# enkeejunior1/Diffusion-Pullback

Measured on AMD Instinct MI355X. Metric: pullback top-k SVD iters/sec (SD-v1.5 mid-block, 4x64x64), higher is better.
Workload: dtype bf16; 1 GPU; BASELINE configs[2]: SD-v1.5 4x64x64 latent, no edit prompt (seeded null ctx[1,77,768]), mid-block h[1280,8,8], t=696.27; pca_rank=5, ctx=null, samples_total=5, samples_this_rank=5, samples_advanced_together=1, spectrum=shaped (configs.Spectrum()), parallelism=single process, no collective, rccl_world_size=0, repeats=7

## Files before the change

diffusion_pullback_amd/csrc/elementwise.hip:

```cpp
#include "kernels.h"

namespace dpb {

static inline unsigned grid_for(long n) {
  long b = (n + 255) / 256;
  return (unsigned)(b < 1 ? 1 : (b > 16384 ? 16384 : b));
}

template <typename T, int MODE>
__global__ __launch_bounds__(256) void geglu_kernel(GegluArgs a, long nrows) {
  constexpr int CH = TT<T>::CH;
  const int fch = a.F / CH;
  const long total = nrows * fch;
  for (long idx = (long)blockIdx.x * 256 + threadIdx.x; idx < total; idx += (long)gridDim.x * 256) {
    const long row = idx / fch;
    const int c = (int)(idx - row * fch) * CH;
    long prow = row;
    if (MODE != MODE_PRIMAL) {
      long j = row / a.rows_per_sample, l = row - j * a.rows_per_sample;
      prow = (j / a.kps) * a.rows_per_sample + l;
    }
    const int ca = a.il ? ((c >> 6) << 7) + (c & 63) : c, dg_ = a.il ? 64 : a.F;
    const T* hp = (const T*)a.h + prow * 2 * a.F;
    float av[CH], gv[CH], o[CH];
    Vec<T>::load(hp + ca, av);
    Vec<T>::load(hp + ca + dg_, gv);
    if (MODE == MODE_PRIMAL) {
      float g1[CH], g2[CH];
#pragma unroll
      for (int e = 0; e < CH; ++e) {
        const float er = erff(gv[e] * 0.70710678118654752f);
        g1[e] = 0.5f * gv[e] * (1.f + er);
        g2[e] = av[e] * (0.5f * (1.f + er) + gv[e] * 0.39894228040143268f * __expf(-0.5f * gv[e] * gv[e]));
        o[e] = av[e] * g1[e];
      }
      Vec<T>::store((T*)a.y + row * a.F + c, o);
      if (a.stash) {
        T* hw = (T*)a.h + prow * 2 * a.F;
        Vec<T>::store(hw + ca, g1);
        Vec<T>::store(hw + ca + dg_, g2);
      }
    } else if (MODE == MODE_TANGENT) {
      const T* dp = (const T*)a.d + row * 2 * a.F;
      float da[CH], dg[CH];
      Vec<T>::load(dp + ca, da);
      Vec<T>::load(dp + ca + dg_, dg);
#pragma unroll
      for (int e = 0; e < CH; ++e) o[e] = da[e] * av[e] + dg[e] * gv[e];
      Vec<T>::store((T*)a.y + row * a.F + c, o);
    } else {
      float gy[CH], o2[CH];
      Vec<T>::load((const T*)a.d + row * a.F + c, gy);
#pragma unroll
      for (int e = 0; e < CH; ++e) {
        o[e] = gy[e] * av[e];
        o2[e] = gy[e] * gv[e];
      }
      T* yp = (T*)a.y + row * 2 * a.F;
      if (a.accumulate) {
        float t1[CH], t2[CH];
        Vec<T>::load(yp + ca, t1);
        Vec<T>::load(yp + ca + dg_, t2);
#pragma unroll
        for (int e = 0; e < CH; ++e) { o[e] += t1[e]; o2[e] += t2[e]; }
      }
      Vec<T>::store(yp + ca, o);
      Vec<T>::store(yp + ca + dg_, o2);
    }
  }
}

template <typename T>
static int geglu_t(int mode, const GegluArgs& a, hipStream_t st) {
  if (a.F % TT<T>::CH) { set_error("geglu: F=%d not chunk aligned", a.F); return -1; }
  if (a.il && (a.il != 64 || a.F % 64)) { set_error("geglu: interleave %d with F=%d unsupported (blocks of 64)", a.il, a.F); return -1; }
  long nrows = (long)(mode == MODE_PRIMAL ? a.Bp : a.NT) * a.rows_per_sample;
  unsigned g = grid_for(nrows * (a.F / TT<T>::CH));
  if (mode == MODE_PRIMAL) DPB_LAUNCH((geglu_kernel<T, MODE_PRIMAL>), dim3(g), dim3(256), 0, st, a, nrows);
  else if (mode == MODE_TANGENT) DPB_LAUNCH((geglu_kernel<T, MODE_TANGENT>), dim3(g), dim3(256), 0, st, a, nrows);
  else DPB_LAUNCH((geglu_kernel<T, MODE_ADJOINT>), dim3(g), dim3(256), 0, st, a, nrows);
  DPB_CHECK(hipGetLastError());
  return 0;
}
int launch_geglu(int dtype, int mode, const GegluArgs& a, hipStream_t st) {
  return DPB_DISPATCH_T(dtype, T, geglu_t<T>(mode, a, st));
}

template <typename T, int OP>
__global__ __launch_bounds__(256) void unary_kernel(const T* x, T* y, long nchunks) {
  constexpr int CH = TT<T>::CH;
  for (long i = (long)blockIdx.x * 256 + threadIdx.x; i < nchunks; i += (long)gridDim.x * 256) {
    float v[CH];
    Vec<T>::load(x + i * CH, v);
    if (OP == 0) {
#pragma unroll
      for (int e = 0; e < CH; ++e) v[e] = silu_(v[e]);
    } else if (OP == 3) {
#pragma unroll
      for (int e = 0; e < CH; ++e) v[e] = v[e] / (1.f + __expf(-1.702f * v[e]));
    } else if (OP == 4) {
#pragma unroll
      for (int e = 0; e < CH; ++e) v[e] = gelu_(v[e]);
    } else if (OP == 2) {
      float o[CH];
      Vec<T>::load(y + i * CH, o);
#pragma unroll
      for (int e = 0; e < CH; ++e) v[e] += o[e];
    }
    Vec<T>::store(y + i * CH, v);
  }
}

template <typename T>
static int unary_t(int op, const void* x, void* y, long n, hipStream_t st) {
  if (n % TT<T>::CH) { set_error("elementwise: n=%ld not chunk aligned", n); return -1; }
  long nc = n / TT<T>::CH;
  unsigned g = grid_for(nc);
  if (op == 0) DPB_LAUNCH((unary_kernel<T, 0>), dim3(g), dim3(256), 0, st, (const T*)x, (T*)y, nc);
  else if (op == 1) DPB_LAUNCH((unary_kernel<T, 1>), dim3(g), dim3(256), 0, st, (const T*)x, (T*)y, nc);
  else if (op == 3) DPB_LAUNCH((unary_kernel<T, 3>), dim3(g), dim3(256), 0, st, (const T*)x, (T*)y, nc);
  else if (op == 4) DPB_LAUNCH((unary_kernel<T, 4>), dim3(g), dim3(256), 0, st, (const T*)x, (T*)y, nc);
  else DPB_LAUNCH((unary_kernel<T, 2>), dim3(g), dim3(256), 0, st, (const T*)x, (T*)y, nc);
  DPB_CHECK(hipGetLastError());
  return 0;
}
int launch_silu(int dtype, const void* x, void* y, long n, hipStream_t st) {
  return DPB_DISPATCH_T(dtype, T, unary_t<T>(0, x, y, n, st));
}
int launch_quick_gelu(int dtype, const void* x, void* y, long n, hipStream_t st) {
  return DPB_DISPATCH_T(dtype, T, unary_t<T>(3, x, y, n, st));
}
int launch_gelu(int dtype, const void* x, void* y, long n, hipStream_t st) {
  return DPB_DISPATCH_T(dtype, T, unary_t<T>(4, x, y, n, st));
}

template <typename T>
__global__ __launch_bounds__(256) void embed_tokens_kernel(const int* ids, const T* tok, const T* pos, float* out, int L, int C, int vocab) {
  const int b = blockIdx.y, t = blockIdx.x;
  int id = ids[b * L + t];
  id = id < 0 ? 0 : (id >= vocab ? vocab - 1 : id);
  for (int c = threadIdx.x; c < C; c += 256)
    out[((long)b * C + c) * L + t] = TT<T>::ld(tok + (long)id * C + c) + TT<T>::ld(pos + (long)t * C + c);
}
int launch_embed_tokens(int dtype, const int* ids, const void* tok, const void* pos, float* out, int batch, int L, int C, int vocab, hipStream_t st) {
  if (batch <= 0 || L <= 0 || C <= 0 || vocab <= 0) { set_error("embed_tokens: empty problem"); return -1; }
  DPB_DISPATCH_STMT(dtype, T, DPB_LAUNCH((embed_tokens_kernel<T>), dim3(L, batch), dim3(256), 0, st, ids, (const T*)tok, (const T*)pos, out, L, C, vocab));
  DPB_CHECK(hipGetLastError());
  return 0;
}

int launch_axpy(int dtype, const void* x, void* y, long n, int accumulate, hipStream_t st) {
  int op = accumulate ? 2 : 1;
  return DPB_DISPATCH_T(dtype, T, unary_t<T>(op, x, y, n, st));
}

template <typename T>
__global__ __launch_bounds__(256) void copy_cols_kernel(const T* src, int lds_, int cs0, T* dst, int ldd, int cd0, long rows,
                                                        int ncols, int accumulate) {
  constexpr int CH = TT<T>::CH;
  const int nch = ncols / CH;
  const long total = rows * nch;
  for (long idx = (long)blockIdx.x * 256 + threadIdx.x; idx < total; idx += (long)gridDim.x * 256) {
    const long r = idx / nch;
    const int c = (int)(idx - r * nch) * CH;
    float v[CH];
    Vec<T>::load(src + r * lds_ + cs0 + c, v);
    T* dp = dst + r * ldd + cd0 + c;
    if (accumulate) {
      float o[CH];
      Vec<T>::load(dp, o);
#pragma unroll
      for (int e = 0; e < CH; ++e) v[e] += o[e];
    }
    Vec<T>::store(dp, v);
  }
}
int launch_copy_cols(int dtype, const void* src, int lds_, int cs0, void* dst, int ldd, int cd0, long rows, int ncols, int accumulate,
                     hipStream_t st) {
  int CH = dt_chunk(dtype);
  if (ncols % CH || cs0 % CH || cd0 % CH || lds_ % CH || ldd % CH) { set_error("copy_cols: misaligned window"); return -1; }
  unsigned g = grid_for(rows * (ncols / CH));
  DPB_DISPATCH_STMT(dtype, T, DPB_LAUNCH((copy_cols_kernel<T>), dim3(g), dim3(256), 0, st, (const T*)src, lds_, cs0, (T*)dst, ldd, cd0, rows, ncols, accumulate));
  DPB_CHECK(hipGetLastError());
  return 0;
}

template <typename T>
__global__ __launch_bounds__(256) void zero_cols_kernel(T* dst, int ldd, int cd0, long rows, int ncols) {
  constexpr int CH = TT<T>::CH;
  const int nch = ncols / CH;
  const long total = rows * nch;
  float v[CH];
#pragma unroll
  for (int e = 0; e < CH; ++e) v[e] = 0.f;
  for (long idx = (long)blockIdx.x * 256 + threadIdx.x; idx < total; idx += (long)gridDim.x * 256) {
    const long r = idx / nch;
    const int c = (int)(idx - r * nch) * CH;
    Vec<T>::store(dst + r * ldd + cd0 + c, v);
  }
}
int launch_zero_cols(int dtype, void* dst, int ldd, int cd0, long rows, int ncols, hipStream_t st) {
  int CH = dt_chunk(dtype);
  if (ncols % CH || cd0 % CH || ldd % CH || cd0 + ncols > ldd) { set_error("zero_cols: misaligned window"); return -1; }
  unsigned g = grid_for(rows * (ncols / CH));
  DPB_DISPATCH_STMT(dtype, T, DPB_LAUNCH((zero_cols_kernel<T>), dim3(g), dim3(256), 0, st, (T*)dst, ldd, cd0, rows, ncols));
  DPB_CHECK(hipGetLastError());
  return 0;
}

template <typename T>
__global__ __launch_bounds__(256) void nchw_to_nhwc_kernel(const float* src, T* dst, int C, int HW, int Cpad) {
  __shared__ float tile[32][33];
  const int n = blockIdx.z;
  const int p0 = blockIdx.x * 32, c0 = blockIdx.y * 32;
  const int tx = threadIdx.x & 31, ty = threadIdx.x >> 5;
  for (int k = ty; k < 32; k += 8) {
    int c = c0 + k, p = p0 + tx;
    tile[k][tx] = (c < C && p < HW) ? src[((long)n * C + c) * HW + p] : 0.f;
  }
  __syncthreads();
  for (int k = ty; k < 32; k += 8) {
    int p = p0 + k, c = c0 + tx;
    if (p < HW && c < Cpad) TT<T>::st(dst + ((long)n * HW + p) * Cpad + c, tile[tx][k]);
  }
}
template <typename T>
__global__ __launch_bounds__(256) void nhwc_to_nchw_kernel(const T* src, float* dst, int C, int HW, int Cpad) {
  __shared__ float tile[32][33];
  const int n = blockIdx.z;
  const int p0 = blockIdx.x * 32, c0 = blockIdx.y * 32;
  const int tx = threadIdx.x & 31, ty = threadIdx.x >> 5;
  for (int k = ty; k < 32; k += 8) {
    int p = p0 + k, c = c0 + tx;
    tile[k][tx] = (p < HW && c < C) ? TT<T>::ld(src + ((long)n * HW + p) * Cpad + c) : 0.f;
  }
  __syncthreads();
  for (int k = ty; k < 32; k += 8) {
    int c = c0 + k, p = p0 + tx;
    if (c < C && p < HW) dst[((long)n * C + c) * HW + p] = tile[tx][k];
  }
}
int launch_nchw_to_nhwc(int dtype, const float* src, void* dst, int n, int C, int HW, int Cpad, hipStream_t st) {
  dim3 grid((HW + 31) / 32, (Cpad + 31) / 32, n);
  DPB_DISPATCH_STMT(dtype, T, DPB_LAUNCH((nchw_to_nhwc_kernel<T>), grid, dim3(256), 0, st, src, (T*)dst, C, HW, Cpad));
  DPB_CHECK(hipGetLastError());
  return 0;
}
int launch_nhwc_to_nchw(int dtype, const void* src, float* dst, int n, int C, int HW, int Cpad, hipStream_t st) {
  dim3 grid((HW + 31) / 32, (C + 31) / 32, n);
  DPB_DISPATCH_STMT(dtype, T, DPB_LAUNCH((nhwc_to_nchw_kernel<T>), grid, dim3(256), 0, st, (const T*)src, dst, C, HW, Cpad));
  DPB_CHECK(hipGetLastError());
  return 0;
}

constexpr int SHIFT_TP = 32, SHIFT_TC = 64;
template <typename T, int VEC>
__global__ __launch_bounds__(256) void shift_tap_kernel(T* h, const float* u, ShiftRows rows, int b0, int nb, int bcast, int C, int Cv, long HW) {
  constexpr int CPP = SHIFT_TC / VEC;
  constexpr int ITER = SHIFT_TP * CPP / 256;
  __shared__ float tile[SHIFT_TC][SHIFT_TP + 1];
  const long p0 = (long)blockIdx.x * SHIFT_TP;
  const int c0 = blockIdx.y * SHIFT_TC;
  const int tx = threadIdx.x & 31, ty = threadIdx.x >> 5;
  const long img = HW * (long)C;
  float src[ITER][VEC];
  auto ld = [&](const T* p, float* o) {
    if constexpr (VEC == 1) o[0] = TT<T>::ld(p); else Vec<T>::load(p, o);
  };
  auto st = [&](T* p, const float* o) {
    if constexpr (VEC == 1) TT<T>::st(p, o[0]); else Vec<T>::store(p, o);
  };
  if (bcast) {
#pragma unroll
    for (int it = 0; it < ITER; ++it) {
      const int q = it * 256 + threadIdx.x, pl = q / CPP, c = c0 + (q % CPP) * VEC;
      if (p0 + pl < HW && c < C) ld(h + (p0 + pl) * C + c, src[it]);
    }
  }
  for (int r = 0; r < nb; ++r) {
    const int b = b0 + r, dir = rows.dir[r];
    const float sc = rows.scale[r];
    if (dir < 0 && !(bcast && b > 0)) continue;
    if (dir >= 0) {
      __syncthreads();
      const float* ub = u + (long)dir * Cv * HW;
      for (int k = ty; k < SHIFT_TC; k += 8) {
        const int c = c0 + k;
        tile[k][tx] = (c < Cv && p0 + tx < HW) ? ub[(long)c * HW + p0 + tx] : 0.f;
      }
      __syncthreads();
    }
    T* hb = h + (long)b * img;
#pragma unroll
    for (int it = 0; it < ITER; ++it) {
      const int q = it * 256 + threadIdx.x, pl = q / CPP, cl = (q % CPP) * VEC, c = c0 + cl;
      if (p0 + pl >= HW || c >= C) continue;
      T* p = hb + (p0 + pl) * C + c;
      float v[VEC];
      if (bcast) {
#pragma unroll
        for (int e = 0; e < VEC; ++e) v[e] = src[it][e];
      } else {
        ld(p, v);
      }
      if (dir >= 0) {
#pragma unroll
        for (int e = 0; e < VEC; ++e) v[e] += sc * tile[cl + e][pl];
      }
      st(p, v);
    }
  }
}

template <typename T>
static int shift_tap_t(void* h, const float* u, const int* dir, const float* scale, int batch, int bcast, int C, int Cv, long HW, hipStream_t st) {
  const dim3 grid((unsigned)((HW + SHIFT_TP - 1) / SHIFT_TP), (unsigned)((C + SHIFT_TC - 1) / SHIFT_TC));
  for (int b0 = (batch - 1) / SHIFT_MAX_ROWS * SHIFT_MAX_ROWS; b0 >= 0; b0 -= SHIFT_MAX_ROWS) {
    ShiftRows rows;
    const int nb = std::min(SHIFT_MAX_ROWS, batch - b0);
    for (int r = 0; r < nb; ++r) { rows.dir[r] = dir[b0 + r]; rows.scale[r] = scale[b0 + r]; }
    if (C % TT<T>::CH == 0) DPB_LAUNCH((shift_tap_kernel<T, TT<T>::CH>), grid, dim3(256), 0, st, (T*)h, u, rows, b0, nb, bcast, C, Cv, HW);
    else DPB_LAUNCH((shift_tap_kernel<T, 1>), grid, dim3(256), 0, st, (T*)h, u, rows, b0, nb, bcast, C, Cv, HW);
    DPB_CHECK(hipGetLastError());
  }
  return 0;
}
int launch_shift_tap(int dtype, void* h, const float* u, const int* dir, const float* scale, int batch, int bcast, int C, int Cv, long HW,
                     hipStream_t st) {
  if (batch < 1 || C < 1 || Cv < 1 || Cv > C || HW < 1) { set_error("shift_tap: empty or inconsistent problem"); return -1; }
  return DPB_DISPATCH_T(dtype, T, shift_tap_t<T>(h, u, dir, scale, batch, bcast, C, Cv, HW, st));
}

__global__ __launch_bounds__(256) void replicate_rows_kernel(ReplTable t, int batch) {
  uint4* p = (uint4*)t.p[blockIdx.y];
  const long n = t.chunks[blockIdx.y];
  for (long i = (long)blockIdx.x * 256 + threadIdx.x; i < n; i += (long)gridDim.x * 256) {
    const uint4 v = p[i];
    for (int b = 1; b < batch; ++b) p[(long)b * n + i] = v;
  }
}
int launch_replicate_rows(void* const* bufs, const size_t* sample_bytes, int nbufs, int batch, hipStream_t st) {
  if (batch < 2) return 0;
  for (int i0 = 0; i0 < nbufs; i0 += REPL_MAX_BUFS) {
    ReplTable t;
    const int n = std::min(REPL_MAX_BUFS, nbufs - i0);
    long most = 1;
    for (int i = 0; i < n; ++i) {
      if (sample_bytes[i0 + i] % 16 || (uintptr_t)bufs[i0 + i] % 16) { set_error("replicate_rows: buffer %d is not a whole number of aligned 16-byte chunks per sample", i0 + i); return -1; }
      t.p[i] = bufs[i0 + i];
      t.chunks[i] = (long)(sample_bytes[i0 + i] / 16);
      most = std::max(most, t.chunks[i]);
    }
    DPB_LAUNCH(replicate_rows_kernel, dim3(std::min(grid_for(most), 2048u), n), dim3(256), 0, st, t, batch);
    DPB_CHECK(hipGetLastError());
  }
  return 0;
}

template <typename T>
__global__ __launch_bounds__(256) void pool2x2_kernel(const T* in, T* out, int n, int H, int W, int C, int accumulate, float scale) {
  constexpr int CH = TT<T>::CH;
  const int cch = C / CH;
  const long total = (long)n * H * W * cch;
  for (long idx = (long)blockIdx.x * 256 + threadIdx.x; idx < total; idx += (long)gridDim.x * 256) {
    const int c = (int)(idx % cch) * CH;
    long pix = idx / cch;
    const int x = (int)(pix % W);
    pix /= W;
    const int y = (int)(pix % H);
    const long s = pix / H;
    float acc[CH];
#pragma unroll
    for (int e = 0; e < CH; ++e) acc[e] = 0.f;
#pragma unroll
    for (int dy = 0; dy < 2; ++dy)
#pragma unroll
      for (int dx = 0; dx < 2; ++dx) {
        float v[CH];
        Vec<T>::load(in + ((s * 2 * H + 2 * y + dy) * 2 * W + 2 * x + dx) * C + c, v);
#pragma unroll
        for (int e = 0; e < CH; ++e) acc[e] += v[e];
      }
    T* op = out + ((s * H + y) * W + x) * C + c;
#pragma unroll
    for (int e = 0; e < CH; ++e) acc[e] *= scale;
    if (accumulate) {
      float o[CH];
      Vec<T>::load(op, o);
#pragma unroll
      for (int e = 0; e < CH; ++e) acc[e] += o[e];
    }
    Vec<T>::store(op, acc);
  }
}
template <typename T>
__global__ __launch_bounds__(256) void up2x2_kernel(const T* in, T* out, int n, int H, int W, int C, int accumulate, float scale) {
  constexpr int CH = TT<T>::CH;
// ... 83 lines not shown
```

diffusion_pullback_amd/csrc/engine.cpp:

```cpp
#include <math.h>
#include <stdarg.h>
#include <stdio.h>
#include <stdlib.h>
#include <string.h>

#include <string>
#include <vector>

#include "../../include/dpb.h"
#include "kernels.h"

namespace dpb {

static thread_local char g_err[1024] = "";
void set_error(const char* fmt, ...) {
  va_list ap;
  va_start(ap, fmt);
  vsnprintf(g_err, sizeof(g_err), fmt, ap);
  va_end(ap);
}
const char* last_error() { return g_err; }
thread_local long launch_count = 0;

static inline size_t align_up(size_t v, size_t a = 256) { return (v + a - 1) / a * a; }
static inline int round8(int v) { return (v + 7) / 8 * 8; }

struct Buf {
  int rows = 0, C = 0, kind = 0, Cv = 0;
  bool is_const = true;
  size_t p_off = 0, t_off = 0, g_off = 0, g_off0 = 0;
};

struct AttnPlan {
  int heads = 0, d = 0, Lq = 0, Lk = 0, Lqp = 0, Lkp = 0;
  bool causal = false;
  bool kv_const = false, fused = false, cross = false;
  int oq = 0, ok = 0, ov = 0;
  size_t P = 0, PT = 0, KT = 0, VT = 0, QT = 0, stats = 0;
  bool fold_ok = false;
  bool fold_live = false;
  int q_op = -1, o_op = -1;
  size_t Gt = 0, Gk = 0, F = 0, Fk = 0, Pf = 0;
  const char* gA = nullptr;
};

struct Op {
  dpb_op_desc d;
  bool is_const = true;
  int attn = -1;
  size_t pstats = 0, tstats = 0;
  size_t aff = 0;
  int geglu_next = -1;
  int geglu_prev = -1;
  int ln_next = -1;
  int ln_prev = -1;
  int fold_plan = -1, fold_role = 0;
};

}

using namespace dpb;

struct dpb_engine {
  int dtype = DT_F32, es = 4;
  int maxB = 1, maxT = 1;
  std::vector<Buf> bufs;
  std::vector<Op> ops;
  std::vector<AttnPlan> plans;
  std::vector<int> producer;
  std::vector<std::vector<int>> mod_users;
  int x_buf = -1, x_channels = 0, temb_buf = -1, temb_dim = 0, temb_flip = 0, temb_hm1 = 0, ctx_buf = -1;
  std::string per_sample_t_why;
  bool temb_read = false;
  hipStream_t stream = 0;
  char* ws = nullptr;
  size_t ws_bytes = 0;
  size_t pstats_off = 0, pstats_bytes = 0, tstats_off = 0, tstats_bytes = 0, gnpart = 0, gnpart_bytes = 0, gnticket = 0;
  size_t S1 = 0, S2 = 0, T1 = 0, Dv = 0, convtmp = 0, io_in = 0, io_out = 0, orth = 0, slab = 0, slab_bytes = 64u << 20, zeros = 0;
  size_t orth_stride = 0;
  size_t pbW = 0;
  size_t temb_host_stage = 0;
  int cur_batch = 0;
  std::vector<int> uses;
  std::vector<std::vector<char>> act_cache;
  int primal_last = -1;
  struct { bool on = false; GemmArgs a; } pend;
  std::vector<char> ginit;
  std::vector<char> skip;
  long n_launch = 0;
  double flops = 0, gbytes = 0;
  struct GraphKey {
    int tap, k, B; const void *V, *U, *s, *conv;
    bool operator==(const GraphKey& o) const { return tap == o.tap && k == o.k && B == o.B && V == o.V && U == o.U && s == o.s && conv == o.conv; }
  };
  hipGraphExec_t gexec = nullptr;
  GraphKey gkey{};
  long g_launches = 0; double g_flops = 0, g_bytes = 0;
  bool profiling = false;
  struct Prof { hipEvent_t a, b; double flops; int big; int M, N, K, Z, gather; };
  std::vector<Prof> prof;
  float prof_overhead_ms = 0.f;

  char* P(int b) const { return ws + bufs[b].p_off; }
  char* T(int b) const { return ws + bufs[b].t_off; }
  char* G(int b) const { return ws + bufs[b].g_off; }
};

namespace {

int fail(const char* fmt, ...) {
  va_list ap;
  va_start(ap, fmt);
  vsnprintf(g_err, sizeof(g_err), fmt, ap);
  va_end(ap);
  return -1;
}

struct Forward {
  bool stash = true;
  bool temb_resident = false;
  int seed = -1;
  const float* h = nullptr;
  const float* u = nullptr; const int32_t* dir = nullptr; const float* scale = nullptr;
  int xbatch = 0;
};

struct Pass {
  int mode, tap;
  int src;
  const char *bact, *oact;
  Forward fwd;
  bool per_sample_t = false;
  int srow = 0;
  Pass(const dpb_engine* e, int mode_, int tap_, int src_, const char* flags)
      : mode(mode_), tap(tap_), src(src_), bact(flags), oact(flags + e->bufs.size()) {}
};

struct OpInputs {
  int id[4], n;
  const int* begin() const { return id; }
  const int* end() const { return id + n; }
};
OpInputs op_inputs(const dpb_op_desc& d) {
  OpInputs r{{d.in0}, 1};
  if (d.kind == DPB_OP_ATTENTION || d.kind == DPB_OP_CONCAT) r.id[r.n++] = d.in1;
  if (d.kind == DPB_OP_ATTENTION) r.id[r.n++] = d.in2;
  if (d.kind == DPB_OP_CONV && d.res >= 0) r.id[r.n++] = d.res;
  if (d.kind == DPB_OP_GROUPNORM && d.ip[2]) r.id[r.n++] = d.in1;
  return r;
}
bool gn_modulated(const dpb_op_desc& d) { return d.kind == DPB_OP_GROUPNORM && d.ip[2] != 0; }

struct LaunchSpan {
  dpb_engine* e; long at;
  explicit LaunchSpan(dpb_engine* e_) : e(e_), at(launch_count) {}
  ~LaunchSpan() { e->n_launch = launch_count - at; }
};

char* primal_ptr(const dpb_engine* e, const Pass& ps, int b) {
  const Buf& bf = e->bufs[b];
  return e->P(b) + (bf.kind == DPB_BUF_SHARED ? (size_t)ps.srow * bf.rows * bf.C * e->es : 0);
}

void gemm_prep(dpb_engine* e, GemmArgs& a) {
  a.slab = (float*)(e->ws + e->slab);
  a.zeros = e->ws + e->zeros;
  a.slab_bytes = e->slab_bytes;
}

int g_lazy_reduce = getenv("DPB_LAZY_REDUCE") ? atoi(getenv("DPB_LAZY_REDUCE")) : 1;
int g_ln_fuse = getenv("DPB_LN_FUSE") ? atoi(getenv("DPB_LN_FUSE")) : 0;
int g_ln_kmax = getenv("DPB_LN_FUSE_KMAX") ? atoi(getenv("DPB_LN_FUSE_KMAX")) : 1024;

int flush_pending(dpb_engine* e) {
  if (!e->pend.on) return 0;
  e->pend.on = false;
  return launch_gemm_reduce(e->dtype, e->pend.a, e->stream);
}

int prof_open(dpb_engine* e, double flops, int kind, int M, int N, int K, int Z, int gather) {
  if (!e->profiling) return -1;
  dpb_engine::Prof p;
  p.flops = flops; p.big = kind; p.M = M; p.N = N; p.K = K; p.Z = Z; p.gather = gather;
  if (hipEventCreate(&p.a) != hipSuccess) return -1;
  if (hipEventCreate(&p.b) != hipSuccess) { (void)hipEventDestroy(p.a); return -1; }
  (void)hipEventRecord(p.a, e->stream);
  e->prof.push_back(p);
  return (int)e->prof.size() - 1;
}
void prof_close(dpb_engine* e, int idx) {
  if (idx >= 0) (void)hipEventRecord(e->prof[idx].b, e->stream);
}

int g_geglu_fwd = getenv("DPB_GEGLU_FWD") ? atoi(getenv("DPB_GEGLU_FWD")) : 1;
int g_cross_primal = getenv("DPB_CROSS_PRIMAL") ? atoi(getenv("DPB_CROSS_PRIMAL")) : 1;
int g_cross_fold = getenv("DPB_CROSS_FOLD") ? atoi(getenv("DPB_CROSS_FOLD")) : 1;
bool fold_route(const dpb_engine* e, const AttnPlan& p) {
  if (!g_cross_fold || !p.fold_ok || e->cur_batch != 1 || !g_cross_primal) return false;
  if (g_cross_fold == 2) return true;
  const long H = p.heads, C = H * p.d;
  return 208 * H * C <= 2 * C * C + 384 * C && (g_cross_fold == 1 || C >= g_cross_fold);
}
bool fold_on(const dpb_engine* e, const Pass& ps, const AttnPlan& p) {
  return p.fold_live && fold_route(e, p) && e->producer[ps.src] < p.q_op && e->producer[ps.tap] >= p.o_op;
}
int gemm(dpb_engine* e, GemmArgs a, bool can_defer = false) {
  if (e->pend.on)
    if (int r = flush_pending(e)) return r;
  gemm_prep(e, a);
  GemmArgs* pend = (can_defer && g_lazy_reduce) ? &e->pend.a : nullptr;
  const double fl = 2.0 * a.M * (double)a.N * ((double)a.K + (a.A2 ? a.K2 : 0)) * a.Z1 * a.Z2;
  e->flops += fl;
  e->gbytes += ((double)a.M * a.K + (double)a.N * a.K + (double)a.M * a.N) * a.Z1 * a.Z2 * e->es;
  const GemmPlan pl = gemm_plan(e->dtype, a);
  const int pi = prof_open(e, fl, pl.row ? pl.row->kind : 0, a.M, a.N, a.K, a.Z1 * a.Z2, a.gather);
  const int r = launch_gemm(e->dtype, a, e->stream, pend, &pl);
  e->pend.on = pend && pend->splitk > 1;
  prof_close(e, pi);
  return r;
}

int conv_fwd(dpb_engine* e, const Op& op, const Pass& ps, int n) {
  const dpb_op_desc& d = op.d;
  const int mode = ps.mode;
  const int H = d.ip[0], W = d.ip[1], Cin = d.ip[2], Ho = d.ip[3], Wo = d.ip[4], Cout = d.ip[5], KS = d.ip[6];
  const Buf& bi = e->bufs[d.in0];
  const Buf& bo = e->bufs[d.out];
  if (mode == 1 && !ps.bact[d.in0]) {
    return launch_axpy(e->dtype, e->T(d.res), e->T(d.out), (long)n * bo.rows * bo.C, 0, e->stream);
  }
  GemmArgs g;
  const bool shared_out = bo.kind == DPB_BUF_SHARED;
  const int ns = shared_out ? 1 : n;
  g.A = mode == 0 ? primal_ptr(e, ps, d.in0) : e->T(d.in0);
  g.B = d.w[0];
  g.C = mode == 0 ? primal_ptr(e, ps, d.out) : e->T(d.out);
  g.N = Cout;
  g.K = KS * KS * Cin;
  g.ldb = g.K;
  g.ldc = bo.C;
  g.lda = bi.C;
  g.gather = d.ip[9];
  if (g.gather == GATHER_NONE) {
    g.M = ns * bi.rows;
  } else {
    g.M = ns * Ho * Wo;
    g.H = H; g.W = W; g.Cin = Cin; g.Ho = Ho; g.Wo = Wo; g.KS = KS; g.stride = d.ip[7]; g.pad = d.ip[8];
  }
  if (mode == 0) {
    g.bias = (const float*)d.w[2];
    if (d.rowbias >= 0) {
      g.rowbias = e->P(d.rowbias) + (size_t)d.ip[10] * e->es;
      g.rows_per_sample = bo.rows;
      g.ldrb = e->bufs[d.rowbias].rows * e->bufs[d.rowbias].C;
      g.rowbias_div = ps.per_sample_t ? 1 : 1 << 30;
    }
  }
  if (d.res >= 0 && (mode == 0 || ps.bact[d.res])) {
    g.R = mode == 0 ? primal_ptr(e, ps, d.res) : e->T(d.res);
    g.ldr = e->bufs[d.res].C;
  }
  if (mode == 1 && op.fold_role && fold_on(e, ps, e->plans[op.fold_plan])) {
    const AttnPlan& p = e->plans[op.fold_plan];
    if (op.fold_role == 1) return 0;
    g.A = e->ws + e->S1; g.lda = 80 * p.heads;
    g.B = e->ws + p.Fk; g.K = g.ldb = 80 * p.heads;
  }
  if (mode == 1 && op.ln_next >= 0 && g_ln_fuse) {
    const dpb_op_desc& ld = e->ops[op.ln_next].d;
    GemmArgs f = g;
    f.epi = EPI_LN_TAN; f.C2 = e->T(ld.out); f.ln_x = e->P(ld.in0); f.ln_gamma = (const float*)ld.w[0]; f.ln_eps = ld.fp[0];
    f.rows_per_sample = bo.rows; f.epi_kps = n / e->cur_batch;
    gemm_prep(e, f);
    if (gemm_epi_supported(e->dtype, f)) {
      e->skip[op.ln_next] = 1;
      return gemm(e, f);
    }
  }
  if (mode == 1 && op.geglu_next >= 0) {
    const dpb_op_desc& gd = e->ops[op.geglu_next].d;
    GemmArgs f = g;
    f.epi = EPI_GEGLU_TAN; f.hprim = e->P(d.out); f.epi_kps = n / e->cur_batch; f.rows_per_sample = bo.rows;
    f.C = e->T(gd.out); f.ldc = e->bufs[gd.out].C;
    gemm_prep(e, f);
    if (gemm_epi_supported(e->dtype, f)) {
      e->skip[op.geglu_next] = 1;
      return gemm(e, f);
    }
  }
  if (mode == 0 && !ps.fwd.stash && op.geglu_next >= 0 && g_geglu_fwd && !shared_out && d.out != ps.tap && d.out != ps.fwd.seed) {
    const dpb_op_desc& gd = e->ops[op.geglu_next].d;
    GemmArgs f = g;
    f.epi = EPI_GEGLU_FWD; f.C = e->P(gd.out); f.ldc = e->bufs[gd.out].C; f.rowbias = nullptr; f.R = nullptr;
    gemm_prep(e, f);
    GemmArgs probe = g; gemm_prep(e, probe);
    if (!g.rowbias && !g.R && gemm_epi_supported(e->dtype, f) && gemm_plan(e->dtype, probe).splitk == 1) {
      e->skip[op.geglu_next] = 1;
      return gemm(e, f);
    }
  }
  return gemm(e, g, mode == 1 && !shared_out);
}

int conv_adj(dpb_engine* e, const Op& op, const Pass& ps, int n) {
  const dpb_op_desc& d = op.d;
  const int H = d.ip[0], W = d.ip[1], Cin = d.ip[2], Ho = d.ip[3], Wo = d.ip[4], KS = d.ip[6];
  const Buf& bi = e->bufs[d.in0];
  const Buf& bo = e->bufs[d.out];
  const int Cout = bo.C;
  if (ps.bact[d.in0]) {
    if (!d.w[1]) return fail("conv op has no transposed weight (w[1]) but its adjoint is needed");
    GemmArgs g;
    g.A = e->G(d.out);
    g.lda = bo.C;
    g.B = d.w[1];
    g.N = Cin;
    g.K = KS * KS * Cout;
    g.ldb = g.K;
    g.ldc = bi.C;
    const int gather = d.ip[9];
    if (op.fold_role && fold_on(e, ps, e->plans[op.fold_plan])) {
      AttnPlan& p = e->plans[op.fold_plan];
      if (op.fold_role == 2) {
        p.gA = e->G(d.out);
        e->ginit[d.in0] = 1;
        goto residual;
      }
      g.A = e->ws + e->S1; g.lda = 80 * p.heads;
      g.B = e->ws + p.Gk; g.K = g.ldb = 80 * p.heads;
    }
    if (gather == GATHER_NONE && op.ln_prev >= 0 && g_ln_fuse && e->uses[d.in0] == 1 && d.in0 != ps.src && (g.K <= g_ln_kmax || (g_ln_fuse & 2))) {
      const dpb_op_desc& ld = e->ops[op.ln_prev].d;
      GemmArgs f = g;
      f.M = n * bi.rows;
      f.epi = EPI_LN_ADJ; f.C = e->G(ld.in0); f.ldc = e->bufs[ld.in0].C; f.accumulate = e->ginit[ld.in0];
      f.ln_x = e->P(ld.in0); f.ln_gamma = (const float*)ld.w[0]; f.ln_eps = ld.fp[0];
      f.rows_per_sample = bi.rows; f.epi_kps = n / e->cur_batch;
      gemm_prep(e, f);
      if (gemm_epi_supported(e->dtype, f)) {
        if (int r = gemm(e, f)) return r;
        e->ginit[ld.in0] = 1;
        goto residual;
      }
    }
    if (gather == GATHER_NONE && op.geglu_prev >= 0 && d.in0 != ps.src) {
      const dpb_op_desc& gd = e->ops[op.geglu_prev].d;
      GemmArgs f = g;
      f.M = n * bi.rows;
      f.epi = EPI_GEGLU_ADJ; f.hprim = e->P(gd.in0); f.epi_kps = n / e->cur_batch; f.rows_per_sample = bi.rows;
      f.C = e->G(gd.in0); f.ldc = e->bufs[gd.in0].C; f.accumulate = e->ginit[gd.in0];
      gemm_prep(e, f);
      if (gemm_epi_supported(e->dtype, f)) {
        if (int r = gemm(e, f)) return r;
        e->ginit[gd.in0] = 1;
        goto residual;
      }
    }
    const bool lone = e->uses[d.in0] == 1 && d.in0 != ps.src;
    if (gather == GATHER_NONE) {
      g.M = n * bi.rows;
      g.C = e->G(d.in0);
      g.accumulate = e->ginit[d.in0];
      if (int r = gemm(e, g, lone)) return r;
    } else if (gather == GATHER_CONV) {
      g.gather = GATHER_CONVT;
      g.M = n * H * W;
      g.H = Ho; g.W = Wo; g.Cin = Cout; g.Ho = H; g.Wo = W; g.KS = KS; g.stride = d.ip[7]; g.pad = d.ip[8];
      g.C = e->G(d.in0);
      g.accumulate = e->ginit[d.in0];
      if (int r = gemm(e, g, lone)) return r;
    } else {
      g.gather = GATHER_CONVT;
      g.M = n * Ho * Wo;
      g.H = Ho; g.W = Wo; g.Cin = Cout; g.Ho = Ho; g.Wo = Wo; g.KS = KS; g.stride = 1; g.pad = 1;
      g.C = e->ws + e->convtmp;
      if (int r = gemm(e, g)) return r;
      if (int r = launch_pool2x2_sum(e->dtype, e->ws + e->convtmp, e->G(d.in0), n, H, W, bi.C, e->ginit[d.in0], e->stream)) return r;
    }
    e->ginit[d.in0] = 1;
  }
residual:
  if (d.res >= 0 && ps.bact[d.res]) {
    Buf& br = e->bufs[d.res];
    if (!e->ginit[d.res] && br.rows == bo.rows && br.C == bo.C && br.kind == bo.kind) {
      std::swap(br.g_off, e->bufs[d.out].g_off);
    } else {
      if (int r = launch_axpy(e->dtype, e->G(d.out), e->G(d.res), (long)n * bo.rows * bo.C, e->ginit[d.res], e->stream)) return r;
    }
    e->ginit[d.res] = 1;
  }
  return 0;
}

void take_pending(dpb_engine* e, SlabSrc& src, const void* d, bool store) {
  if (!e->pend.on || e->pend.a.C != d) return;
  const GemmArgs& g = e->pend.a;
  src.slab = g.slab; src.splitk = g.splitk; src.MN = (long)g.M * g.N; src.N = g.N;
  src.R = g.R; src.ldr = g.ldr;
  src.store = store ? g.C : nullptr;
  e->pend.on = false;
}

bool consumes_pending(dpb_engine* e, const Op& op, int mode) {
  if (mode == MODE_PRIMAL || (op.d.kind != DPB_OP_GROUPNORM && op.d.kind != DPB_OP_LAYERNORM)) return false;
  const void* d = mode == MODE_TANGENT ? (const void*)e->T(op.d.in0) : (const void*)e->G(op.d.out);
  if (d != e->pend.a.C) return false;
  const Buf& bi = e->bufs[op.d.in0];
  if (e->pend.a.N != bi.C) return false;
  if (op.d.kind == DPB_OP_GROUPNORM) {
    GNArgs a; a.HW = bi.rows; a.C = bi.C; a.G = op.d.ip[0]; a.NT = 1;
    return groupnorm_is_one_launch(e->dtype, a);
  }
  return true;
}

template <class A>
void fill_io(dpb_engine* e, const dpb_op_desc& d, const Pass& ps, int n, A& a) {
  if (ps.mode == MODE_PRIMAL) { a.Bp = n; a.y = e->P(d.out); return; }
  a.Bp = e->cur_batch; a.NT = n; a.kps = n / e->cur_batch;
  if (ps.mode == MODE_TANGENT) { a.d = e->T(d.in0); a.y = e->T(d.out); return; }
  a.d = e->G(d.out); a.y = e->G(d.in0);
  a.accumulate = e->ginit[d.in0];
  e->ginit[d.in0] = 1;
}
template <class A>
void fill_norm_io(dpb_engine* e, const dpb_op_desc& d, const Pass& ps, int n, A& a) {
  fill_io(e, d, ps, n, a);
  if (ps.mode != MODE_PRIMAL) take_pending(e, a.src, a.d, ps.mode == MODE_TANGENT && (e->uses[d.in0] > 1 || d.in0 == ps.tap));
}

int gn_run(dpb_engine* e, const Op& op, const Pass& ps, int n) {
  const dpb_op_desc& d = op.d;
  const Buf& bi = e->bufs[d.in0];
  GNArgs a;
  a.x = e->P(d.in0);
  a.gamma = (const float*)d.w[0];
  a.beta = (const float*)d.w[1];
  if (gn_modulated(d)) {
    a.gamma = (const float*)(e->ws + op.aff);
    a.beta = a.gamma + (size_t)e->maxB * bi.C;
    a.astride = bi.C;
  }
  a.pstats = (double*)(e->ws + op.pstats);
  a.tstats = (double*)(e->ws + op.tstats);
  a.part = (float*)(e->ws + e->gnpart); a.part_bytes = e->gnpart_bytes; a.ticket = (int*)(e->ws + e->gnticket);
  a.det = gn_deterministic();
  a.HW = bi.rows; a.C = bi.C; a.G = d.ip[0]; a.silu = d.ip[1]; a.eps = d.fp[0];
  fill_norm_io(e, d, ps, n, a);
  return launch_groupnorm(e->dtype, ps.mode, a, e->stream);
}

int ln_run(dpb_engine* e, const Op& op, const Pass& ps, int n) {
  const dpb_op_desc& d = op.d;
  const Buf& bi = e->bufs[d.in0];
  LNArgs a;
  a.x = e->P(d.in0);
  a.gamma = (const float*)d.w[0];
  a.beta = (const float*)d.w[1];
  a.rows_per_sample = bi.rows; a.C = bi.C; a.eps = d.fp[0];
  fill_norm_io(e, d, ps, n, a);
  return launch_layernorm(e->dtype, ps.mode, a, e->stream);
}

int geglu_run(dpb_engine* e, const Op& op, const Pass& ps, int n) {
  const dpb_op_desc& d = op.d;
  const Buf& bi = e->bufs[d.in0];
  GegluArgs a;
  a.h = e->P(d.in0);
  a.rows_per_sample = bi.rows; a.F = bi.C / 2; a.il = d.ip[1];
  a.stash = ps.fwd.stash;
  fill_io(e, d, ps, n, a);
  return launch_geglu(e->dtype, ps.mode, a, e->stream);
}

int fill_affine(dpb_engine* e, int src, const Pass& ps, int batch) {
  const std::vector<int>& users = e->mod_users[src];
  if (users.empty()) return 0;
  const Buf& be = e->bufs[e->ops[src].d.out];
  std::vector<AdaGNOp> t(users.size());
  for (size_t i = 0; i < users.size(); ++i) {
    const Op& u = e->ops[users[i]];
    const int C = e->bufs[u.d.in0].C;
    t[i].gamma = (const float*)u.d.w[0]; t[i].beta = (const float*)u.d.w[1];
    t[i].emb = e->P(u.d.in1) + (size_t)u.d.ip[3] * e->es;
    t[i].og = (float*)(e->ws + u.aff); t[i].ob = t[i].og + (size_t)e->maxB * C;
    t[i].C = C;
  }
  return launch_adagn_affine(e->dtype, t.data(), (int)t.size(), (long)be.rows * be.C, batch, ps.per_sample_t ? 1 : 0, e->stream);
}

int resample_run(dpb_engine* e, const Op& op, const Pass& ps, int n) {
  const dpb_op_desc& d = op.d;
  const bool up = d.ip[0] == 1;
  const int H = d.ip[1], W = d.ip[2], C = e->bufs[d.in0].C;
  const int h = up ? H : H / 2, w = up ? W : W / 2;
  if (ps.mode == MODE_ADJOINT) {
    const int acc = e->ginit[d.in0];
    e->ginit[d.in0] = 1;
    return up ? launch_pool2x2(e->dtype, e->G(d.out), e->G(d.in0), n, h, w, C, 1.f, acc, e->stream)
              : launch_up2x2(e->dtype, e->G(d.out), e->G(d.in0), n, h, w, C, 0.25f, acc, e->stream);
  }
  const char* in = ps.mode == MODE_PRIMAL ? e->P(d.in0) : e->T(d.in0);
  char* out = ps.mode == MODE_PRIMAL ? e->P(d.out) : e->T(d.out);
  return up ? launch_up2x2(e->dtype, in, out, n, h, w, C, 1.f, 0, e->stream) : launch_pool2x2(e->dtype, in, out, n, h, w, C, 0.25f, 0, e->stream);
}

int concat_run(dpb_engine* e, const Op& op, const Pass& ps, int n) {
  const dpb_op_desc& d = op.d;
  const int mode = ps.mode;
  const Buf& b0 = e->bufs[d.in0];
  const Buf& b1 = e->bufs[d.in1];
  const Buf& bo = e->bufs[d.out];
  const long rows = (long)n * bo.rows;
  if (mode == MODE_ADJOINT) {
    if (ps.bact[d.in0]) {
      if (int r = launch_copy_cols(e->dtype, e->G(d.out), bo.C, 0, e->G(d.in0), b0.C, 0, rows, b0.C, e->ginit[d.in0], e->stream)) return r;
      e->ginit[d.in0] = 1;
    }
    if (ps.bact[d.in1]) {
      if (int r = launch_copy_cols(e->dtype, e->G(d.out), bo.C, b0.C, e->G(d.in1), b1.C, 0, rows, b1.C, e->ginit[d.in1], e->stream)) return r;
      e->ginit[d.in1] = 1;
    }
    return 0;
  }
  if (mode == MODE_TANGENT && (!ps.bact[d.in0] || !ps.bact[d.in1])) {
    char* o = e->T(d.out);
    if (int r = ps.bact[d.in0] ? launch_copy_cols(e->dtype, e->T(d.in0), b0.C, 0, o, bo.C, 0, rows, b0.C, 0, e->stream)
                               : launch_zero_cols(e->dtype, o, bo.C, 0, rows, b0.C, e->stream)) return r;
    return ps.bact[d.in1] ? launch_copy_cols(e->dtype, e->T(d.in1), b1.C, 0, o, bo.C, b0.C, rows, b1.C, 0, e->stream)
                          : launch_zero_cols(e->dtype, o, bo.C, b0.C, rows, b1.C, e->stream);
  }
  char* o = mode == MODE_PRIMAL ? e->P(d.out) : e->T(d.out);
  const char* i0 = mode == MODE_PRIMAL ? e->P(d.in0) : e->T(d.in0);
  const char* i1 = mode == MODE_PRIMAL ? e->P(d.in1) : e->T(d.in1);
  if (int r = launch_copy_cols(e->dtype, i0, b0.C, 0, o, bo.C, 0, rows, b0.C, 0, e->stream)) return r;
  return launch_copy_cols(e->dtype, i1, b1.C, 0, o, bo.C, b0.C, rows, b1.C, 0, e->stream);
}

struct AttnPtrs {
  const char *Q, *K, *V; char* O;
  int ldq, ldk, ldv, ldo;
};
static AttnPtrs attn_ptrs(dpb_engine* e, const dpb_op_desc& d, const AttnPlan& p, int which ) {
  AttnPtrs a;
  auto base = [&](int b) { return which == 0 ? e->P(b) : which == 1 ? e->T(b) : e->G(b); };
  a.ldq = e->bufs[d.in0].C; a.ldk = e->bufs[d.in1].C; a.ldv = e->bufs[d.in2].C; a.ldo = e->bufs[d.out].C;
  a.Q = base(d.in0) + (size_t)p.oq * e->es;
  a.K = (which == 0 || !p.kv_const) ? base(d.in1) + (size_t)p.ok * e->es : nullptr;
  a.V = (which == 0 || !p.kv_const) ? base(d.in2) + (size_t)p.ov * e->es : nullptr;
  a.O = base(d.out);
  return a;
}

void fill_fused(dpb_engine* e, const AttnPlan& p, const AttnPtrs& x, FusedAttnArgs& f, int kps, float scale) {
  char* ws = e->ws;
  f.Q = x.Q; f.K = x.K; f.V = x.V; f.O = x.O; f.VT = ws + p.VT; f.KT = ws + p.KT; f.QT = ws + p.QT;
  f.stats = (const float*)(ws + p.stats);
  f.L = p.Lq; f.C = x.ldq; f.Co = x.ldo; f.H = p.heads; f.d = p.d; f.kps = kps; f.scale = scale; f.fl = e->dtype == DT_F16;
}
void fill_cross(dpb_engine* e, const AttnPlan& p, const AttnPtrs& x, CrossAttnArgs& f, int kps, float scale, const void* BT, const void* X, int Cx,
                void* Y, int Cy) {
  f.Q = x.Q; f.K = x.K; f.V = x.V; f.BT = BT; f.X = X; f.Y = Y;
  f.L = p.Lq; f.Lk = p.Lk; f.Lkp = p.Lkp; f.C = x.ldq; f.Ck = x.ldk; f.Cx = Cx; f.Cy = Cy;
  f.H = p.heads; f.d = p.d; f.kps = kps; f.scale = scale; f.fl = e->dtype == DT_F16;
}

template <class F>
int attn_launch(dpb_engine* e, const AttnPlan& p, int kind, int n_prod, int Z1, int gather, F launch) {
  const double fl = 2.0 * p.Lq * (double)p.Lk * p.d * n_prod * Z1 * p.heads;
  e->flops += fl;
  const int pi = prof_open(e, fl, kind, p.Lq, p.Lk, p.d, Z1 * p.heads, gather);
  const int r = launch();
  prof_close(e, pi);
  return r;
}

enum Side { SIDE_A, SIDE_B, SIDE_C, SIDE_A2, SIDE_B2 };
void set_side(GemmArgs& g, Side s, const void* ptr, int ld, long s1, long s2, int div) {
  switch (s) {
    case SIDE_A: g.A = ptr; g.lda = ld; g.sA1 = s1; g.sA2 = s2; g.divA = div; break;
    case SIDE_B: g.B = ptr; g.ldb = ld; g.sB1 = s1; g.sB2 = s2; g.divB = div; break;
    case SIDE_C: g.C = (void*)ptr; g.ldc = ld; g.sC1 = s1; g.sC2 = s2; break;
    case SIDE_A2: g.A2 = ptr; g.lda2 = ld; g.sA21 = s1; g.sA22 = s2; g.divA2 = div; break;
    case SIDE_B2: g.B2 = ptr; g.ldb2 = ld; g.sB21 = s1; g.sB22 = s2; g.divB2 = div; break;
  }
}
void side_rows(GemmArgs& g, Side s, const void* ptr, int ld, int L, int d, int div = 1) { set_side(g, s, ptr, ld, (long)L * ld, d, div); }
void side_tile(GemmArgs& g, Side s, const void* ptr, int H, int rows, int Lp, int div = 1) {
  set_side(g, s, ptr, Lp, (long)H * rows * Lp, (long)rows * Lp, div);
}
void dims(GemmArgs& g, int M, int N, int K, int Z1, int Z2, float alpha = 1.f) { g.M = M; g.N = N; g.K = K; g.Z1 = Z1; g.Z2 = Z2; g.alpha = alpha; }
int head_transpose(dpb_engine* e, const AttnPlan& p, const void* in, int ld, void* out, int Z, int L, int Lp) {
  return launch_transpose(e->dtype, in, out, Z, p.heads, (long)L * ld, p.d, L, p.d, ld, Lp, (long)p.d * Lp, e->stream);
}

int fold_build(dpb_engine* e, const AttnPlan& p, const AttnPtrs& x, float scale) {
  const int H = p.heads, C = H * p.d, W = 80 * H;
  const void* WqT = e->ops[p.q_op].d.w[1];
  const void* Wo = e->ops[p.o_op].d.w[0];
  char* ws = e->ws;
  for (int which = 0; which < 2; ++which) {
    const void* kv = which ? x.V : x.K; const int ldkv = which ? x.ldv : x.ldk;
    const void* w = which ? Wo : WqT;
    const float alpha = which ? 1.f : scale;
    GemmArgs t;
    side_rows(t, SIDE_A, kv, ldkv, p.Lk, p.d);
    side_rows(t, SIDE_B, w, C, C, p.d);
    set_side(t, SIDE_C, ws + (which ? p.F : p.Gt), C, 0, 128L * C, 1);
    dims(t, p.Lk, C, p.d, 1, H, alpha);
    if (int r = gemm(e, t)) return r;
    GemmArgs k;
    side_rows(k, SIDE_A, w, C, C, p.d);
    side_rows(k, SIDE_B, kv, ldkv, p.Lk, p.d);
    set_side(k, SIDE_C, ws + (which ? p.Fk : p.Gk), W, 0, 80, 1);
    dims(k, C, p.Lk, p.d, 1, H, alpha);
    if (int r = gemm(e, k)) return r;
  }
  return 0;
}

int fold_product1(dpb_engine* e, const AttnPlan& p, const void* X, int ldx, size_t B, int nt) {
  const int H = p.heads, C = H * p.d;
  GemmArgs g;
  g.A = X; g.lda = ldx; g.B = e->ws + B; g.ldb = C;
// ... 279 lines not shown
extern "C" {

const char* dpb_last_error(void) { return g_err; }
int dpb_abi_version(void) { return DPB_ABI_VERSION; }

int dpb_engine_create(const dpb_net_desc* net, dpb_engine** out) {
  if (!net || !out) return fail("null argument");
  if (net->dtype != DPB_F32 && net->dtype != DPB_BF16 && net->dtype != DPB_F16) return fail("bad dtype %d", net->dtype);
  if (net->max_batch < 1 || net->max_tangents < 1) return fail("max_batch/max_tangents must be >= 1");
  dpb_engine* e = new dpb_engine();
  e->dtype = net->dtype;
  e->es = net->dtype == DPB_F32 ? 4 : 2;
  e->maxB = net->max_batch;
  e->maxT = net->max_tangents;
  e->x_buf = net->x_buf; e->x_channels = net->x_channels; e->temb_buf = net->temb_buf; e->temb_dim = net->temb_dim;
  e->temb_flip = net->temb_flip_sin_to_cos; e->temb_hm1 = net->temb_half_minus_one; e->ctx_buf = net->ctx_buf;
  const int nb = net->n_buffers;
  e->bufs.resize(nb);
  e->producer.assign(nb, -1);
  auto bad = [&](const char* m, int i) { fail("op %d: %s", i, m); delete e; return -1; };
  for (int i = 0; i < nb; ++i) {
    e->bufs[i].rows = net->buffers[i].rows;
    e->bufs[i].C = net->buffers[i].channels;
    e->bufs[i].kind = net->buffers[i].kind;
    e->bufs[i].Cv = net->buffers[i].valid_channels > 0 ? net->buffers[i].valid_channels : net->buffers[i].channels;
    if (e->bufs[i].rows < 1 || e->bufs[i].C < 8 || e->bufs[i].C % 8) { fail("buffer %d: rows=%d channels=%d (channels must be a multiple of 8)", i, e->bufs[i].rows, e->bufs[i].C); delete e; return -1; }
  }
  if (net->x_buf < 0 || net->x_buf >= nb) { fail("bad x_buf"); delete e; return -1; }
  e->bufs[net->x_buf].is_const = false;
  auto okb = [&](int b) { return b >= 0 && b < nb; };
  for (int i = 0; i < net->n_ops; ++i) {
    Op op;
    op.d = net->ops[i];
    const dpb_op_desc& d = op.d;
    if (!okb(d.out)) return bad("bad buffer id", i);
    bool c = true;
    for (int b : op_inputs(d)) {
      if (!okb(b)) return bad("bad buffer id", i);
      c = c && e->bufs[b].is_const;
    }
    if (d.kind == DPB_OP_ATTENTION) {
      AttnPlan p;
      p.heads = d.ip[0];
      p.oq = d.ip[1]; p.ok = d.ip[2]; p.ov = d.ip[3];
      p.causal = d.ip[4] != 0;
      const int Cattn = e->bufs[d.out].C;
      if (p.heads < 1 || Cattn % p.heads) return bad("channels not divisible by heads", i);
      p.d = Cattn / p.heads;
      if (p.oq % 8 || p.ok % 8 || p.ov % 8 || p.oq + Cattn > e->bufs[d.in0].C || p.ok + Cattn > e->bufs[d.in1].C || p.ov + Cattn > e->bufs[d.in2].C)
        return bad("bad q/k/v column window", i);
      auto part = [&](int b0, int o0, int b1, int o1) { return b0 == b1 && o0 != o1 && o0 < o1 + Cattn && o1 < o0 + Cattn; };
      if (part(d.in0, p.oq, d.in1, p.ok) || part(d.in0, p.oq, d.in2, p.ov) || part(d.in1, p.ok, d.in2, p.ov))
        return bad("q/k/v windows of one buffer must coincide or be disjoint", i);
      if (p.d % 8) return bad("head dim must be a multiple of 8", i);
      p.Lq = e->bufs[d.in0].rows; p.Lk = e->bufs[d.in1].rows;
      p.Lqp = round8(p.Lq); p.Lkp = round8(p.Lk);
      if (e->bufs[d.in1].is_const != e->bufs[d.in2].is_const) return bad("k and v must both depend on x or both not", i);
      if (e->bufs[d.in0].is_const) return bad("attention query independent of x is unsupported", i);
      p.kv_const = e->bufs[d.in1].is_const;
      op.attn = (int)e->plans.size();
      e->plans.push_back(p);
    }
    if (d.kind == DPB_OP_CONV) {
      if (d.rowbias >= 0 && (!okb(d.rowbias) || e->bufs[d.rowbias].kind != DPB_BUF_SHARED)) return bad("rowbias must be a SHARED buffer", i);
      if (d.rowbias >= 0 && (d.ip[10] < 0 || d.ip[10] % 8 || d.ip[10] + round8(d.ip[5]) > e->bufs[d.rowbias].C)) return bad("bad rowbias column window", i);
      if (!d.w[0]) return bad("missing weight", i);
      if (d.ip[2] != e->bufs[d.in0].C || e->bufs[d.out].C != round8(d.ip[5])) return bad("conv channel mismatch", i);
    }
    if (d.kind == DPB_OP_GROUPNORM) {
      const Buf& gi = e->bufs[d.in0];
      if (gn_modulated(d)) {
        if (e->bufs[d.in1].kind != DPB_BUF_SHARED || e->bufs[d.in1].rows != 1 || e->producer[d.in1] < 0)
          return bad("modulated groupnorm: in1 must be a one-row SHARED buffer produced by an earlier op (the embedding projection)", i);
        if (gi.kind != DPB_BUF_ACT) return bad("modulated groupnorm: the normalised buffer must be a per-sample activation", i);
        if (d.ip[3] < 0 || d.ip[3] % 8 || d.ip[3] + 2 * gi.C > e->bufs[d.in1].C) return bad("modulated groupnorm: bad (scale | shift) column window", i);
        if (!d.w[0] || !d.w[1]) return bad("modulated groupnorm: missing gamma / beta", i);
      }
    }
    if (d.kind == DPB_OP_RESAMPLE) {
      const Buf& ri = e->bufs[d.in0];
      const Buf& ro = e->bufs[d.out];
      const int H = d.ip[1], W = d.ip[2];
      if (d.ip[0] != 0 && d.ip[0] != 1) return bad("resample: ip[0] must be 0 (2x2 average pool) or 1 (nearest x2 upsample)", i);
      if (H < 1 || W < 1 || (long)H * W != ri.rows || ri.C != ro.C || ri.kind != DPB_BUF_ACT || ro.kind != DPB_BUF_ACT) return bad("resample: input shape mismatch", i);
      if (d.ip[0] == 0 ? (H % 2 || W % 2 || (long)(H / 2) * (W / 2) != ro.rows) : (long)4 * H * W != ro.rows) return bad("resample: output shape mismatch", i);
    }
    for (int b : op_inputs(d)) e->temb_read = e->temb_read || b == e->temb_buf;
    if (e->per_sample_t_why.empty()) {
      char why[160] = "";
      const bool so = e->bufs[d.out].kind == DPB_BUF_SHARED;
      for (int b : op_inputs(d))
        if ((e->bufs[b].kind == DPB_BUF_SHARED) != so && !(gn_modulated(d) && b == d.in1))
          snprintf(why, sizeof(why), "op %d reads %s buffer %d into %s buffer %d", i, so ? "per-sample" : "SHARED", b, so ? "SHARED" : "per-sample", d.out);
      if (so && !(d.kind == DPB_OP_SILU || (d.kind == DPB_OP_CONV && d.ip[9] == DPB_GATHER_NONE && d.rowbias < 0)))
        snprintf(why, sizeof(why), "op %d writes SHARED buffer %d and is neither a linear layer nor an activation", i, d.out);
      e->per_sample_t_why = why;
    }
    op.is_const = c;
    e->bufs[d.out].is_const = c;
    if (e->producer[d.out] >= 0) return bad("buffer written twice (tape must be SSA)", i);
    e->producer[d.out] = i;
    e->ops.push_back(op);
  }
  e->mod_users.assign(e->ops.size(), std::vector<int>());
  for (size_t i = 0; i < e->ops.size(); ++i)
    if (gn_modulated(e->ops[i].d)) e->mod_users[e->producer[e->ops[i].d.in1]].push_back((int)i);
  {
    std::vector<int> uses(nb, 0), user(nb, -1);
    for (size_t i = 0; i < e->ops.size(); ++i) {
      for (int b : op_inputs(e->ops[i].d)) { uses[b]++; user[b] = (int)i; }
    }
    e->uses = uses;
    for (size_t j = 0; j < e->ops.size(); ++j) {
      const dpb_op_desc& d = e->ops[j].d;
      if (d.kind != DPB_OP_LAYERNORM || e->ops[j].is_const || e->dtype == DT_F32 || e->bufs[d.in0].C != 320 || e->bufs[d.in0].kind != DPB_BUF_ACT) continue;
      const int pi = e->producer[d.in0];
      if (pi >= 0 && e->ops[pi].d.kind == DPB_OP_CONV && e->ops[pi].d.ip[9] == DPB_GATHER_NONE && !e->ops[pi].is_const) e->ops[pi].ln_next = (int)j;
      if (uses[d.out] == 1) {
        const int ci = user[d.out];
        const dpb_op_desc& cd = e->ops[ci].d;
        if (cd.kind == DPB_OP_CONV && cd.ip[9] == DPB_GATHER_NONE && cd.in0 == d.out && cd.w[1]) e->ops[ci].ln_prev = (int)j;
      }
    }
    for (size_t j = 0; j < e->ops.size(); ++j) {
      const dpb_op_desc& d = e->ops[j].d;
      if (d.kind == DPB_OP_GEGLU && uses[d.in0] != 1) return bad("the input buffer of a GEGLU op must have no other consumer (the primal pass overwrites it in place)", (int)j);
      if (d.kind != DPB_OP_GEGLU || d.ip[1] != 64 || e->ops[j].is_const || getenv("DPB_NO_GEGLU_FUSE")) continue;
      const int pi = e->producer[d.in0];
      if (pi >= 0 && uses[d.in0] == 1) {
        const dpb_op_desc& pd = e->ops[pi].d;
        if (pd.kind == DPB_OP_CONV && pd.ip[9] == DPB_GATHER_NONE && pd.res < 0 && e->bufs[d.in0].kind == DPB_BUF_ACT) e->ops[pi].geglu_next = (int)j;
      }
      if (uses[d.out] == 1) {
        const int ci = user[d.out];
        const dpb_op_desc& cd = e->ops[ci].d;
        if (cd.kind == DPB_OP_CONV && cd.ip[9] == DPB_GATHER_NONE && cd.in0 == d.out) e->ops[ci].geglu_prev = (int)j;
      }
    }
    for (size_t j = 1; j + 1 < e->ops.size(); ++j) {
      const dpb_op_desc& d = e->ops[j].d;
      if (d.kind != DPB_OP_ATTENTION || e->ops[j].is_const) continue;
      AttnPlan& p = e->plans[e->ops[j].attn];
      const int C = p.heads * p.d;
      if (!p.kv_const || p.causal || e->dtype == DT_F32 || p.oq != 0 || e->bufs[d.in0].C != C || e->bufs[d.out].C != C || p.Lk > 80) continue;
      const dpb_op_desc &qd = e->ops[j - 1].d, &od = e->ops[j + 1].d;
      auto plain = [&](const dpb_op_desc& c) {
        return c.kind == DPB_OP_CONV && c.ip[9] == DPB_GATHER_NONE && c.ip[6] == 1 && c.ip[2] == C && c.ip[5] == C && c.rowbias < 0 && c.w[1] &&
               e->bufs[c.in0].kind == DPB_BUF_ACT && e->bufs[c.out].kind == DPB_BUF_ACT;
      };
      if (!plain(qd) || qd.out != d.in0 || qd.res >= 0 || uses[d.in0] != 1 || e->ops[j - 1].is_const) continue;
      if (!plain(od) || od.in0 != d.out || uses[d.out] != 1) continue;
      p.q_op = (int)j - 1; p.o_op = (int)j + 1; p.fold_ok = true;
    }
    e->skip.assign(e->ops.size(), 0);
  }
  size_t off = 0;
  auto take = [&](size_t bytes) { size_t o = off; off = align_up(off + bytes); return o; };
  const size_t es = e->es;
  for (auto& b : e->bufs) {
    size_t n = e->maxB;
    b.p_off = take(n * b.rows * (size_t)b.C * es);
  }
  for (auto& b : e->bufs)
    if (!b.is_const) b.t_off = take((size_t)e->maxT * b.rows * b.C * es);
  for (auto& b : e->bufs)
    if (!b.is_const) b.g_off = b.g_off0 = take((size_t)e->maxT * b.rows * b.C * es);
  size_t s1 = 0, s2 = 0, t1 = 0, dv = 0, ctmp = 0, maxrc = 0;
  for (auto& op : e->ops) {
    const dpb_op_desc& d = op.d;
    if (d.kind == DPB_OP_ATTENTION) {
      AttnPlan& p = e->plans[op.attn];
      const size_t H = p.heads;
      p.fused = !p.causal && fused_attention_supported(e->dtype, p.d, p.Lq, p.kv_const) && !getenv("DPB_NO_FUSED_ATTN") &&
                p.Lq >= (getenv("DPB_FUSED_ATTN_MIN_L") ? atoi(getenv("DPB_FUSED_ATTN_MIN_L")) : 64) &&
                e->bufs[d.in0].C == e->bufs[d.in1].C && e->bufs[d.in0].C == e->bufs[d.in2].C;
      p.cross = !p.causal && cross_attention_supported(e->dtype, p.d, p.Lq, p.Lk, p.kv_const) && !getenv("DPB_NO_CROSS_ATTN") &&
                e->bufs[d.in1].C == e->bufs[d.in2].C;
      if (!p.fused) p.P = take((size_t)e->maxB * H * p.Lq * p.Lkp * es);
      p.fold_ok = p.fold_ok && p.cross;
      if (p.fold_ok) {
        const size_t C = H * p.d;
        p.Gt = take(H * 128 * C * es); p.F = take(H * 128 * C * es);
        p.Gk = take(C * 80 * H * es); p.Fk = take(C * 80 * H * es);
        p.Pf = take((size_t)p.Lq * H * 80 * sizeof(float));
        s1 = std::max(s1, (size_t)e->maxT * H * p.Lq * 80 * es);
        e->ops[p.q_op].fold_plan = e->ops[p.o_op].fold_plan = op.attn;
        e->ops[p.q_op].fold_role = 1; e->ops[p.o_op].fold_role = 2;
      }
      p.VT = take((size_t)e->maxB * H * p.d * p.Lkp * es);
      p.KT = take((size_t)e->maxB * H * p.d * p.Lkp * es);
      if (!p.fused) s1 = std::max(s1, (size_t)e->maxT * H * p.Lq * p.Lkp * es);
      size_t lmax = std::max(p.Lqp, p.Lkp);
      t1 = std::max(t1, (size_t)e->maxT * H * p.d * lmax * es);
      if (p.fused) p.stats = take((size_t)e->maxB * H * p.Lq * 2 * sizeof(float));
      if (!p.kv_const) {
        if (!p.fused) p.PT = take((size_t)e->maxB * H * p.Lk * p.Lqp * es);
        p.QT = take((size_t)e->maxB * H * p.d * p.Lqp * es);
        if (!p.fused) s2 = std::max(s2, (size_t)e->maxT * H * p.Lk * p.Lqp * es);
        dv = std::max(dv, (size_t)e->maxT * H * p.Lq * sizeof(float));
      }
    } else if (d.kind == DPB_OP_GROUPNORM) {
      op.pstats = e->pstats_bytes;
      e->pstats_bytes += (size_t)e->maxB * d.ip[0] * 2 * sizeof(double);
      if (!op.is_const) {
        op.tstats = e->tstats_bytes;
        e->tstats_bytes += (size_t)e->maxT * d.ip[0] * 2 * sizeof(double);
      }
      if (gn_modulated(d)) op.aff = take((size_t)2 * e->maxB * e->bufs[d.in0].C * sizeof(float));
    } else if (d.kind == DPB_OP_CONV && d.ip[9] == DPB_GATHER_UPCONV && !op.is_const) {
      ctmp = std::max(ctmp, (size_t)e->maxT * d.ip[3] * d.ip[4] * e->bufs[d.in0].C * es);
    }
  }
  for (auto& b : e->bufs) maxrc = std::max(maxrc, (size_t)b.rows * b.C);
  e->pstats_off = take(e->pstats_bytes);
  e->tstats_off = take(e->tstats_bytes);
  {
    size_t need = 0;
    for (auto& op : e->ops)
      if (op.d.kind == DPB_OP_GROUPNORM) {
        const size_t hw = e->bufs[op.d.in0].rows, nmax = (size_t)std::max(e->maxB, e->maxT);
        const size_t blocks = std::max<size_t>(nmax * ((hw + 7) / 8), 1);
        need = std::max(need, std::min<size_t>(blocks, std::max<size_t>(1024, nmax * ((hw + 63) / 64))) * 2 * op.d.ip[0] * sizeof(float));
      }
    e->gnpart_bytes = need;
    e->gnpart = take(need);
    e->gnticket = take(sizeof(int) * (size_t)std::max(e->maxB, e->maxT));
  }
  for (auto& op : e->ops)
    if (op.d.kind == DPB_OP_GROUPNORM) { op.pstats += e->pstats_off; op.tstats += e->tstats_off; }
  e->S1 = take(s1); e->S2 = take(s2); e->T1 = take(t1); e->Dv = take(dv); e->convtmp = take(ctmp);
  const size_t nio = (size_t)std::max(e->maxB, e->maxT) * maxrc * sizeof(float);
  e->io_in = take(nio);
  e->io_out = take(nio);
  e->orth_stride = align_up(orth_scratch_bytes(std::min(ORTH_MAX_RANK, std::max(56, e->maxT)), (long)e->bufs[e->x_buf].rows * e->x_channels));
  e->orth = take(e->orth_stride * (size_t)e->maxB);
  e->slab = take(e->slab_bytes);
  e->zeros = take(256);
  const size_t nx = (size_t)e->bufs[e->x_buf].rows * e->x_channels;
  e->pbW = take((size_t)e->maxT * nx * sizeof(float));
  e->ws_bytes = off;
  e->ginit.assign(nb, 0);
  e->act_cache.assign(nb, std::vector<char>());
  if (!seed_flags(e, e->x_buf)) { delete e; return -1; }
  *out = e;
  return 0;
}

void dpb_engine_destroy(dpb_engine* e) {
  if (e && e->gexec) (void)hipGraphExecDestroy(e->gexec);
  delete e;
}

int dpb_engine_set_stream(dpb_engine* e, void* s) {
  if (!e) return fail("null engine");
  e->stream = (hipStream_t)s;
  return 0;
}

size_t dpb_engine_workspace_bytes(const dpb_engine* e) { return e ? e->ws_bytes : 0; }

int dpb_engine_set_workspace(dpb_engine* e, void* ws, size_t bytes) {
  if (!e || !ws) return fail("null argument");
  if (bytes < e->ws_bytes) return fail("workspace too small: %zu < %zu", bytes, e->ws_bytes);
  if ((uintptr_t)ws % 256) return fail("workspace must be 256-byte aligned");
  e->ws = (char*)ws;
  e->cur_batch = 0;
  DPB_CHECK(hipMemsetAsync(ws, 0, e->ws_bytes, e->stream));
  return 0;
}

static int shift_seed(dpb_engine* e, const Forward& f, int batch, int xb, int last) {
  const int src = f.seed, ps = e->producer[src];
  const Buf& bs = e->bufs[src];
  if (int r = launch_shift_tap(e->dtype, e->P(src), f.u, f.dir, f.scale, batch, xb < batch, bs.C, bs.Cv, bs.rows, e->stream)) return r;
  if (xb == batch) return 0;
  std::vector<char> seen(e->bufs.size(), 0);
  std::vector<void*> ptr;
  std::vector<size_t> bytes;
  for (int i = ps + 1; i <= last; ++i)
    for (int b : op_inputs(e->ops[i].d)) {
      if (b == src || seen[b] || e->bufs[b].kind == DPB_BUF_SHARED || e->producer[b] > ps) continue;
      seen[b] = 1;
      ptr.push_back(e->P(b));
      bytes.push_back((size_t)e->bufs[b].rows * e->bufs[b].C * e->es);
    }
  return launch_replicate_rows(ptr.data(), bytes.data(), (int)ptr.size(), batch, e->stream);
}

static void temb_row(const dpb_engine* e, float t, float* emb) {
  const int half = e->temb_dim / 2;
  for (int i = 0; i < half; ++i) {
    float fr;
    if (e->temb_hm1) fr = expf((float)i * (float)(-(log(10000.0) / (double)(half - 1))));
    else fr = expf(((float)(-log(10000.0)) * (float)i) / (float)half);
    float ang = t * fr;
    float s = sinf(ang), c = cosf(ang);
    if (e->temb_flip) { emb[i] = c; emb[half + i] = s; } else { emb[i] = s; emb[half + i] = c; }
  }
}

static int primal_pass(dpb_engine* e, const float* x, int batch, float t, const float* ctx, int upto_buf, const Forward& f, const float* tv = nullptr) {
  if (!e || !x) return fail("null argument");
  if (!e->ws) return fail("workspace not set (dpb_engine_set_workspace)");
  if (batch < 1 || batch > e->maxB) return fail("batch=%d outside [1,%d]", batch, e->maxB);
  if (upto_buf < 0 || upto_buf >= (int)e->bufs.size() || e->producer[upto_buf] < 0) return fail("invalid upto buffer %d", upto_buf);
  const LaunchSpan span(e);
  e->flops = 0; e->gbytes = 0;
  Pass ps(e, MODE_PRIMAL, upto_buf, e->x_buf, seed_flags(e, e->x_buf));
  ps.fwd = f;
  ps.per_sample_t = tv != nullptr;
  const Buf& bx = e->bufs[e->x_buf];
  const int xb = f.u ? f.xbatch : batch;
  if (int r = launch_nchw_to_nhwc(e->dtype, x, e->P(e->x_buf), xb, e->x_channels, bx.rows, bx.C, e->stream)) return r;
  if (e->ctx_buf >= 0) {
    if (!ctx) return fail("this network needs ctx (encoder_hidden_states)");
    const Buf& bc = e->bufs[e->ctx_buf];
    if (int r = launch_nchw_to_nhwc(e->dtype, ctx, e->P(e->ctx_buf), xb * bc.rows, bc.Cv, 1, bc.C, e->stream)) return r;
  }
  if (e->temb_buf >= 0 && !f.temb_resident) {
    const int nrow = tv ? batch : 1;
    const size_t C = e->bufs[e->temb_buf].C;
    std::vector<float> emb(nrow * C, 0.f);
    for (int b = 0; b < nrow; ++b) temb_row(e, tv ? tv[b] : t, emb.data() + b * C);
    float* stage = (float*)(e->ws + e->io_in);
    DPB_CHECK(hipMemcpyAsync(stage, emb.data(), emb.size() * sizeof(float), hipMemcpyHostToDevice, e->stream));
    DPB_CHECK(hipStreamSynchronize(e->stream));
    for (int b = 0; b < nrow; ++b)
      if (int r = launch_nchw_to_nhwc(e->dtype, stage + b * C, e->P(e->temb_buf) + b * C * e->es, 1, (int)C, 1, (int)C, e->stream)) return r;
  }
  if (e->pstats_bytes && !gn_deterministic()) DPB_CHECK(hipMemsetAsync(e->ws + e->pstats_off, 0, e->pstats_bytes, e->stream));
  e->cur_batch = batch;
  e->pend.on = false;
  const int last = e->producer[upto_buf];
  const int seed_op = f.seed >= 0 ? e->producer[f.seed] : -1;
  e->primal_last = -1;
  for (auto& p : e->plans) p.fold_live = false;
  std::fill(e->skip.begin(), e->skip.end(), 0);
  for (int i = 0; i <= last; ++i) {
    if (e->skip[i]) continue;
    const int reps = tv && e->bufs[e->ops[i].d.out].kind == DPB_BUF_SHARED ? batch : 1;
    for (ps.srow = 0; ps.srow < reps; ++ps.srow)
      if (int r = run_op(e, e->ops[i], ps, i <= seed_op ? xb : batch)) return r;
    ps.srow = 0;
    if (int r = fill_affine(e, i, ps, batch)) return r;
    if (i == seed_op && f.u) {
      if (int r = shift_seed(e, f, batch, xb, last)) return r;
    } else if (i == seed_op) {
      const Buf& bs = e->bufs[f.seed];
      if (int r = launch_nchw_to_nhwc(e->dtype, f.h, e->P(f.seed), batch, bs.Cv, bs.rows, bs.C, e->stream)) return r;
    }
  }
  if (f.stash) e->primal_last = last;
  return 0;
}

int dpb_primal(dpb_engine* e, const float* x, int batch, float t, const float* ctx, int upto_buf) {
  return primal_pass(e, x, batch, t, ctx, upto_buf, Forward());
}

static int check_timesteps(dpb_engine* e, int batch, const float* t, const float** tv) {
  if (!e || !t) return fail("null argument");
  if (batch < 1 || batch > e->maxB) return fail("batch=%d outside [1,%d]", batch, e->maxB);
  *tv = nullptr;
  for (int b = 0; b < batch; ++b) {
    if (!isfinite(t[b])) return fail("t[%d] is not finite", b);
    if (t[b] != t[0]) *tv = t;
  }
  if (!*tv) return 0;
  if (e->temb_buf < 0 || !e->temb_read) return fail("distinct timesteps on a network without a timestep embedding (no op reads temb_buf): its samples cannot differ in t");
  if (e->bufs[e->temb_buf].kind != DPB_BUF_SHARED || e->bufs[e->temb_buf].rows != 1) return fail("distinct timesteps need temb_buf to be a SHARED buffer of one row");
  if (!e->per_sample_t_why.empty()) return fail("distinct timesteps are unsupported on this tape: %s", e->per_sample_t_why.c_str());
  return 0;
}

int dpb_primal_t(dpb_engine* e, const float* x, int batch, const float* t, const float* ctx, int upto_buf) {
  const float* tv;
  if (int r = check_timesteps(e, batch, t, &tv)) return r;
  return primal_pass(e, x, batch, t[0], ctx, upto_buf, Forward(), tv);
}

static int forward_pass(dpb_engine* e, const float* x, int batch, float t, const float* ctx, int upto_buf, int channels, float* out, const Forward& f,
                        const float* tv = nullptr) {
  if (!e || !out) return fail("null argument");
  int r = primal_pass(e, x, batch, t, ctx, upto_buf, f, tv);
  if (!r) r = dpb_read_buffer(e, upto_buf, channels, out);
  e->cur_batch = 0;
  return r;
}

int dpb_forward(dpb_engine* e, const float* x, int batch, float t, const float* ctx, int upto_buf, int channels, float* out) {
  Forward f;
  f.stash = false;
  return forward_pass(e, x, batch, t, ctx, upto_buf, channels, out, f);
}

int dpb_forward_t(dpb_engine* e, const float* x, int batch, const float* t, const float* ctx, int upto_buf, int channels, float* out) {
  const float* tv;
  if (int r = check_timesteps(e, batch, t, &tv)) return r;
  Forward f;
  f.stash = false;
  return forward_pass(e, x, batch, t[0], ctx, upto_buf, channels, out, f, tv);
}

int dpb_forward_from(dpb_engine* e, const float* x, int batch, float t, const float* ctx, int src_buf, const float* h, int dst_buf, int channels,
                     float* out) {
  if (!e || !out || !h) return fail("null argument");
  if (int r = check_pair(e, src_buf, dst_buf, FOR_FORWARD)) return r;
  Forward f;
  f.stash = false; f.seed = src_buf; f.h = h;
  return forward_pass(e, x, batch, t, ctx, dst_buf, channels, out, f);
}

int dpb_forward_shift(dpb_engine* e, const float* x, int xbatch, int batch, float t, const float* ctx, int src_buf, const float* u, int nu,
                      const int32_t* dir, const float* scale, int dst_buf, int channels, float* out) {
  if (!e || !x || !out || !dir || !scale) return fail("null argument");
  e->cur_batch = 0;
  if (batch < 1 || batch > e->maxB) return fail("batch=%d outside [1,%d]", batch, e->maxB);
  if (xbatch != 1 && xbatch != batch) return fail("xbatch=%d must be 1 (one sample shared by the batch) or batch=%d", xbatch, batch);
  if (nu < 1) return fail("nu=%d: at least one direction is needed", nu);
  if (!u) return fail("null argument");
  for (int b = 0; b < batch; ++b)
    if (dir[b] < -1 || dir[b] >= nu) return fail("dir[%d]=%d outside [-1,%d) (-1: no shift)", b, dir[b], nu);
  if (int r = check_pair(e, src_buf, dst_buf, FOR_FORWARD)) return r;
  Forward f;
  f.stash = false; f.seed = src_buf; f.u = u; f.dir = dir; f.scale = scale; f.xbatch = xbatch;
  return forward_pass(e, x, batch, t, ctx, dst_buf, channels, out, f);
}

int dpb_read_buffer(dpb_engine* e, int buf, int channels, float* out) {
  if (!e || !out) return fail("null argument");
  if (buf < 0 || buf >= (int)e->bufs.size()) return fail("bad buffer %d", buf);
  const Buf& b = e->bufs[buf];
  if (channels < 1 || channels > b.C) return fail("bad channel count");
  int n = b.kind == DPB_BUF_SHARED ? 1 : e->cur_batch;
  if (n < 1) return fail("no primal state to read (dpb_forward invalidates it; run dpb_primal first)");
  return launch_nhwc_to_nchw(e->dtype, e->P(buf), out, n, channels, b.rows, b.C, e->stream);
}

static int jvp_pass(dpb_engine* e, int src, int tap, const float* V, int nt, float* U) {
  if (!e || !V) return fail("null argument");
  const char* flags;
  if (int r = check_pass(e, src, tap, nt, &flags)) return r;
  const Pass ps(e, MODE_TANGENT, tap, src, flags);
  const LaunchSpan span(e);
  e->flops = 0; e->gbytes = 0;
  const Buf& bx = e->bufs[src];
  if (int r = launch_nchw_to_nhwc(e->dtype, V, e->T(src), nt, seed_channels(e, src), bx.rows, bx.C, e->stream)) return r;
  if (e->tstats_bytes && !gn_deterministic()) DPB_CHECK(hipMemsetAsync(e->ws + e->tstats_off, 0, e->tstats_bytes, e->stream));
  const int last = e->producer[tap];
  std::fill(e->skip.begin(), e->skip.end(), 0);
  e->pend.on = false;
  for (int i = e->producer[src] + 1; i <= last; ++i) {
    if (!ps.oact[i] || e->skip[i]) continue;
    if (int r = run_op(e, e->ops[i], ps, nt)) return r;
  }
  if (int r = flush_pending(e)) return r;
  if (!U) return 0;
  const Buf& bt = e->bufs[tap];
  return launch_nhwc_to_nchw(e->dtype, e->T(tap), U, nt, bt.Cv, bt.rows, bt.C, e->stream);
}

int dpb_jvp(dpb_engine* e, int tap, const float* V, int nt, float* U) {
  if (!U) return fail("null argument");
  return jvp_pass(e, e ? e->x_buf : -1, tap, V, nt, U);
}

int dpb_jvp_between(dpb_engine* e, int src_buf, int dst_buf, const float* V, int nt, float* U) {
  if (!e || !U) return fail("null argument");
  return jvp_pass(e, src_buf, dst_buf, V, nt, U);
}

static int vjp_pass(dpb_engine* e, int src, int tap, const float* U, int nt, float* W) {
  if (!e || !W) return fail("null argument");
  const char* flags;
  if (int r = check_pass(e, src, tap, nt, &flags)) return r;
  const Pass ps(e, MODE_ADJOINT, tap, src, flags);
  const LaunchSpan span(e);
  e->flops = 0; e->gbytes = 0;
  const Buf& bt = e->bufs[tap];
  std::fill(e->ginit.begin(), e->ginit.end(), 0);
  for (auto& b : e->bufs) b.g_off = b.g_off0;
  if (U) {
    if (int r = launch_nchw_to_nhwc(e->dtype, U, e->G(tap), nt, bt.Cv, bt.rows, bt.C, e->stream)) return r;
  } else {
    e->bufs[tap].g_off = e->bufs[tap].t_off;
  }
  e->ginit[tap] = 1;
  if (e->tstats_bytes && !gn_deterministic()) DPB_CHECK(hipMemsetAsync(e->ws + e->tstats_off, 0, e->tstats_bytes, e->stream));
  e->pend.on = false;
  for (int i = e->producer[tap]; i > e->producer[src]; --i) {
    const Op& op = e->ops[i];
    if (!ps.oact[i] || !e->ginit[op.d.out]) continue;
    if (int r = run_op(e, op, ps, nt)) return r;
  }
  if (int r = flush_pending(e)) return r;
  if (!e->ginit[src]) {
    for (auto& b : e->bufs) b.g_off = b.g_off0;
    return src == e->x_buf ? fail("tap buffer %d is not connected to x", tap) : fail("dst buffer %d is not connected to source buffer %d", tap, src);
  }
  const Buf& bx = e->bufs[src];
  const int r = launch_nhwc_to_nchw(e->dtype, e->G(src), W, nt, seed_channels(e, src), bx.rows, bx.C, e->stream);
  for (auto& b : e->bufs) b.g_off = b.g_off0;
  return r;
}

int dpb_vjp(dpb_engine* e, int tap, const float* U, int nt, float* W) {
  if (!U) return fail("null argument");
  return vjp_pass(e, e ? e->x_buf : -1, tap, U, nt, W);
}

int dpb_vjp_between(dpb_engine* e, int src_buf, int dst_buf, const float* U, int nt, float* W) {
  if (!e || !U) return fail("null argument");
  return vjp_pass(e, src_buf, dst_buf, U, nt, W);
}

static OrthArgs orth_args(const float* W, const float* Vprev, float* V, float* s, float* conv, void* scratch, size_t scratch_bytes, int k, long N) {
  OrthArgs a;
  a.W = W; a.Vprev = Vprev; a.V = V; a.s = s; a.conv = conv; a.scratch = (double*)scratch; a.scratch_bytes = scratch_bytes; a.k = k; a.N = N;
  return a;
}

int dpb_orth(const float* W, const float* Vprev, float* V, float* s, float* conv, void* scratch, int k, int64_t N, void* stream) {
  if (!W || !Vprev || !V || !s || !conv || !scratch) return fail("null argument");
  return launch_orth(orth_args(W, Vprev, V, s, conv, scratch, orth_scratch_bytes(k, N) , k, N), (hipStream_t)stream);
}

int dpb_orth_checked(const float* W, const float* Vprev, float* V, float* s, float* conv, void* scratch, size_t scratch_bytes, int k, int64_t N,
                     void* stream) {
  if (!W || !Vprev || !V || !s || !conv || !scratch) return fail("null argument");
  if (k < 1 || k > ORTH_MAX_RANK || N < 1) return fail("dpb_orth: k=%d outside [1,%d] or N=%lld < 1", k, ORTH_MAX_RANK, (long long)N);
  const size_t need = orth_scratch_bytes(k, N);
  if (scratch_bytes < need) return fail("dpb_orth: scratch of %zu bytes, dpb_orth_scratch_bytes(%d, %lld) = %zu", scratch_bytes, k, (long long)N, need);
  return launch_orth(orth_args(W, Vprev, V, s, conv, scratch, scratch_bytes, k, N), (hipStream_t)stream);
}

size_t dpb_orth_scratch_bytes(int k, int64_t N) { return (k < 1 || k > ORTH_MAX_RANK || N < 1) ? 0 : orth_scratch_bytes(k, N); }

size_t dpb_pca_scratch_bytes(int q, int64_t N, int64_t D) { return pca_scratch_bytes(q, N, D); }

int dpb_pca_lowrank(const float* H, int64_t N, int64_t D, const float* R, int q, int niter, float* u, float* s, void* scratch,
                    size_t scratch_bytes, void* stream) {
  if (!H || !R || !u || !s || (!scratch && scratch_bytes)) return fail("dpb_pca_lowrank: null argument");
  return launch_pca_lowrank(H, N, D, R, q, niter, u, s, scratch, scratch_bytes, (hipStream_t)stream);
}

int dpb_cross_gram(const float* X, const float* Y, double* G, int Ra, int Rb, int64_t N, void* stream) {
  if (!X || !G) return fail("dpb_cross_gram: null argument");
  return launch_cross_gram(X, Y, G, Ra, Rb, N, (hipStream_t)stream);
}

size_t dpb_subspace_angles_scratch_bytes(int Ba, int Bb, int k, int64_t N) { return subspace_angles_scratch_bytes(Ba, Bb, k, N); }

int dpb_subspace_angles(const float* A, const float* B, int Ba, int Bb, int k, int64_t N, float* theta, float* dist, void* scratch, size_t scratch_bytes,
                        void* stream) {
  if (!A || !theta || !dist || !scratch) return fail("dpb_subspace_angles: null argument");
  return launch_subspace_angles(A, B, Ba, Bb, k, N, theta, dist, scratch, scratch_bytes, (hipStream_t)stream);
}

size_t dpb_transport_scratch_bytes(int D, int P, int k, int64_t N_h, int64_t N_x) { return transport_scratch_bytes(D, P, k, N_h, N_x); }

int dpb_transport_directions(const float* u_src, const float* u_dst, const float* vT_dst, const int32_t* pcs, int P, int D, int k, int64_t N_h,
                             int64_t N_x, float* vk, float* coef, float* coef_norm, void* scratch, size_t scratch_bytes, void* stream) {
  if (!u_src || !u_dst || !vT_dst || !pcs || !vk || !coef || !coef_norm || !scratch) return fail("dpb_transport_directions: null argument");
  return launch_transport_directions(u_src, u_dst, vT_dst, pcs, P, D, k, N_h, N_x, vk, coef, coef_norm, scratch, scratch_bytes, (hipStream_t)stream);
}

size_t dpb_frechet_scratch_bytes(int B, int k, int64_t N, int max_iter) { return frechet_scratch_bytes(B, k, N, max_iter); }

int dpb_frechet_init(const float* X, int B, int k, int64_t N, int init, int max_iter, void* scratch, size_t scratch_bytes, void* stream) {
  if (!X || !scratch) return fail("dpb_frechet_init: null argument");
  return launch_frechet_init(X, B, k, N, max_iter, init, scratch, scratch_bytes, (hipStream_t)stream);
}

int dpb_frechet_iterate(int n_iter, double step, double tol, int B, int k, int64_t N, int max_iter, void* scratch, size_t scratch_bytes, void* stream) {
  if (!scratch) return fail("dpb_frechet_iterate: null argument");
  return launch_frechet_iterate(B, k, N, max_iter, n_iter, step, tol, scratch, scratch_bytes, (hipStream_t)stream);
}

int dpb_frechet_finish(const float* X, float* Y, float* weight, float* theta, double* info, int B, int k, int64_t N, int max_iter, void* scratch,
                       size_t scratch_bytes, void* stream) {
  if (!X || !Y || !weight || !theta || !info || !scratch) return fail("dpb_frechet_finish: null argument");
  return launch_frechet_finish(X, B, k, N, max_iter, Y, weight, theta, info, scratch, scratch_bytes, (hipStream_t)stream);
}

size_t dpb_linear_assignment_scratch_bytes(int B, int k) { return linear_assignment_scratch_bytes(B, k); }

int dpb_linear_assignment(const double* cost, int B, int k, int32_t* col_of_row, double* total, void* scratch, size_t scratch_bytes, void* stream) {
  if (!cost || !col_of_row || !total || !scratch) return fail("dpb_linear_assignment: null argument");
  return launch_linear_assignment(cost, B, k, col_of_row, total, scratch, scratch_bytes, (hipStream_t)stream);
}

size_t dpb_matched_mean_scratch_bytes(int B, int k, int64_t N) { return matched_mean_scratch_bytes(B, k, N); }

int dpb_matched_mean(const float* X, int B, int k, int64_t N, const float* anchor, int init, int distance, float* Y, int32_t* perm, int32_t* sign,
                     double* info, void* scratch, size_t scratch_bytes, void* stream) {
  if (!X || !Y || !perm || !sign || !info || !scratch) return fail("dpb_matched_mean: null argument");
  return launch_matched_mean(X, B, k, N, anchor, init, distance, Y, perm, sign, info, scratch, scratch_bytes, (hipStream_t)stream);
}

int dpb_row_sumsq(const float* X, int64_t rows, int64_t N, double* ss, void* stream) {
// ... 110 lines not shown
      if (r) { if (g) (void)hipGraphDestroy(g); return r; }
      DPB_CHECK(ce);
      DPB_CHECK(hipGraphInstantiate(&e->gexec, g, nullptr, nullptr, 0));
      (void)hipGraphDestroy(g);
      e->gkey = key;
    }
    for (; it < n_iters; ++it) {
      DPB_CHECK(hipGraphLaunch(e->gexec, e->stream));
      replayed += e->g_launches; fl += e->g_flops; gb += e->g_bytes;
    }
  }
  for (; it < n_iters; ++it)
    if (int r = body(it == n_iters - 1)) return r;
  e->n_launch = launch_count - at + replayed; e->flops = fl; e->gbytes = gb;
  return 0;
}

int dpb_pullback_iterate(dpb_engine* e, int tap, float* V, float* U, float* s, float* conv, int k, int n_iters) {
  if (!e || !V || !U || !s || !conv) return fail("null argument");
  if (k < 1 || k > ORTH_MAX_RANK) return fail("pca_rank k=%d outside [1,%d]", k, ORTH_MAX_RANK);
  const int B = e->cur_batch;
  if (int r = check_tap(e, tap, k * (B > 0 ? B : 1))) return r;
  return iterate_pass(e, e->x_buf, tap, V, U, s, conv, k, n_iters, (float*)(e->ws + e->pbW), e->ws + e->orth, e->orth_stride);
}

static size_t between_scratch_bytes(const dpb_engine* e, int src, int k, int batch) {
  const long N = (long)e->bufs[src].rows * seed_channels(e, src);
  return align_up((size_t)batch * k * N * sizeof(float)) + (size_t)batch * align_up(orth_scratch_bytes(k, N));
}

size_t dpb_pullback_scratch_bytes(const dpb_engine* e, int src_buf, int k) {
  if (!e || k < 1 || k > ORTH_MAX_RANK || src_buf < 0 || src_buf >= (int)e->bufs.size() || e->bufs[src_buf].kind != DPB_BUF_ACT) return 0;
  return between_scratch_bytes(e, src_buf, k, e->maxB);
}

int dpb_pullback_iterate_between(dpb_engine* e, int src_buf, int dst_buf, float* V, float* U, float* s, float* conv, int k, int n_iters, void* scratch,
                                 size_t scratch_bytes) {
  if (!e || !V || !U || !s || !conv || !scratch) return fail("null argument");
  if (k < 1 || k > ORTH_MAX_RANK) return fail("pca_rank k=%d outside [1,%d]", k, ORTH_MAX_RANK);
  const int B = e->cur_batch;
  if (int r = check_pass(e, src_buf, dst_buf, k * (B > 0 ? B : 1))) return r;
  if ((uintptr_t)scratch % 256) return fail("scratch must be 256-byte aligned");
  const size_t need = between_scratch_bytes(e, src_buf, k, B);
  if (scratch_bytes < need) return fail("scratch of %zu bytes, the iteration needs %zu (dpb_pullback_scratch_bytes)", scratch_bytes, need);
  const long N = (long)e->bufs[src_buf].rows * seed_channels(e, src_buf);
  const size_t wbytes = align_up((size_t)B * k * N * sizeof(float));
  return iterate_pass(e, src_buf, dst_buf, V, U, s, conv, k, n_iters, (float*)scratch, (char*)scratch + wbytes, align_up(orth_scratch_bytes(k, N)));
}

int dpb_ddim_step(const float* x, const float* eps, float* out, float* x0, int64_t n, float a_t, float a_next, void* stream) {
  if (!x || !eps || !out) return fail("null argument");
  return launch_ddim_step(x, eps, out, x0, n, a_t, a_next, (hipStream_t)stream);
}

int dpb_embed_tokens(const int32_t* ids, const void* tok_table, const void* pos_table, int dtype, float* out, int batch, int tokens,
                     int channels, int vocab, void* stream) {
  if (!ids || !tok_table || !pos_table || !out) return fail("null argument");
  if (dtype != DPB_F32 && dtype != DPB_BF16 && dtype != DPB_F16) return fail("bad dtype %d", dtype);
  return launch_embed_tokens(dtype, ids, tok_table, pos_table, out, batch, tokens, channels, vocab, (hipStream_t)stream);
}

int dpb_lincomb(const float* x, const float* y, const float* z, float* out, int64_t n, float a, float b, float c, void* stream) {
  if (!x || !y || !out) return fail("null argument");
  return launch_lincomb(x, y, z, out, n, a, b, c, (hipStream_t)stream);
}

int dpb_engine_profile(dpb_engine* e, int enable) {
  if (!e) return fail("null engine");
  for (auto& p : e->prof) { (void)hipEventDestroy(p.a); (void)hipEventDestroy(p.b); }
  e->prof.clear();
  e->profiling = enable != 0;
  if (e->profiling) {
    hipEvent_t a, b;
    DPB_CHECK(hipEventCreate(&a));
    DPB_CHECK(hipEventCreate(&b));
    float best = 1e9f;
    for (int i = 0; i < 24; ++i) {
      DPB_CHECK(hipEventRecord(a, e->stream));
      if (int r = launch_axpy(e->dtype, e->ws + e->zeros, e->ws + e->zeros, 64, 0, e->stream)) return r;
      DPB_CHECK(hipEventRecord(b, e->stream));
      DPB_CHECK(hipEventSynchronize(b));
      float ms = 0;
      DPB_CHECK(hipEventElapsedTime(&ms, a, b));
      if (i >= 4) best = ms < best ? ms : best;
    }
    (void)hipEventDestroy(a);
    (void)hipEventDestroy(b);
    best -= 1.5e-3f;
    if (best < 0.f) best = 0.f;
    e->prof_overhead_ms = best < 1e8f ? best : 0.f;
  }
  return 0;
}

int dpb_engine_profile_dump(dpb_engine* e, const char* path) {
  if (!e || !path) return fail("null argument");
  DPB_CHECK(hipStreamSynchronize(e->stream));
  FILE* f = fopen(path, "w");
  if (!f) return fail("cannot open %s", path);
  fprintf(f, "idx,big,gather,M,N,K,Z,us,tflops,raw_us,bracket_overhead_us\n");
  int i = 0;
  for (auto& p : e->prof) {
    float raw = 0;
    (void)hipEventElapsedTime(&raw, p.a, p.b);
    const float ms = raw > e->prof_overhead_ms ? raw - e->prof_overhead_ms : 0.f;
    fprintf(f, "%d,%d,%d,%d,%d,%d,%d,%.2f,%.2f,%.2f,%.2f\n", i++, p.big, p.gather, p.M, p.N, p.K, p.Z, ms * 1e3, ms > 0 ? p.flops / (ms * 1e-3) / 1e12 : 0.0,
            raw * 1e3, e->prof_overhead_ms * 1e3);
  }
  fclose(f);
  return 0;
}

int dpb_engine_profile_read(dpb_engine* e, int big_tile, int64_t* count, double* total_ms, double* flops) {
  if (!e || !count || !total_ms || !flops) return fail("null argument");
  DPB_CHECK(hipStreamSynchronize(e->stream));
  *count = 0; *total_ms = 0; *flops = 0;
  const bool raw = big_tile >= 1000;
  if (raw) big_tile -= 1000;
  if (big_tile < 0 || big_tile > 12) return fail("dpb_engine_profile_read: kind must be 0..12 or 1000..1012");
  for (auto& p : e->prof) {
    if (p.big != big_tile) continue;
    float ms = 0;
    DPB_CHECK(hipEventElapsedTime(&ms, p.a, p.b));
    if (!raw) ms = ms > e->prof_overhead_ms ? ms - e->prof_overhead_ms : 0.f;
    *count += 1; *total_ms += ms; *flops += p.flops;
  }
  return 0;
}

int dpb_engine_profile_overhead(const dpb_engine* e, double* bracket_overhead_ms) {
  if (!e || !bracket_overhead_ms) return fail("null argument");
  *bracket_overhead_ms = e->prof_overhead_ms;
  return 0;
}

int dpb_debug_set(const char* key, int value) {
  static int tile = 0, splitk = 0, kch = 0;
  if (!key) return fail("null key");
  if (!strcmp(key, "gemm_tile")) tile = value;
  else if (!strcmp(key, "gemm_splitk")) splitk = value;
  else if (!strcmp(key, "gemm_kch")) kch = value;
  else if (!strcmp(key, "gemm_dma_auto")) { gemm_debug_dma_auto(value); return 0; }
  else if (!strcmp(key, "gemm_order")) { gemm_debug_order(value); return 0; }
  else if (!strcmp(key, "p8")) { gemm_debug_p8(value); return 0; }
  else if (!strcmp(key, "halo_loop")) { conv_halo_debug_loop(value); return 0; }
  else if (!strcmp(key, "wres")) { gemm_debug_wres(value); return 0; }
  else if (!strcmp(key, "gn_deterministic")) { gn_debug_deterministic(value); return 0; }
  else if (!strcmp(key, "graph_iterate")) { g_graph_iterate = value; return 0; }
  else if (!strcmp(key, "attn_shared")) { attn_debug_shared(value); return 0; }
  else if (!strcmp(key, "lazy_reduce")) { g_lazy_reduce = value; return 0; }
  else if (!strcmp(key, "ln_fuse")) { g_ln_fuse = value; return 0; }
  else if (!strcmp(key, "cross_primal")) { g_cross_primal = value; return 0; }
  else if (!strcmp(key, "cross_fold")) { g_cross_fold = value; return 0; }
  else if (!strcmp(key, "geglu_fwd")) { g_geglu_fwd = value; return 0; }
  else if (!strcmp(key, "iter_alias")) { g_iter_alias = value; return 0; }
  else return fail("unknown debug key %s", key);
  gemm_debug_set(tile, splitk, kch);
  return 0;
}

int dpb_debug_gemm_plan(int dtype, int M, int N, int K, int conv_hw, int conv_cin, int epilogue, int64_t slab_bytes, int* kind, int* tile,
                        int* splitk) {
  if (!kind || !tile || !splitk) return fail("null argument");
  if (dtype != DPB_F32 && dtype != DPB_BF16 && dtype != DPB_F16) return fail("bad dtype %d", dtype);
  static char dummy[16];
  GemmArgs a;
  a.M = M; a.N = N; a.K = K; a.lda = K; a.ldb = K; a.ldc = N;
  a.zeros = dummy;
  if (slab_bytes > 0) { a.slab = (float*)dummy; a.slab_bytes = (size_t)slab_bytes; }
  a.epi = epilogue;
  if (epilogue == EPI_XATT) { a.xatt_p = (const float*)dummy; a.xatt_h = N / 128; a.xatt_lk = 77; a.ldc = 80 * a.xatt_h; a.C = dummy; }
  if (conv_hw > 0) {
    if (conv_cin <= 0 || K != 9 * conv_cin || M % (conv_hw * conv_hw)) return fail("conv plan: K must be 9*cin and M whole images");
    a.gather = GATHER_CONV; a.H = a.W = a.Ho = a.Wo = conv_hw; a.Cin = conv_cin; a.KS = 3; a.stride = 1; a.pad = 1; a.lda = conv_cin;
  }
  const GemmPlan pl = gemm_plan(dtype, a);
  if (!pl.row) return -1;
  *kind = pl.kind; *tile = pl.tile; *splitk = pl.splitk;
  return 0;
}

int dpb_debug_cross_fold(const dpb_engine* e, int index, int64_t* info) {
  if (!e || !info) return fail("null argument");
  int n = 0;
  for (size_t i = 0; i < e->ops.size(); ++i) {
    if (e->ops[i].d.kind != DPB_OP_ATTENTION || !e->plans[e->ops[i].attn].fold_ok) continue;
    if (n++ != index) continue;
    const AttnPlan& p = e->plans[e->ops[i].attn];
    const int64_t v[12] = {(int64_t)i, p.fold_live, p.heads * p.d, p.heads, p.Lq, p.Lk, (int64_t)p.Gt, (int64_t)p.Gk, (int64_t)p.F, (int64_t)p.Fk, (int64_t)p.Pf, (int64_t)e->S1};
    memcpy(info, v, sizeof(v));
    return 0;
  }
  return fail("dpb_debug_cross_fold: the tape has %d layers that can take the folded route, index %d", n, index);
}

int dpb_engine_stats(const dpb_engine* e, int64_t* launches, double* gemm_flops, double* gemm_bytes) {
  if (!e) return fail("null engine");
  if (launches) *launches = e->n_launch;
  if (gemm_flops) *gemm_flops = e->flops;
  if (gemm_bytes) *gemm_bytes = e->gbytes;
  return 0;
}

}
```

diffusion_pullback_amd/csrc/epilogue.h:

```cpp
#pragma once
#include "kernels.h"

#ifndef DPB_SLAB_FULL_LINES
#define DPB_SLAB_FULL_LINES 1
#endif
#ifndef DPB_SLAB_STORE
#define DPB_SLAB_STORE 0
#endif

namespace dpb {

__device__ inline float seg8_sum(float v) {
  v += __shfl_xor(v, 4, 64);
  v += __shfl_xor(v, 2, 64);
  v += __shfl_xor(v, 1, 64);
  return v;
}
template <int WN> struct LnPre { uint4 xr[2][2 * WN / 64], rres[2][2 * WN / 64]; };
template <int FL, int WN, int EPI>
__device__ __forceinline__ void ln_prefetch(const GemmArgs& p, const bf16* C, const bf16* R, int wave, int lane, int mrow0_block, LnPre<WN>& q) {
  constexpr int NI = 2 * WN / 64;
  const int wy = wave >> 1, rg = lane >> 3, l = lane & 7;
#pragma unroll
  for (int ps = 0; ps < 2; ++ps) {
    const int m = min(mrow0_block + wy * 32 + (wave & 1) * 16 + ps * 8 + rg, p.M - 1);
    const int smp = m / p.rows_per_sample, lr = m - smp * p.rows_per_sample;
    const long prow = (long)(smp / p.epi_kps) * p.rows_per_sample + lr;
#pragma unroll
    for (int i = 0; i < NI; ++i) {
      const int n = (l + 8 * i) * 8;
      q.xr[ps][i] = *reinterpret_cast<const uint4*>((const bf16*)p.ln_x + prow * p.N + n);
      q.rres[ps][i] = make_uint4(0, 0, 0, 0);
      if (EPI == EPI_LN_TAN && R) q.rres[ps][i] = *reinterpret_cast<const uint4*>(R + (long)m * p.ldr + n);
      if (EPI == EPI_LN_ADJ && p.accumulate) q.rres[ps][i] = *reinterpret_cast<const uint4*>(C + (long)m * p.ldc + n);
    }
  }
}

template <int FL, int WN, int SLD, int EPI>
__device__ __forceinline__ void epilogue_ln(const GemmArgs& p, bf16* C, const bf16* R, const float* smem_f, int wave, int lane, int mrow0_block, const LnPre<WN>& q) {
  constexpr int NI = 2 * WN / 64;
  static_assert(2 * WN % 64 == 0, "N = 2 WN must be a multiple of 64");
  const OutBuf ob2 = out_buf(EPI == EPI_LN_TAN ? p.C2 : (void*)C, (long)p.M * p.ldc * 2);
  const int wy = wave >> 1, rg = lane >> 3, l = lane & 7;
  const float inv_c = 1.f / (float)p.N;
  float gam[NI][8];
#pragma unroll
  for (int i = 0; i < NI; ++i) { Vec<float>::load(p.ln_gamma + (l + 8 * i) * 8, gam[i]); Vec<float>::load(p.ln_gamma + (l + 8 * i) * 8 + 4, gam[i] + 4); }
#pragma unroll
  for (int ps = 0; ps < 2; ++ps) {
    const int row = (wave & 1) * 16 + ps * 8 + rg;
    const int m = mrow0_block + wy * 32 + row;
    const bool live = m < p.M;
    float v[NI][8], x[NI][8];
    float sx = 0.f;
#pragma unroll
    for (int i = 0; i < NI; ++i) {
      const int n = (l + 8 * i) * 8, half = n / WN, cn = n - half * WN;
      const float* sp = smem_f + ((wy * 2 + half) * 32 + row) * SLD + cn;
      Vec<float>::load(sp, v[i]); Vec<float>::load(sp + 4, v[i] + 4);
      H16<FL>::load8(reinterpret_cast<const bf16*>(&q.xr[ps][i]), x[i]);
      if (EPI == EPI_LN_TAN && R) {
        float r8[8];
        H16<FL>::load8(reinterpret_cast<const bf16*>(&q.rres[ps][i]), r8);
#pragma unroll
        for (int e = 0; e < 8; ++e) v[i][e] += r8[e];
      }
      const bf16x8 pk = H16<FL>::pack8(v[i]);
      if (EPI == EPI_LN_TAN && live) *reinterpret_cast<bf16x8*>(C + (long)m * p.ldc + n) = pk;
      H16<FL>::load8(reinterpret_cast<const bf16*>(&pk), v[i]);
#pragma unroll
      for (int e = 0; e < 8; ++e) sx += x[i][e];
    }
    const float mean = seg8_sum(sx) * inv_c;
    float vs = 0.f;
#pragma unroll
    for (int i = 0; i < NI; ++i)
#pragma unroll
      for (int e = 0; e < 8; ++e) { x[i][e] -= mean; vs += x[i][e] * x[i][e]; }
    const float rstd = rsqrtf(seg8_sum(vs) * inv_c + p.ln_eps);
    float s1 = 0.f, s2 = 0.f;
#pragma unroll
    for (int i = 0; i < NI; ++i)
#pragma unroll
      for (int e = 0; e < 8; ++e) {
        if (EPI == EPI_LN_ADJ) v[i][e] *= gam[i][e];
        x[i][e] *= rstd;
        s1 += v[i][e];
        s2 += x[i][e] * v[i][e];
      }
    const float m1 = seg8_sum(s1) * inv_c, m2 = seg8_sum(s2) * inv_c;
    if (!live) continue;
#pragma unroll
    for (int i = 0; i < NI; ++i) {
      const int n = (l + 8 * i) * 8;
      float o[8];
#pragma unroll
      for (int e = 0; e < 8; ++e) {
        const float w = rstd * (v[i][e] - m1 - x[i][e] * m2);
        o[e] = EPI == EPI_LN_TAN ? w * gam[i][e] : w;
      }
      if (EPI == EPI_LN_ADJ && p.accumulate) {
        float old[8];
        H16<FL>::load8(reinterpret_cast<const bf16*>(&q.rres[ps][i]), old);
#pragma unroll
        for (int e = 0; e < 8; ++e) o[e] += old[e];
      }
      store8_at<FL>(ob2, (EPI == EPI_LN_TAN ? (bf16*)p.C2 : C) + (long)m * p.ldc + n, o);
    }
  }
}

template <int FL, int WN, int SLD, int EPI>
__device__ __forceinline__ void epilogue_slab(const GemmArgs& p, bf16* C, const bf16* R, const float* smem_f, int wave, int lane, int mrow0, int n0,
                                     long slab_idx) {
  constexpr int CPR = WN / 8;
  const int wx = wave & 1;
  const float* stage = smem_f + wave * 32 * SLD;
  const OutBuf cb = out_buf(C, (long)p.M * p.ldc * 2);
  if constexpr (EPI == EPI_GEGLU_FWD) {
    const int F2 = p.N;
    constexpr int NIT = WN == 64 ? 2 : 4;
#pragma unroll
    for (int it = 0; it < NIT; ++it) {
      const int item = it * 64 + lane;
      int row, c8, n, ncol;
      const float *pa, *pg;
      if constexpr (WN == 64) {
        const float* sa = smem_f + (wave & ~1) * 32 * SLD;
        row = wx * 16 + item / CPR; c8 = item % CPR;
        n = n0 + c8 * 8; ncol = (n0 >> 1) + c8 * 8;
        pa = sa + row * SLD + c8 * 8; pg = sa + 32 * SLD + row * SLD + c8 * 8;
      } else {
        row = item >> 3; c8 = item & 7;
        n = n0 + wx * WN + c8 * 8; ncol = ((n0 + wx * WN) >> 1) + c8 * 8;
        pa = stage + row * SLD + c8 * 8; pg = pa + 64;
      }
      const int m = mrow0 + row;
      if (m >= p.M || n >= p.N) continue;
      float a8[8], g8[8], o[8];
      Vec<float>::load(pa, a8); Vec<float>::load(pa + 4, a8 + 4);
      Vec<float>::load(pg, g8); Vec<float>::load(pg + 4, g8 + 4);
      if (p.bias) {
        float b8[8];
        Vec<float>::load(p.bias + n, b8); Vec<float>::load(p.bias + n + 4, b8 + 4);
#pragma unroll
        for (int e = 0; e < 8; ++e) a8[e] = p.alpha * a8[e] + b8[e];
        Vec<float>::load(p.bias + n + 64, b8); Vec<float>::load(p.bias + n + 68, b8 + 4);
#pragma unroll
        for (int e = 0; e < 8; ++e) g8[e] = p.alpha * g8[e] + b8[e];
      }
      const bf16x8 ar = H16<FL>::pack8(a8), gr = H16<FL>::pack8(g8);
      H16<FL>::load8(reinterpret_cast<const bf16*>(&ar), a8);
      H16<FL>::load8(reinterpret_cast<const bf16*>(&gr), g8);
#pragma unroll
      for (int e = 0; e < 8; ++e) {
        const float er = erff(g8[e] * 0.70710678118654752f);
        const float g1 = 0.5f * g8[e] * (1.f + er);
        o[e] = a8[e] * g1;
      }
      store8_at<FL>(cb, C + (long)m * p.ldc + ncol, o);
    }
    (void)F2;
    return;
  }
  if constexpr (EPI == EPI_GEGLU_TAN) {
    if constexpr (WN == 64) {
      const float* sa = smem_f + (wave & ~1) * 32 * SLD;
      const float* sg = sa + 32 * SLD;
      const int F2 = p.N;
#pragma unroll
      for (int it = 0; it < 2; ++it) {
        const int item = it * 64 + lane;
        const int row = wx * 16 + item / CPR, c8 = item % CPR;
        const int m = mrow0 + row;
        const int n = n0 + c8 * 8;
        if (m >= p.M || n >= p.N) continue;
        float da[8], dg[8], ap[8], gp[8], o[8];
        Vec<float>::load(sa + row * SLD + c8 * 8, da); Vec<float>::load(sa + row * SLD + c8 * 8 + 4, da + 4);
        Vec<float>::load(sg + row * SLD + c8 * 8, dg); Vec<float>::load(sg + row * SLD + c8 * 8 + 4, dg + 4);
        const int smp = m / p.rows_per_sample, l = m - smp * p.rows_per_sample;
        const bf16* hp = (const bf16*)p.hprim + ((long)(smp / p.epi_kps) * p.rows_per_sample + l) * F2 + n;
        H16<FL>::load8(hp, ap);
        H16<FL>::load8(hp + 64, gp);
#pragma unroll
        for (int e = 0; e < 8; ++e) o[e] = p.alpha * (da[e] * ap[e] + dg[e] * gp[e]);
        store8_at<FL>(cb, C + (long)m * p.ldc + (n0 >> 1) + c8 * 8, o);
      }
    } else if constexpr (WN == 128) {
      const int F2 = p.N;
#pragma unroll
      for (int it = 0; it < 4; ++it) {
        const int item = it * 64 + lane;
        const int row = item >> 3, c8 = item & 7;
        const int m = mrow0 + row;
        const int n = n0 + wx * WN + c8 * 8;
        if (m >= p.M || n >= p.N) continue;
        float da[8], dg[8], ap[8], gp[8], o[8];
        Vec<float>::load(stage + row * SLD + c8 * 8, da); Vec<float>::load(stage + row * SLD + c8 * 8 + 4, da + 4);
        Vec<float>::load(stage + row * SLD + 64 + c8 * 8, dg); Vec<float>::load(stage + row * SLD + 64 + c8 * 8 + 4, dg + 4);
        const int smp = m / p.rows_per_sample, l = m - smp * p.rows_per_sample;
        const bf16* hp = (const bf16*)p.hprim + ((long)(smp / p.epi_kps) * p.rows_per_sample + l) * F2 + n;
        H16<FL>::load8(hp, ap);
        H16<FL>::load8(hp + 64, gp);
#pragma unroll
        for (int e = 0; e < 8; ++e) o[e] = p.alpha * (da[e] * ap[e] + dg[e] * gp[e]);
        store8_at<FL>(cb, C + (long)m * p.ldc + ((n0 + wx * WN) >> 1) + c8 * 8, o);
      }
    }
    return;
  }
  if constexpr (EPI == EPI_XATT) {
    static_assert(WN == 64, "EPI_XATT: 128-column tiles in the wave-pair form");
    const float* s0 = smem_f + (wave & ~1) * 32 * SLD;
    const float* s1 = s0 + 32 * SLD;
    const int Hh = p.xatt_h, h = n0 >> 7, c8 = lane & 7, rg = lane >> 3;
    const bool hi = c8 < 2;
    float pa[2][8], pb[2][8];
#pragma unroll
    for (int it = 0; it < 2; ++it) {
      const int mc = min(mrow0 + wx * 16 + it * 8 + rg, p.M - 1);
      const int smp = mc / p.rows_per_sample, l = mc - smp * p.rows_per_sample;
      const float* pp = p.xatt_p + (((long)(smp / p.epi_kps) * p.rows_per_sample + l) * Hh + h) * 80 + c8 * 8;
      Vec<float>::load(pp, pa[it]); Vec<float>::load(pp + 4, pa[it] + 4);
#pragma unroll
      for (int e = 0; e < 8; ++e) pb[it][e] = 0.f;
      if (hi) { Vec<float>::load(pp + 64, pb[it]); Vec<float>::load(pp + 68, pb[it] + 4); }
    }
#pragma unroll
    for (int it = 0; it < 2; ++it) {
      const int row = wx * 16 + it * 8 + rg, m = mrow0 + row;
      float a8[8], b8[8];
      Vec<float>::load(s0 + row * SLD + c8 * 8, a8); Vec<float>::load(s0 + row * SLD + c8 * 8 + 4, a8 + 4);
#pragma unroll
      for (int e = 0; e < 8; ++e) b8[e] = 0.f;
      if (hi) { Vec<float>::load(s1 + row * SLD + c8 * 8, b8); Vec<float>::load(s1 + row * SLD + c8 * 8 + 4, b8 + 4); }
      float ds = 0.f;
#pragma unroll
      for (int e = 0; e < 8; ++e) {
        if (c8 * 8 + e >= p.xatt_lk) a8[e] = 0.f;
        if (64 + c8 * 8 + e >= p.xatt_lk) b8[e] = 0.f;
        ds += pa[it][e] * a8[e] + pb[it][e] * b8[e];
      }
      const float delta = seg8_sum(ds);
      if (m >= p.M) continue;
#pragma unroll
      for (int e = 0; e < 8; ++e) {
        a8[e] = c8 * 8 + e < p.xatt_lk ? pa[it][e] * (a8[e] - delta) : 0.f;
        b8[e] = 64 + c8 * 8 + e < p.xatt_lk ? pb[it][e] * (b8[e] - delta) : 0.f;
      }
      bf16* cp = C + (long)m * p.ldc + h * 80 + c8 * 8;
      store8_at<FL>(cb, cp, a8);
      if (hi) store8_at<FL>(cb, cp + 64, b8);
    }
    return;
  }
  constexpr int ITEMS = 32 * CPR / 64, RPI = 64 / CPR;
  static_assert(64 % CPR == 0, "a lane keeps its column across items");
  const int c8 = lane % CPR, r0 = lane / CPR;
  const int n = n0 + wx * WN + c8 * 8;
  if (DPB_SLAB_FULL_LINES && EPI == EPI_PLAIN && p.splitk > 1 && !(p.N & 3)) {
// ... 143 lines not shown
```

diffusion_pullback_amd/csrc/gemm.hip:

```cpp
#include <cstdio>
#include <vector>

#include "kernels.h"

namespace dpb {


template <typename T> struct V8;
template <> struct V8<float> {
  __device__ static inline void load(const float* p, float* o) { Vec<float>::load(p, o); Vec<float>::load(p + 4, o + 4); }
  __device__ static inline void store(float* p, const float* o) { Vec<float>::store(p, o); Vec<float>::store(p + 4, o + 4); }
};
template <> struct V8<bf16> {
  __device__ static inline void load(const bf16* p, float* o) { Vec<bf16>::load(p, o); }
  __device__ static inline void store(bf16* p, const float* o) { Vec<bf16>::store(p, o); }
};
template <> struct V8<f16> {
  __device__ static inline void load(const f16* p, float* o) { Vec<f16>::load(p, o); }
  __device__ static inline void store(f16* p, const float* o) { Vec<f16>::store(p, o); }
};
template <typename T> struct FlavourOf { static constexpr int FL = 0; };
template <> struct FlavourOf<f16> { static constexpr int FL = 1; };

template <typename T, int BM, int BN, int KCH, int GATHER>
// ... 345 lines not shown
      if (p.bias) {
#pragma unroll
        for (int e = 0; e < 8; ++e) v[e] += bias8[e];
      }
      if (p.rowbias) {
#pragma unroll
        for (int e = 0; e < 8; ++e) v[e] += rb8[e];
      }
      if (p.R) {
#pragma unroll
        for (int e = 0; e < 8; ++e) v[e] += r8[e];
      }
      if (p.accumulate) {
#pragma unroll
        for (int e = 0; e < 8; ++e) v[e] += old8[e];
      }
      V8<T>::store(cp, v);
    }
    return;
  }
  const long total = MN * Z;
  for (long idx = (long)blockIdx.x * 256 + threadIdx.x; idx < total; idx += (long)gridDim.x * 256) {
    const int z = (int)(idx / MN);
    const long mn = idx - (long)z * MN;
    const int m = (int)(mn / p.N), n = (int)(mn - (long)m * p.N);
    float acc = 0.f;
    for (int s = 0; s < p.splitk; ++s) acc += p.slab[((long)s * Z + z) * MN + mn];
    const int z1 = z / p.Z2, z2 = z % p.Z2;
    float x = p.alpha * acc;
    if (p.bias) x += p.bias[n];
    if (p.rowbias) x += TT<T>::ld((const T*)p.rowbias + (long)((m / p.rows_per_sample) / p.rowbias_div) * p.ldrb + n);
    if (p.R) x += TT<T>::ld((const T*)p.R + (long)z1 * p.sR1 + (long)z2 * p.sR2 + (long)m * p.ldr + n);
    T* cp = (T*)p.C + (long)z1 * p.sC1 + (long)z2 * p.sC2 + (long)m * p.ldc + n;
    if (p.accumulate) x += TT<T>::ld(cp);
    TT<T>::st(cp, x);
  }
}

static int g_force_tile = 0, g_force_splitk = 0, g_kch = 0, g_dma_auto = 1, g_force_order = -1;
void gemm_debug_order(int o) { g_force_order = o; }
void gemm_debug_set(int tile, int splitk, int kch) { g_force_tile = tile; g_force_splitk = splitk; g_kch = kch; }
void gemm_debug_dma_auto(int on) { g_dma_auto = on; }
static int g_p8 = 1;
void gemm_debug_p8(int on) { g_p8 = on; }
static int g_wres = 1;
void gemm_debug_wres(int on) { g_wres = on; }
void gemm_variant_error(const GemmTile& t, const GemmArgs& a) { set_error("gemm: tile %d has no kernel of this family for gather %d with epilogue %d", t.code, a.gather, a.epi); }
static thread_local GemmArgs* t_pending = nullptr;

static const GemmTile* pick_reg_tile(int dtype, const GemmArgs& a) {
  const GemmTile *small = &kGemmTiles[T_REG64], *big = &kGemmTiles[T_REG128];
  if (g_force_tile) return g_force_tile == big->forced ? big : small;
  if (dtype != DT_F32 || a.A2) return small;
  return gemm_tile_count(*big, a) >= 1024 ? big : small;
}

struct ShapeOverride { int M, N, K, gather, code, split; };
static const std::vector<ShapeOverride>& shape_overrides() {
  static const std::vector<ShapeOverride> v = [] {
    std::vector<ShapeOverride> o;
    const char* e = getenv("DPB_GEMM_OVERRIDE");
    while (e && *e) {
      ShapeOverride r{};
      int used = 0;
      if (sscanf(e, "%dx%dx%d:%d=%d/%d%n", &r.M, &r.N, &r.K, &r.gather, &r.code, &r.split, &used) == 6) o.push_back(r);
      else break;
      e += used;
      if (*e == ',') ++e;
    }
    return o;
  }();
  return v;
}
static const ShapeOverride* find_override(const GemmArgs& a) {
  for (const auto& r : shape_overrides())
    if (r.M == a.M && r.N == a.N && r.K == a.K && r.gather == a.gather && a.Z1 * a.Z2 == 1) return &r;
  return nullptr;
}
static int forced_code(const GemmArgs& a) {
  const ShapeOverride* ov = g_force_tile ? nullptr : find_override(a);
  return ov ? ov->code : g_force_tile;
}
static long forced_splitk(const GemmArgs& a) {
  const ShapeOverride* ov = g_force_splitk ? nullptr : find_override(a);
  return g_force_splitk ? g_force_splitk : ov ? ov->split : 0;
}

static int wres_wants(int dtype, const GemmArgs& a) {
  static const int wres_env = getenv("DPB_WRES") ? atoi(getenv("DPB_WRES")) : 1;
  static const int min_m = getenv("DPB_WRES_MIN_M") ? atoi(getenv("DPB_WRES_MIN_M")) : 49152;
  if (!wres_env || !g_wres || !gemm_wres_supported(dtype, a)) return 0;
  return a.M >= (a.N == 320 ? (long)min_m : 3L * min_m);
}

static int p8_wants(int dtype, const GemmArgs& a) {
  static const int p8_env = getenv("DPB_P8") ? atoi(getenv("DPB_P8")) : 1;
  if (!p8_env || !g_p8 || dtype == DT_F32 || a.A2 || !a.zeros || a.Z1 * a.Z2 != 1 || a.K % 8 || !gemm_p8_fits32(a)) return 0;
  if (a.gather != GATHER_NONE && (a.Cin % 64 || a.epi != EPI_PLAIN)) return 0;
  if (a.epi == EPI_LN_TAN || a.epi == EPI_LN_ADJ || (a.epi != EPI_PLAIN && a.N % 256)) return 0;
  const long t256 = (long)((a.M + 255) / 256) * ((a.N + 255) / 256), rounds = (t256 + 255) / 256;
  if (t256 < 160 || (a.K < 640 && !(a.K >= 320 && t256 >= 4096))) return 0;
  const double fill = (double)a.M * a.N / ((double)t256 * 65536.0);
  if (fill < ((t256 >= 2048 && a.gather == GATHER_NONE) ? 0.6 : 0.75)) return 0;
  if (a.gather != GATHER_NONE && fill < 0.9 && t256 > 512) return 0;
  return t256 >= 1024 || (double)t256 >= 0.58 * 256.0 * (double)rounds;
}

static bool wants_halo(int dtype, const GemmArgs& a) {
  static const int halo_env = getenv("DPB_CONV_HALO") ? atoi(getenv("DPB_CONV_HALO")) : 1;
  const int force = forced_code(a);
  const bool forced = force == kGemmTiles[T_HALO].forced;
  const bool want = forced || (halo_env && force == 0 && g_dma_auto && !p8_wants(dtype, a));
  return want && dtype != DT_F32 && conv_halo_supported(a) && (a.H * a.W >= 256 || forced);
}

static const GemmTile* pick_async_tile(int dtype, const GemmArgs& a) {
  if (dtype == DT_F32 || a.A2 || !a.zeros) return nullptr;
  if (a.epi == EPI_XATT) {
    const GemmTile* f = gemm_tile_forced(forced_code(a));
    if (f && (f->flags & TILE_XATT)) return f;
    return &kGemmTiles[gemm_tile_count(kGemmTiles[T_R64_S2], a) < 256 ? T_R64_HALF : T_R64_S2];
  }
  if (const GemmTile* f = gemm_tile_forced(forced_code(a))) {
    if (f->family == FAM_REG) return nullptr;
    if (f->family != FAM_HALO) {
      const bool takes = gemm_tile_builds(*f, a.gather, a.epi) && !((f->flags & TILE_CIN64) && a.gather != GATHER_NONE && a.Cin % 64) &&
                         (f->family != FAM_WRES || gemm_wres_supported(dtype, a));
      return (takes || f->substitute == T_NONE) ? f : &kGemmTiles[f->substitute];
    }
  }
  const long t128 = gemm_tile_count(kGemmTiles[T_R64_S2], a), t64 = gemm_tile_count(kGemmTiles[T_R32_64], a);
  if (!g_dma_auto || a.K < 256) return nullptr;
  if (wres_wants(dtype, a)) return &kGemmTiles[T_WRES];
  if (p8_wants(dtype, a)) return &kGemmTiles[T_P8];
  static const int big_env = getenv("DPB_TILE256") ? atoi(getenv("DPB_TILE256")) : 1;
  if (big_env && a.gather == GATHER_NONE && a.K >= 640 && a.Z1 * a.Z2 == 1) {
    const long t256 = (long)((a.M + 255) / 256) * ((a.N + 255) / 256);
    if (t256 >= 160 && (double)t256 * 65536.0 <= 1.07 * (double)a.M * a.N) return &kGemmTiles[T_R64_256];
  }
  static const int half_env = getenv("DPB_HALF_TILE") ? atoi(getenv("DPB_HALF_TILE")) : 3;
  static const int half_kmin = getenv("DPB_HALF_KMIN") ? atoi(getenv("DPB_HALF_KMIN")) : 256;
  if ((half_env & 1) && a.gather == GATHER_NONE && a.epi == EPI_PLAIN && a.Z1 * a.Z2 == 1 && a.K >= half_kmin && a.K <= 4096 && t128 >= 128 && t128 < 256) return &kGemmTiles[T_R64_HALF];
  if ((half_env & 2) && a.epi == EPI_PLAIN && a.gather != GATHER_UPCONV && a.Z1 * a.Z2 == 1 && a.K >= 2048 && t128 < 128 && (a.M % 128) && (a.M % 128) <= 64) return &kGemmTiles[T_R64_HALF];
  if (a.K >= 512 && (t128 >= 200 || a.K >= 2048)) return &kGemmTiles[T_R64_S2];
  if (t128 >= 400) return &kGemmTiles[(a.K % 64 == 0 && t128 <= 1280) ? T_R64_S2 : T_R32_S3];
  if (a.K >= 2048 && t128 >= 64) return &kGemmTiles[T_R32_TALL];
  if (t64 >= 256 || (t64 >= 96 && a.K >= 1024)) return &kGemmTiles[T_R32_64];
  return nullptr;
}

int gemm_epi_supported(int dtype, const GemmArgs& a) {
  if (a.epi == EPI_LN_TAN || a.epi == EPI_LN_ADJ) {
    const GemmTile& ln = kGemmTiles[T_R64_LN];
    return dtype != DT_F32 && a.Z1 * a.Z2 == 1 && a.gather == GATHER_NONE && a.N == ln.bn && a.ldc == ln.bn && a.M >= ln.bm && a.K % 64 == 0 && a.zeros &&
           a.ln_x && a.ln_gamma && !a.A2 && !a.bias && !a.rowbias && a.alpha == 1.f && (a.epi == EPI_LN_ADJ || (a.C2 && !a.accumulate)) && (!a.R || a.ldr % 8 == 0);
  }
  if (dtype == DT_F32 || a.Z1 * a.Z2 != 1 || a.gather != GATHER_NONE || a.N % 128 || a.M <= 0) return 0;
  if (a.epi == EPI_XATT)
    return a.xatt_p && a.xatt_h > 0 && a.N == 128 * a.xatt_h && a.ldc == 80 * a.xatt_h && a.xatt_lk > 0 && a.xatt_lk <= 80 && a.K % 8 == 0 && a.zeros && !a.A2 &&
           !a.bias && !a.rowbias && !a.R && !a.accumulate && a.alpha == 1.f && a.rows_per_sample > 0 && a.epi_kps > 0 && !((uintptr_t)a.C & 15);
  if (a.epi == EPI_GEGLU_ADJ && a.N % 64) return 0;
  const GemmTile* t = pick_async_tile(dtype, a);
  if (!t || !(t->flags & TILE_GEGLU) || t->bn % 128) return 0;
  return !(t->flags & TILE_EPI_N256) || a.N % 256 == 0;
}

static int gemm_kch(const GemmArgs&) { return g_kch ? g_kch : 4; }

static long pick_splitk(int dtype, const GemmArgs& a, const GemmTile& t) {
  const long tiles = gemm_tile_count(t, a);
  if (t.family == FAM_HALO) {
    const int nch = a.Cin / 64;
    long best = 1L << 60, s = 1;
    for (long c = 1; c <= nch; ++c) {
      const long cost = ((tiles * c + 255) / 256) * ((nch + c - 1) / c + 2);
      if (cost < best) { best = cost; s = c; }
    }
    return s;
  }
  if (t.family == FAM_REG) {
    const int nk = (a.K + (dtype == DT_F32 ? 4 : 8) * gemm_kch(a) - 1) / ((dtype == DT_F32 ? 4 : 8) * gemm_kch(a));
    if (t.bm == 128 || tiles >= 768 || nk < 32) return 1;
    const long s = std::min<long>((1024 + tiles - 1) / tiles, nk / 8);
    return std::min<long>(s, 32);
  }
  if (t.flags & TILE_NOSPLIT) return 1;
  const int nk = (a.K + 31) / 32;
  if (t.family != FAM_RING32) {
    static const long target = getenv("DPB_SPLITK_TARGET") ? atol(getenv("DPB_SPLITK_TARGET")) : 448;
    if (tiles >= 192) return (tiles < 256 && nk >= 128) ? 2 : 1;
    return std::min<long>(std::max<long>(1, (target + tiles / 2) / tiles), std::max(1, nk / 16));
  }
  if (tiles >= 256 || nk < 64) return 1;
  const long s = std::min<long>((1024 + tiles - 1) / tiles, nk / 12);
  return std::min<long>(s, 32);
}

GemmPlan gemm_plan(int dtype, const GemmArgs& a) {
  const GemmTile* t;
  if (a.M <= 0 || a.N <= 0 || a.K <= 0) { set_error("gemm: empty problem M=%d N=%d K=%d", a.M, a.N, a.K); return GemmPlan{-1, 0, 1, nullptr}; }
  if (wants_halo(dtype, a)) {
    t = &kGemmTiles[T_HALO];
  } else if (a.epi != EPI_PLAIN && !gemm_epi_supported(dtype, a)) {
    set_error("gemm: fused epilogue %d requested for a launch no ring kernel with 128-column tiles takes (M=%d N=%d K=%d)", a.epi, a.M, a.N, a.K);
    return GemmPlan{-1, 0, 1, nullptr};
  } else if (a.epi == EPI_LN_TAN || a.epi == EPI_LN_ADJ) {
    t = &kGemmTiles[T_R64_LN];
  } else {
    t = pick_async_tile(dtype, a);
    if (!t) t = pick_reg_tile(dtype, a);
  }
  long s = 1;
  if (a.slab && (a.epi == EPI_PLAIN || t->family == FAM_HALO) && !(t->flags & TILE_NOSLAB) && !(t->family == FAM_REG && a.A2)) {
    s = forced_splitk(a);
    if (!s) s = pick_splitk(dtype, a, *t);
    const int kstep = t->family == FAM_REG ? (dtype == DT_F32 ? 4 : 8) * gemm_kch(a) : 32;
    s = std::min<long>(s, t->family == FAM_HALO ? a.Cin / 64 : (a.K + kstep - 1) / kstep);
    const long per = (long)a.M * a.N * a.Z1 * a.Z2 * 4;
    if (s > 1 && s * per > (long)a.slab_bytes) s = (long)a.slab_bytes / per;
  }
  return GemmPlan{gemm_plan_kind(*t), t->code, (int)std::max<long>(s, 1), t};
}

template <typename T, int BM, int BN, int KCH>
static void launch_reg_t(const GemmArgs& a, dim3 grid, hipStream_t st) {
  switch (a.gather) {
    case GATHER_NONE: DPB_LAUNCH((gemm_kernel<T, BM, BN, KCH, GATHER_NONE>), grid, dim3(256), 0, st, a); break;
    case GATHER_CONV: DPB_LAUNCH((gemm_kernel<T, BM, BN, KCH, GATHER_CONV>), grid, dim3(256), 0, st, a); break;
    case GATHER_CONVT: DPB_LAUNCH((gemm_kernel<T, BM, BN, KCH, GATHER_CONVT>), grid, dim3(256), 0, st, a); break;
    default: DPB_LAUNCH((gemm_kernel<T, BM, BN, KCH, GATHER_UPCONV>), grid, dim3(256), 0, st, a); break;
  }
}

template <typename T>
static int launch_t(int dtype, GemmArgs a, hipStream_t st, const GemmPlan* plan) {
  constexpr int CH = TT<T>::CH;
  if (a.K % CH || a.lda % CH || a.ldb % CH || (a.gather != GATHER_NONE && a.Cin % CH)) {
    set_error("gemm: K=%d lda=%d ldb=%d Cin=%d must be multiples of %d", a.K, a.lda, a.ldb, a.Cin, CH);
    return -1;
  }
  if (a.A2 && (a.K2 % CH || a.lda2 % CH || a.ldb2 % CH || a.gather != GATHER_NONE)) {
    set_error("gemm: second operand pair misaligned or combined with a gather");
    return -1;
  }
  a.vec_ok = !(a.ldc & 7) && !(a.sC1 & 7) && !(a.sC2 & 7) && (!a.R || (!(a.ldr & 7) && !(a.sR1 & 7) && !(a.sR2 & 7))) &&
             (!a.rowbias || !(a.N & 7)) && !((uintptr_t)a.C & 15) && !((uintptr_t)a.R & 15) && !((uintptr_t)a.bias & 15);
  const int Z = a.Z1 * a.Z2;
  {
    const double ua = (double)a.M * (a.gather == GATHER_NONE ? a.K : a.Cin), ub = (double)a.N * a.K;
    static const int env_order = getenv("DPB_GEMM_ORDER") ? atoi(getenv("DPB_GEMM_ORDER")) : -1;
    const int force = g_force_order >= 0 ? g_force_order : env_order;
    a.order = force >= 0 ? force : (ub > ua ? 1 : 0);
  }
  const GemmPlan pl = plan ? *plan : gemm_plan(dtype, a);
  if (!pl.row) return -1;
  const GemmTile& t = *pl.row;
  a.splitk = pl.splitk;
  int r = 0;
  switch (t.family) {
    case FAM_HALO: r = launch_conv_halo(a, st); break;
    case FAM_WRES: r = launch_gemm_wres(a, st); break;
    case FAM_P8: r = launch_gemm_p8(a, t.code, st); break;
    case FAM_RING64: r = launch_gemm_ring64(a, t, st); break;
    case FAM_RING32: r = launch_gemm_dma(a, t, st); break;
    default:
      if (t.bm == 128) launch_reg_t<T, 128, 128, 4>(a, gemm_tile_grid(t, a), st);
      else if (gemm_kch(a) == 8) launch_reg_t<T, 64, 64, 8>(a, gemm_tile_grid(t, a), st);
      else launch_reg_t<T, 64, 64, 4>(a, gemm_tile_grid(t, a), st);
  }
  if (r) return r;
  if (a.splitk > 1) {
    const bool plain = Z == 1 && a.alpha == 1.f && !a.bias && !a.rowbias && !a.accumulate && a.ldc == a.N && a.vec_ok && !(a.N & 7) && a.epi == EPI_PLAIN;
    if (t_pending && plain) {
      *t_pending = a;
    } else {
      long total = (long)a.M * a.N * Z / 4;
      unsigned g = (unsigned)std::max<long>(1, std::min<long>((total + 255) / 256, 4096));
      DPB_LAUNCH((splitk_reduce_kernel<T>), dim3(g), dim3(256), 0, st, a);
    }
  }
  DPB_CHECK(hipGetLastError());
  return 0;
}

int launch_gemm_reduce(int dtype, const GemmArgs& a, hipStream_t st) {
  if (a.splitk <= 1) return 0;
  const long total = (long)a.M * a.N * a.Z1 * a.Z2 / 4;
  const unsigned g = (unsigned)std::max<long>(1, std::min<long>((total + 255) / 256, 4096));
  DPB_DISPATCH_STMT(dtype, T, DPB_LAUNCH((splitk_reduce_kernel<T>), dim3(g), dim3(256), 0, st, a));
  DPB_CHECK(hipGetLastError());
  return 0;
}

int launch_gemm(int dtype, const GemmArgs& a, hipStream_t st, GemmArgs* pending, const GemmPlan* plan) {
  GemmArgs b = a;
  b.fl = dtype == DT_F16;
  if (pending) pending->splitk = 1;
  t_pending = pending;
  static const int trace = getenv("DPB_GEMM_TRACE") ? atoi(getenv("DPB_GEMM_TRACE")) : 0;
  GemmPlan traced;
  if (trace) {
    if (!plan) { traced = gemm_plan(dtype, b); plan = &traced; }
    fprintf(stderr, "gemm M=%d N=%d K=%d Z=%d gather=%d epi=%d lda=%d ldb=%d ldc=%d ldr=%d acc=%d R=%d bias=%d rowbias=%d tile=%d splitk=%d\n", b.M, b.N, b.K, b.Z1 * b.Z2, b.gather,
            b.epi, b.lda, b.ldb, b.ldc, b.ldr, b.accumulate, b.R != nullptr, b.bias != nullptr, b.rowbias != nullptr, plan->tile, plan->splitk);
    fflush(stderr);
  }
  const int r = DPB_DISPATCH_T(dtype, T, launch_t<T>(dtype, b, st, plan));
  if (trace && hipStreamSynchronize(st) != hipSuccess) fprintf(stderr, "gemm: the launch above failed\n");
  t_pending = nullptr;
  return r;
}

}
```

diffusion_pullback_amd/csrc/kernels.h:

```cpp
#pragma once
#include <algorithm>
#include <type_traits>
#include <utility>

#include "common.h"

namespace dpb {

enum { GATHER_NONE = 0, GATHER_CONV = 1, GATHER_CONVT = 2, GATHER_UPCONV = 3 };
enum { EPI_PLAIN = 0, EPI_GEGLU_TAN = 1, EPI_GEGLU_ADJ = 2, EPI_LN_TAN = 3, EPI_LN_ADJ = 4, EPI_GEGLU_FWD = 5, EPI_XATT = 6 };
struct GemmArgs {
  const void* A = nullptr; const void* B = nullptr; void* C = nullptr; const void* R = nullptr;
  const float* bias = nullptr;
  const void* rowbias = nullptr;
  int rows_per_sample = 1, rowbias_div = 1;
  int ldrb = 0;
  int M = 0, N = 0, K = 0;
  int lda = 0, ldb = 0, ldc = 0, ldr = 0;
  int Z1 = 1, Z2 = 1;
  long sA1 = 0, sA2 = 0, sB1 = 0, sB2 = 0, sC1 = 0, sC2 = 0, sR1 = 0, sR2 = 0;
  int divA = 1, divB = 1;
  float alpha = 1.f;
  int accumulate = 0;
  int gather = GATHER_NONE;
  int H = 0, W = 0, Cin = 0, Ho = 0, Wo = 0, KS = 1, stride = 1, pad = 0;
  const void* A2 = nullptr; const void* B2 = nullptr;
  int K2 = 0, lda2 = 0, ldb2 = 0, divA2 = 1, divB2 = 1;
  long sA21 = 0, sA22 = 0, sB21 = 0, sB22 = 0;
  float* slab = nullptr; size_t slab_bytes = 0;
  const void* zeros = nullptr;
  int splitk = 1, vec_ok = 0;
  int epi = EPI_PLAIN, epi_kps = 1;
  const void* hprim = nullptr;
  const void* ln_x = nullptr; const float* ln_gamma = nullptr; float ln_eps = 1e-5f; void* C2 = nullptr;
  const float* xatt_p = nullptr; int xatt_h = 0, xatt_lk = 0;
  int fl = 0;
  int order = 0;
};
enum GemmFamily { FAM_REG = 0, FAM_RING32, FAM_RING64, FAM_P8, FAM_WRES, FAM_HALO };
enum : unsigned {
  TILE_CONV = 1,
  TILE_UPCONV = 2,
  TILE_CIN64 = 4,
  TILE_GEGLU = 8,
  TILE_LN = 16,
  TILE_EPI_N256 = 32,
  TILE_NOSPLIT = 64,
  TILE_NOSLAB = 128,
  TILE_XATT = 256,
};
enum GemmTileId { T_REG64 = 0, T_REG128, T_R32_S4, T_R32_S3, T_R32_S2, T_R32_TALL, T_R32_64, T_R32_64B, T_R64_S3, T_R64_TALL, T_R64_S4, T_R64_S2, T_R64_TALL8,
                  T_R64_TALL8_S2, T_R64_256, T_R64_LN, T_R64_HALF, T_R64_HALF_S2, T_R64_HALFN, T_P8, T_WRES, T_HALO, GEMM_TILES, T_NONE = -1 };
struct GemmTile {
  int family;
  int code;
  int forced;
  int bm, bn, stages, waves;
  int kind;
  unsigned flags;
  int substitute;
};
constexpr unsigned TILE_ANY = TILE_CONV | TILE_UPCONV;
inline constexpr GemmTile kGemmTiles[GEMM_TILES] = {
    {FAM_REG,      64,  64,    64,  64,  0, 4,    0,    TILE_ANY,                                                      T_NONE},
    {FAM_REG,      128, 128,   128, 128, 0, 4,    1,    TILE_ANY,                                                      T_NONE},
    {FAM_RING32,   128, 129,   128, 128, 4, 4,    2,    TILE_ANY | TILE_GEGLU,                                         T_NONE},
    {FAM_RING32,   130, 131,   128, 128, 3, 4,    2,    TILE_ANY | TILE_GEGLU,                                         T_NONE},
    {FAM_RING32,   132, 133,   128, 128, 2, 4,    2,    TILE_ANY | TILE_GEGLU,                                         T_NONE},
    {FAM_RING32,   256, 257,   256, 128, 3, 4,    2,    TILE_ANY | TILE_GEGLU,                                         T_NONE},
    {FAM_RING32,   64,  65,    64,  64,  4, 4,    3,    TILE_ANY | TILE_GEGLU,                                         T_NONE},
    {FAM_RING32,   66,  67,    64,  64,  4, 4,    3,    TILE_ANY | TILE_GEGLU,                                         T_NONE},
    {FAM_RING64,   512, 512,   128, 128, 3, 4,    4,    TILE_ANY | TILE_GEGLU,                                         T_NONE},
    {FAM_RING64,   513, 513,   256, 128, 3, 4,    4,    TILE_ANY | TILE_GEGLU,                                         T_NONE},
    {FAM_RING64,   514, 514,   128, 128, 4, 4,    4,    TILE_ANY | TILE_GEGLU,                                         T_NONE},
    {FAM_RING64,   515, 515,   128, 128, 2, 4,    4,    TILE_ANY | TILE_GEGLU | TILE_XATT,                                      T_NONE},
    {FAM_RING64,   516, 516,   256, 128, 3, 8,    4,    TILE_ANY | TILE_GEGLU,                                         T_NONE},
    {FAM_RING64,   517, 517,   256, 128, 2, 8,    4,    TILE_ANY | TILE_GEGLU,                                         T_NONE},
    {FAM_RING64,   518, 518,   256, 256, 2, 8,    6,    TILE_GEGLU | TILE_EPI_N256 | TILE_NOSPLIT,                     T_R64_S2},
    {FAM_RING64,   520, 0,     128, 320, 2, 4,    4,    TILE_LN | TILE_NOSLAB,                                         T_NONE},
    {FAM_RING64,   521, 521,   64,  128, 3, 4,    4,    TILE_CONV | TILE_XATT,                                         T_R64_S2},
    {FAM_RING64,   522, 522,   64,  128, 2, 4,    4,    0,                                                             T_R64_S2},
    {FAM_RING64,   523, 523,   128, 64,  3, 4,    4,    0,                                                             T_R64_S2},
    {FAM_P8,       530, 530,   256, 256, 2, 8,    11,   TILE_ANY | TILE_CIN64 | TILE_GEGLU | TILE_EPI_N256 | TILE_NOSPLIT, T_R64_S2},
    {FAM_WRES,     540, 540,   32,  320, 0, 5,    12,   TILE_NOSLAB,                                                   T_R64_S2},
    {FAM_HALO,     600, 600,   256, 128, 0, 8,    5,    TILE_CONV | TILE_CIN64,                                        T_NONE},
};
constexpr const GemmTile* gemm_tile_forced(int forced) {
  for (const GemmTile& t : kGemmTiles)
    if (forced && t.forced == forced) return &t;
  return nullptr;
}
constexpr int gemm_plan_kind(const GemmTile& t) { return t.family == FAM_REG ? (t.bm == 128) : t.family == FAM_HALO ? 3 : 2; }
constexpr bool gemm_tile_builds(const GemmTile& t, int gather, int epi) {
  if (gather == GATHER_UPCONV ? !(t.flags & TILE_UPCONV) : (gather != GATHER_NONE && !(t.flags & TILE_CONV))) return false;
  if (epi == EPI_PLAIN) return !(t.flags & TILE_LN);
  if (gather != GATHER_NONE) return false;
  if (epi == EPI_XATT) return (t.flags & TILE_XATT) != 0;
  return (t.flags & ((epi == EPI_LN_TAN || epi == EPI_LN_ADJ) ? TILE_LN : TILE_GEGLU)) != 0;
}
inline long gemm_tile_count(const GemmTile& t, const GemmArgs& a) { return (long)((a.M + t.bm - 1) / t.bm) * ((a.N + t.bn - 1) / t.bn) * a.Z1 * a.Z2; }
inline dim3 gemm_tile_grid(const GemmTile& t, const GemmArgs& a) { return dim3(((a.M + t.bm - 1) / t.bm) * ((a.N + t.bn - 1) / t.bn), a.Z1 * a.Z2, a.splitk > 1 ? a.splitk : 1); }
template <int V> using GemmTag = std::integral_constant<int, V>;
template <int... Vs, typename F>
int gemm_tag_switch(int v, F&& f) {
  int r = -1;
  (void)((v == Vs && ((r = f(GemmTag<Vs>{})), true)) || ...);
  return r;
}
void gemm_variant_error(const GemmTile& t, const GemmArgs& a);
template <int FAM, typename F, int... Is>
int gemm_family_launch(const GemmArgs& a, const GemmTile& t, F&& launch, std::integer_sequence<int, Is...>) {
  const int r = gemm_tag_switch<Is...>((int)(&t - kGemmTiles), [&](auto row) {
    return gemm_tag_switch<0, 1>(a.fl, [&](auto fl) {
      return gemm_tag_switch<EPI_PLAIN, EPI_GEGLU_TAN, EPI_GEGLU_ADJ, EPI_LN_TAN, EPI_LN_ADJ, EPI_GEGLU_FWD, EPI_XATT>(a.epi, [&](auto epi) {
        return gemm_tag_switch<GATHER_NONE, GATHER_CONV, GATHER_CONVT, GATHER_UPCONV>(a.gather, [&](auto gather) {
          constexpr GemmTile R = kGemmTiles[decltype(row)::value];
          if constexpr (R.family == FAM && gemm_tile_builds(R, decltype(gather)::value, decltype(epi)::value)) { launch(row, fl, epi, gather); return 0; }
          else return -1;
        });
      });
    });
  });
  if (r) gemm_variant_error(t, a);
  return r;
}
using GemmTileSeq = std::make_integer_sequence<int, GEMM_TILES>;

struct GemmPlan { int kind, tile, splitk; const GemmTile* row; };
int launch_gemm(int dtype, const GemmArgs& a, hipStream_t st, GemmArgs* pending = nullptr, const GemmPlan* plan = nullptr);
int launch_gemm_reduce(int dtype, const GemmArgs& pending, hipStream_t st);
GemmPlan gemm_plan(int dtype, const GemmArgs& a);
void gemm_debug_set(int tile, int splitk, int kch);
int launch_gemm_dma(const GemmArgs& a, const GemmTile& t, hipStream_t st);
int launch_gemm_ring64(const GemmArgs& a, const GemmTile& t, hipStream_t st);
bool gemm_p8_fits32(const GemmArgs& a);
int launch_gemm_p8(const GemmArgs& a, int tile, hipStream_t st);
int conv_halo_supported(const GemmArgs& a);
int launch_conv_halo(const GemmArgs& a, hipStream_t st);
void conv_halo_debug_loop(int on);
int gemm_epi_supported(int dtype, const GemmArgs& a);
void gemm_debug_dma_auto(int on);
void gn_debug_deterministic(int on);
int gn_deterministic();
bool gemm_wres_supported(int dtype, const GemmArgs& a);
int launch_gemm_wres(const GemmArgs& a, hipStream_t st);
void gemm_debug_wres(int on);
void gemm_debug_p8(int on);
void gemm_debug_order(int o);

enum { MODE_PRIMAL = 0, MODE_TANGENT = 1, MODE_ADJOINT = 2 };
struct SlabSrc {
  const float* slab = nullptr; int splitk = 0; long MN = 0; int N = 0;
  const void* R = nullptr; int ldr = 0;
  void* store = nullptr;
};
struct GNArgs {
  const void* x = nullptr;
  const void* d = nullptr;
  void* y = nullptr;
  const float* gamma = nullptr; const float* beta = nullptr;
  int astride = 0;
  double* pstats = nullptr;
  double* tstats = nullptr;
  float* part = nullptr;
  size_t part_bytes = 0;
  int* ticket = nullptr;
  int det = 1;
  int red = 0;
  int Bp = 1, NT = 0, kps = 1;
  int HW = 0, C = 0, G = 32;
  float eps = 1e-5f;
  int silu = 0, accumulate = 0;
  SlabSrc src;
};
int launch_groupnorm(int dtype, int mode, const GNArgs& a, hipStream_t st);
constexpr int ADAGN_MAX_OPS = 32;
struct AdaGNTable { const float* gamma[ADAGN_MAX_OPS]; const float* beta[ADAGN_MAX_OPS]; const void* emb[ADAGN_MAX_OPS]; float* og[ADAGN_MAX_OPS]; float* ob[ADAGN_MAX_OPS]; int C[ADAGN_MAX_OPS]; };
struct AdaGNOp { const float* gamma; const float* beta; const void* emb; float* og; float* ob; int C; };
int launch_adagn_affine(int dtype, const AdaGNOp* ops, int nops, long ld, int batch, int per_sample, hipStream_t st);
bool groupnorm_is_one_launch(int dtype, const GNArgs& a);

struct LNArgs {
  const void* x = nullptr; const void* d = nullptr; void* y = nullptr;
  const float* gamma = nullptr; const float* beta = nullptr;
  int rows_per_sample = 0, Bp = 1, NT = 0, kps = 1, C = 0;
  float eps = 1e-5f;
  int accumulate = 0;
  SlabSrc src;
};
int launch_layernorm(int dtype, int mode, const LNArgs& a, hipStream_t st);

int launch_softmax_fwd(int dtype, void* S, long Z, int Lq, int Lk, int ld, int causal, hipStream_t st);
int launch_softmax_jvp(int dtype, const void* P, void* dS, float* D, long Z, int Z2, int kps, int Lq, int Lk, int ld,
                       hipStream_t st);
int launch_softmax_adjT(int dtype, const void* PT, void* gPT, const float* D, long Z, int Z2, int kps, int Lk, int Lq,
                        int ld, hipStream_t st);
int launch_transpose(int dtype, const void* in, void* out, int Z1, int Z2, long s1, long s2, int R, int Ccols, int ldin,
                     int ldout, long outZstride, hipStream_t st);

struct FusedAttnArgs {
  const void *Q = nullptr, *K = nullptr, *V = nullptr, *O = nullptr, *KT = nullptr, *VT = nullptr, *QT = nullptr;
  const float* stats = nullptr;
  float* Drow = nullptr;
  const void *dQ = nullptr, *dK = nullptr, *dV = nullptr, *dVT = nullptr; void* dO = nullptr;
  const void *gO = nullptr, *gOT = nullptr; void *gQ = nullptr, *gK = nullptr, *gV = nullptr;
  int accQ = 0, accK = 0, accV = 0;
  int fl = 0;
  int L = 0, C = 0, Co = 0, H = 0, d = 0, kps = 1;
  float scale = 1.f;
};
int fused_attention_supported(int dtype, int d, int L, int kv_const);
void attn_debug_shared(int bits);
struct CrossAttnArgs {
  const void *Q = nullptr, *K = nullptr, *V = nullptr;
  const void* BT = nullptr;
  const void* X = nullptr; void* Y = nullptr;
  int L = 0, Lk = 0, Lkp = 0, C = 0, Ck = 0, Cx = 0, Cy = 0, H = 0, d = 0, kps = 1, adjoint = 0, accumulate = 0, fl = 0;
  int primal = 0;
  float* Pstash = nullptr;
  float scale = 1.f;
};
int cross_attention_supported(int dtype, int d, int Lq, int Lk, int kv_const);
int launch_attn_cross(const CrossAttnArgs& f, int nt, hipStream_t st);
int attn_adj_route_bits(int d, int L, int kps, int nt);
int attn_jvp_block_waves(int d, int L, int pairs);
int launch_attn_fwd_fused(const FusedAttnArgs& f, int batch, void* O, float* stats, hipStream_t st);
int launch_attn_jvp_fused(const FusedAttnArgs& f, int nt, hipStream_t st);
int launch_attn_adj_fused(const FusedAttnArgs& f, int nt, hipStream_t st);

struct GegluArgs {
  const void* h = nullptr;
  const void* d = nullptr;
  void* y = nullptr;
  int rows_per_sample = 0, Bp = 1, NT = 0, kps = 1, F = 0;
  int accumulate = 0;
  int stash = 1;
  int il = 0;
};
int launch_geglu(int dtype, int mode, const GegluArgs& a, hipStream_t st);
int launch_silu(int dtype, const void* x, void* y, long n, hipStream_t st);
int launch_quick_gelu(int dtype, const void* x, void* y, long n, hipStream_t st);
int launch_gelu(int dtype, const void* x, void* y, long n, hipStream_t st);
int launch_embed_tokens(int dtype, const int* ids, const void* tok, const void* pos, float* out, int batch, int L, int C, int vocab, hipStream_t st);
int launch_axpy(int dtype, const void* x, void* y, long n, int accumulate, hipStream_t st);
int launch_copy_cols(int dtype, const void* src, int lds, int cs0, void* dst, int ldd, int cd0, long rows, int ncols,
                     int accumulate, hipStream_t st);
int launch_zero_cols(int dtype, void* dst, int ldd, int cd0, long rows, int ncols, hipStream_t st);
int launch_nchw_to_nhwc(int dtype, const float* src, void* dst, int n, int C, int HW, int Cpad, hipStream_t st);
int launch_nhwc_to_nchw(int dtype, const void* src, float* dst, int n, int C, int HW, int Cpad, hipStream_t st);
constexpr int SHIFT_MAX_ROWS = 64;
struct ShiftRows { int dir[SHIFT_MAX_ROWS]; float scale[SHIFT_MAX_ROWS]; };
int launch_shift_tap(int dtype, void* h, const float* u, const int* dir, const float* scale, int batch, int bcast, int C, int Cv, long HW,
                     hipStream_t st);
constexpr int REPL_MAX_BUFS = 32;
struct ReplTable { void* p[REPL_MAX_BUFS]; long chunks[REPL_MAX_BUFS]; };
int launch_replicate_rows(void* const* bufs, const size_t* sample_bytes, int nbufs, int batch, hipStream_t st);
int launch_pool2x2_sum(int dtype, const void* in, void* out, int n, int H, int W, int C, int accumulate, hipStream_t st);
int launch_pool2x2(int dtype, const void* in, void* out, int n, int H, int W, int C, float scale, int accumulate, hipStream_t st);
int launch_up2x2(int dtype, const void* in, void* out, int n, int H, int W, int C, float scale, int accumulate, hipStream_t st);

struct OrthArgs {
  const float* W = nullptr;
  const float* Vprev = nullptr;
  float* V = nullptr;
  float* s = nullptr;
  float* conv = nullptr;
  double* scratch = nullptr;
  size_t scratch_bytes = 0;
  int k = 0; long N = 0;
  int batch = 1; long stride_w = 0, stride_v = 0, stride_s = 0, stride_conv = 0; size_t scratch_stride = 0;
};
constexpr int ORTH_MAX_RANK = 128;
int launch_orth(const OrthArgs& a, hipStream_t st);
size_t orth_scratch_bytes(int k, long N);

const char* pca_invalid(int q, long N, long D);
size_t pca_scratch_bytes(int q, long N, long D);
int launch_pca_lowrank(const float* H, long N, long D, const float* R, int q, int niter, float* u, float* s, void* scratch, size_t scratch_bytes,
                       hipStream_t st);

int launch_cross_gram(const float* X, const float* Y, double* G, int Ra, int Rb, long N, hipStream_t st);
size_t subspace_angles_scratch_bytes(long Ba, long Bb, int k, long N);
int launch_subspace_angles(const float* A, const float* B, long Ba, long Bb, int k, long N, float* theta, float* dist, void* scratch, size_t scratch_bytes,
                           hipStream_t st);

void launch_angles_prep(double* Dg, int* flags, int n, int k, hipStream_t st);

constexpr int FRECHET_MAX_RANK = 64;
size_t frechet_scratch_bytes(long B, int k, long N, long max_iter);
int launch_frechet_init(const float* X, long B, int k, long N, long max_iter, int init, void* scratch, size_t scratch_bytes, hipStream_t st);
int launch_frechet_iterate(long B, int k, long N, long max_iter, int n_iter, double step, double tol, void* scratch, size_t scratch_bytes, hipStream_t st);
int launch_frechet_finish(const float* X, long B, int k, long N, long max_iter, float* Y, float* weight, float* theta, double* info, void* scratch,
                          size_t scratch_bytes, hipStream_t st);

constexpr int HUNGARIAN_MAX_RANK = 128;
size_t linear_assignment_scratch_bytes(long B, int k);
int launch_linear_assignment(const double* cost, long B, int k, int32_t* col_of_row, double* total, void* scratch, size_t scratch_bytes, hipStream_t st);
size_t matched_mean_scratch_bytes(long B, int k, long N);
int launch_matched_mean(const float* X, long B, int k, long N, const float* anchor, int init, int distance, float* Y, int32_t* perm, int32_t* sign,
                        double* info, void* scratch, size_t scratch_bytes, hipStream_t st);

size_t transport_scratch_bytes(long D, int P, int k, long Nh, long Nx);
int launch_rowsumsq(const float* X, long rows, long N, double* ss, hipStream_t st);
int launch_transport_directions(const float* u_src, const float* u_dst, const float* vT_dst, const int32_t* pcs, int P, long D, int k, long Nh, long Nx,
                                float* vk, float* coef, float* coef_norm, void* scratch, size_t scratch_bytes, hipStream_t st);

size_t perturb_scratch_bytes(int B, long n);
int launch_perturb_unit(const float* x, const float* noise, uint64_t seed, int64_t first, int B, long n, float norm, float* out, float* noise_out,
                        void* scratch, size_t scratch_bytes, hipStream_t st);

int launch_ddim_step(const float* x, const float* e, float* out, float* x0, long n, float a_t, float a_next, hipStream_t st);
int launch_lincomb(const float* x, const float* y, const float* z, float* out, long n, float a, float b, float c, hipStream_t st);

}
```

diffusion_pullback_amd/csrc/norm.hip:

```cpp
#include "kernels.h"

namespace dpb {

static int g_gn_det = getenv("DPB_GN_DETERMINISTIC") ? atoi(getenv("DPB_GN_DETERMINISTIC")) : 1;
void gn_debug_deterministic(int on) { g_gn_det = on; }
int gn_deterministic() { return g_gn_det; }


template <typename T>
__device__ inline uint4 slab_chunk(const SlabSrc& s, long row, int c0) {
  constexpr int CH = TT<T>::CH;
  float v[CH];
#pragma unroll
  for (int e = 0; e < CH; ++e) v[e] = 0.f;
  const float* sp = s.slab + row * s.N + c0;
  auto ld = [&](int k, float* t) {
    Vec<float>::load(sp + (long)k * s.MN, t);
    if constexpr (CH == 8) Vec<float>::load(sp + (long)k * s.MN + 4, t + 4);
  };
  int k = 0;
  for (; k + 8 <= s.splitk; k += 8) {
    float t[8][CH];
#pragma unroll
    for (int u = 0; u < 8; ++u) ld(k + u, t[u]);
#pragma unroll
    for (int u = 0; u < 8; ++u)
#pragma unroll
      for (int e = 0; e < CH; ++e) v[e] += t[u][e];
  }
  if (k + 4 <= s.splitk) {
    float t[4][CH];
#pragma unroll
    for (int u = 0; u < 4; ++u) ld(k + u, t[u]);
#pragma unroll
    for (int u = 0; u < 4; ++u)
#pragma unroll
      for (int e = 0; e < CH; ++e) v[e] += t[u][e];
    k += 4;
  }
  for (; k < s.splitk; ++k) {
    float t[CH];
    ld(k, t);
#pragma unroll
    for (int e = 0; e < CH; ++e) v[e] += t[e];
  }
  if (s.R) {
    float r[CH];
    Vec<T>::load((const T*)s.R + row * s.ldr + c0, r);
#pragma unroll
    for (int e = 0; e < CH; ++e) v[e] += r[e];
  }
  const uint4 packed = Raw<T>::pack(v);
  if (s.store) *reinterpret_cast<uint4*>((T*)s.store + row * s.N + c0) = packed;
  return packed;
}

template <typename T>
__device__ inline float gn_shift(const GNArgs& a, int b, int g) {
  return TT<T>::ld((const T*)a.x + (long)b * a.HW * a.C + g * (a.C / a.G));
}

template <typename T, int MODE, bool STATS>
__global__ __launch_bounds__(256) void gn_kernel(GNArgs a, int ppb) {
  constexpr int CH = TT<T>::CH;
  const OutBuf yb = out_buf(a.y, (long)max(a.NT, a.Bp) * a.HW * a.C * (long)sizeof(T));
  extern __shared__ float lch[];
  __shared__ float lsum[2 * 256];
  __shared__ double lseg[4][2 * 256];
  const int tid = threadIdx.x;
  const int j = blockIdx.y;
  const int b = (MODE == MODE_PRIMAL) ? j : j / a.kps;
  const int cols = a.C / CH;
  const int cw = cols < 256 ? cols : 256;
  const int rpi = 256 / cw;
  const int r = tid / cw, c0 = tid % cw;
  const int ncp = (cols + cw - 1) / cw;
  const int cpg = a.C / a.G;
  const int p0 = blockIdx.x * ppb;
  const int p1 = min(p0 + ppb, a.HW);
  const double inv_n = 1.0 / ((double)a.HW * cpg);
  if (STATS && !a.det) {
    for (int i = tid; i < 2 * a.G; i += 256) lsum[i] = 0.f;
    __syncthreads();
  }
  if (!STATS && a.red) {
    const int nblk = gridDim.x, n2 = 2 * a.G;
    const float* pj = a.part + (long)j * nblk * n2;
    for (int t = tid; t < 4 * n2; t += 256) {
      const int q = t / n2, i = t - q * n2;
      const int b0 = (int)((long)nblk * q / 4), b1 = (int)((long)nblk * (q + 1) / 4);
      double acc = 0.0;
      for (int bb = b0; bb < b1; bb += 32) {
        float v[32];
#pragma unroll
        for (int u = 0; u < 32; ++u) v[u] = pj[(long)min(bb + u, b1 - 1) * n2 + i];
#pragma unroll
        for (int u = 0; u < 32; ++u) v[u] = bb + u < b1 ? v[u] : 0.f;
#pragma unroll
        for (int u = 0; u < 32; ++u) acc += (double)v[u];
      }
      lseg[q][i] = acc;
    }
    __syncthreads();
    for (int i = tid; i < n2; i += 256) {
      const double acc = ((lseg[0][i] + lseg[1][i]) + lseg[2][i]) + lseg[3][i];
      if (MODE == MODE_PRIMAL) lseg[0][i] = acc;
      else lsum[i] = (float)(acc * inv_n);
    }
    __syncthreads();
    if (MODE == MODE_PRIMAL) {
      for (int g = tid; g < a.G; g += 256) {
        const double ms = lseg[0][2 * g] * inv_n;
        double v = lseg[0][2 * g + 1] * inv_n - ms * ms;
        if (v < 0) v = 0;
        const double m = (double)gn_shift<T>(a, j, g) + ms;
        const double rs = 1.0 / sqrt(v + (double)a.eps);
        lsum[2 * g] = (float)m; lsum[2 * g + 1] = (float)rs;
        if (blockIdx.x == 0) { a.pstats[((long)j * a.G + g) * 2] = m; a.pstats[((long)j * a.G + g) * 2 + 1] = rs; }
      }
      __syncthreads();
    }
  }
  if (r < rpi) {
    for (int q = 0; q < ncp; ++q) {
      const int col = c0 + q * cw;
      if (col >= cols) break;
      const int ch0 = col * CH;
      float mean[CH], rstd[CH], gam[CH], bet[CH], m1[CH], m2[CH];
      int grp[CH];
      const float* gp = a.gamma + (long)b * a.astride + ch0;
      const float* bp = a.beta + (long)b * a.astride + ch0;
      Vec<float>::load(gp, gam);
      Vec<float>::load(bp, bet);
      if constexpr (CH == 8) { Vec<float>::load(gp + 4, gam + 4); Vec<float>::load(bp + 4, bet + 4); }
      if (cpg >= CH) {
        const int g0 = ch0 / cpg, g1 = min(g0 + 1, a.G - 1);
        float me[2] = {0.f, 0.f}, rs[2] = {0.f, 0.f}, t1[2] = {0.f, 0.f}, t2[2] = {0.f, 0.f};
        if (MODE == MODE_PRIMAL && !STATS && a.red) {
          me[0] = lsum[2 * g0]; rs[0] = lsum[2 * g0 + 1]; me[1] = lsum[2 * g1]; rs[1] = lsum[2 * g1 + 1];
        } else if (MODE != MODE_PRIMAL || !STATS) {
          me[0] = (float)a.pstats[((long)b * a.G + g0) * 2]; rs[0] = (float)a.pstats[((long)b * a.G + g0) * 2 + 1];
          me[1] = (float)a.pstats[((long)b * a.G + g1) * 2]; rs[1] = (float)a.pstats[((long)b * a.G + g1) * 2 + 1];
        } else {
          me[0] = gn_shift<T>(a, b, g0); me[1] = gn_shift<T>(a, b, g1);
        }
        if (MODE != MODE_PRIMAL && !STATS && a.red) {
          t1[0] = lsum[2 * g0]; t2[0] = lsum[2 * g0 + 1]; t1[1] = lsum[2 * g1]; t2[1] = lsum[2 * g1 + 1];
        } else if (MODE != MODE_PRIMAL && !STATS) {
          t1[0] = (float)(a.tstats[((long)j * a.G + g0) * 2] * inv_n); t2[0] = (float)(a.tstats[((long)j * a.G + g0) * 2 + 1] * inv_n);
          t1[1] = (float)(a.tstats[((long)j * a.G + g1) * 2] * inv_n); t2[1] = (float)(a.tstats[((long)j * a.G + g1) * 2 + 1] * inv_n);
        }
#pragma unroll
        for (int e = 0; e < CH; ++e) {
          const int hi = (ch0 + e) >= (g0 + 1) * cpg ? 1 : 0;
          grp[e] = g0 + hi;
          mean[e] = me[hi]; rstd[e] = rs[hi]; m1[e] = t1[hi]; m2[e] = t2[hi];
        }
      } else {
#pragma unroll
        for (int e = 0; e < CH; ++e) {
          grp[e] = (ch0 + e) / cpg;
          mean[e] = rstd[e] = m1[e] = m2[e] = 0.f;
          if (MODE == MODE_PRIMAL && !STATS && a.red) {
            mean[e] = lsum[2 * grp[e]]; rstd[e] = lsum[2 * grp[e] + 1];
          } else if (MODE != MODE_PRIMAL || !STATS) {
            mean[e] = (float)a.pstats[((long)b * a.G + grp[e]) * 2];
            rstd[e] = (float)a.pstats[((long)b * a.G + grp[e]) * 2 + 1];
          } else {
            mean[e] = gn_shift<T>(a, b, grp[e]);
          }
          if (MODE != MODE_PRIMAL && !STATS && a.red) {
            m1[e] = lsum[2 * grp[e]]; m2[e] = lsum[2 * grp[e] + 1];
          } else if (MODE != MODE_PRIMAL && !STATS) {
            m1[e] = (float)(a.tstats[((long)j * a.G + grp[e]) * 2] * inv_n);
            m2[e] = (float)(a.tstats[((long)j * a.G + grp[e]) * 2 + 1] * inv_n);
          }
        }
      }
      float s1[CH], s2[CH];
#pragma unroll
      for (int e = 0; e < CH; ++e) s1[e] = s2[e] = 0.f;
      for (int p = p0 + r; p < p1; p += rpi) {
        float x[CH], d[CH], o[CH];
        Vec<T>::load((const T*)a.x + ((long)b * a.HW + p) * a.C + ch0, x);
        if (MODE != MODE_PRIMAL) Vec<T>::load((const T*)a.d + ((long)j * a.HW + p) * a.C + ch0, d);
#pragma unroll
        for (int e = 0; e < CH; ++e) {
          if (MODE == MODE_PRIMAL) {
            if (STATS) {
              const float xs = x[e] - mean[e];
              s1[e] += xs;
              s2[e] += xs * xs;
            } else {
              float y = (x[e] - mean[e]) * rstd[e] * gam[e] + bet[e];
              o[e] = a.silu ? silu_(y) : y;
            }
          } else {
            float xh = (x[e] - mean[e]) * rstd[e];
            float y = gam[e] * xh + bet[e];
            float act = a.silu ? dsilu_(y) : 1.f;
            float v = (MODE == MODE_TANGENT) ? d[e] : gam[e] * act * d[e];
            if (STATS) {
              s1[e] += v;
              s2[e] += xh * v;
            } else {
              float w = rstd[e] * (v - m1[e] - xh * m2[e]);
// ... 255 lines not shown
  const float* pj = a.part + (long)j * nblk * n2;
  if (tid < SEG * n2) {
    const int q = tid / n2, i = tid - q * n2;
    const int b0 = (int)((long)nblk * q / SEG), b1 = (int)((long)nblk * (q + 1) / SEG);
    double acc = 0.0;
    for (int bb = b0; bb < b1; bb += 32) {
      float v[32];
#pragma unroll
      for (int u = 0; u < 32; ++u) v[u] = pj[(long)min(bb + u, b1 - 1) * n2 + i];
#pragma unroll
      for (int u = 0; u < 32; ++u) acc += bb + u < b1 ? (double)v[u] : 0.0;
    }
    lseg[q * n2 + i] = acc;
  }
  __syncthreads();
  auto total = [&](int i) { double t = 0.0; for (int q = 0; q < SEG; ++q) t += lseg[q * n2 + i]; return t; };
  double* dst = (MODE == MODE_PRIMAL) ? a.pstats : a.tstats;
  if (MODE != MODE_PRIMAL) {
    for (int i = tid; i < n2; i += 1024) dst[(long)j * n2 + i] = total(i);
  } else {
    for (int g = tid; g < a.G; g += 1024) {
      const double s1 = total(2 * g), s2 = total(2 * g + 1);
      const double ms = s1 * inv_n;
      double v = s2 * inv_n - ms * ms;
      if (v < 0) v = 0;
      const double m = (double)gn_shift<T>(a, j, g) + ms;
      dst[((long)j * a.G + g) * 2] = m;
      dst[((long)j * a.G + g) * 2 + 1] = 1.0 / sqrt(v + (double)a.eps);
    }
  }
}

template <typename T>
__global__ void gn_finalize(GNArgs a, double* st, int n_groups, double inv_n, double eps) {
  int i = blockIdx.x * blockDim.x + threadIdx.x;
  if (i >= n_groups) return;
  double ms = st[2 * i] * inv_n;
  double v = st[2 * i + 1] * inv_n - ms * ms;
  if (v < 0) v = 0;
  const double m = (double)gn_shift<T>(a, i / a.G, i % a.G) + ms;
  st[2 * i] = m;
  st[2 * i + 1] = 1.0 / sqrt(v + eps);
}

static int gn_two_pass_ppb(int HW, int n) {
  static const long gn_blocks = getenv("DPB_GN_BLOCKS") ? atol(getenv("DPB_GN_BLOCKS")) : 512;
  int ppb = 64;
  while (ppb > 8 && (long)((HW + ppb - 1) / ppb) * n < gn_blocks) ppb >>= 1;
  return ppb;
}

template <typename T, int MODE>
static int gn_launch(const GNArgs& a, hipStream_t st) {
  constexpr int CH = TT<T>::CH;
  if (a.C % CH || a.C % a.G || a.G > 256) { set_error("groupnorm: C=%d G=%d unsupported", a.C, a.G); return -1; }
  const int n = (MODE == MODE_PRIMAL) ? a.Bp : a.NT;
  if (const int gc = gn_fused_groups(a.C, a.G, a.HW, CH, (int)sizeof(T))) {
    const int cpc = gc * (a.C / a.G) / CH, ppi = 512 / cpc, sweeps = (a.HW + ppi - 1) / ppi;
    dim3 grid(a.G / gc, n);
    if (sweeps > 4) { set_error("groupnorm: %d sweeps exceed the one-launch kernel's register window", sweeps); return -1; }
    DPB_LAUNCH((gn_fused_kernel<T, MODE, 4>), grid, dim3(512), 0, st, a, gc);
    DPB_CHECK(hipGetLastError());
    return 0;
  }
  if (a.src.slab) { set_error("groupnorm: split-K slab input is taken by the one-launch kernel only"); return -1; }
  const int ppb = gn_two_pass_ppb(a.HW, n);
  dim3 grid((a.HW + ppb - 1) / ppb, n);
  size_t lds = 0;
  if (a.det) {
    const int cols = a.C / CH, cw = cols < 256 ? cols : 256, rpi = 256 / cw;
    lds = (size_t)rpi * a.C * 2 * sizeof(float);
    if (!a.part || (size_t)grid.x * n * 2 * a.G * sizeof(float) > a.part_bytes) {
      set_error("groupnorm: statistics scratch missing or too small (%u blocks x %d x %d groups)", grid.x, n, a.G);
      return -1;
    }
    if (lds > 48 * 1024) { set_error("groupnorm: C=%d needs %zu bytes of LDS for the ordered reduction", a.C, lds); return -1; }
  }
  GNArgs b = a;
  b.red = a.det && (int)grid.x <= GN_RED_MAX;
  DPB_LAUNCH((gn_kernel<T, MODE, true>), grid, dim3(256), lds, st, b, ppb);
  if (a.det && !b.red) DPB_LAUNCH((gn_reduce_kernel<T, MODE>), dim3(n), dim3(1024), 0, st, b, (int)grid.x);
  if (MODE == MODE_PRIMAL && !a.det) {
    int ng = a.Bp * a.G;
    DPB_LAUNCH(gn_finalize<T>, dim3((ng + 255) / 256), dim3(256), 0, st, a, a.pstats, ng, 1.0 / ((double)a.HW * (a.C / a.G)), (double)a.eps);
  }
  DPB_LAUNCH((gn_kernel<T, MODE, false>), grid, dim3(256), 0, st, b, ppb);
  DPB_CHECK(hipGetLastError());
  return 0;
}

bool groupnorm_is_one_launch(int dtype, const GNArgs& a) {
  return gn_fused_groups(a.C, a.G, a.HW, dt_chunk(dtype), dtype == DT_F32 ? 4 : 2) != 0;
}

template <typename T>
__global__ __launch_bounds__(256) void adagn_affine_kernel(AdaGNTable t, long ld, int per_sample) {
  const int i = blockIdx.y, b = blockIdx.z, C = t.C[i];
  const T* e = (const T*)t.emb[i] + (per_sample ? (long)b * ld : 0);
  for (int c = blockIdx.x * 256 + threadIdx.x; c < C; c += gridDim.x * 256) {
    const float s = 1.f + TT<T>::ld(e + c), h = TT<T>::ld(e + C + c);
    t.og[i][(long)b * C + c] = t.gamma[i][c] * s;
    t.ob[i][(long)b * C + c] = t.beta[i][c] * s + h;
  }
}
int launch_adagn_affine(int dtype, const AdaGNOp* ops, int nops, long ld, int batch, int per_sample, hipStream_t st) {
  if (batch < 1) { set_error("adagn_affine: batch=%d", batch); return -1; }
  for (int i0 = 0; i0 < nops; i0 += ADAGN_MAX_OPS) {
    AdaGNTable t;
    const int n = std::min(ADAGN_MAX_OPS, nops - i0);
    int cmax = 1;
    for (int i = 0; i < n; ++i) {
      const AdaGNOp& o = ops[i0 + i];
      if (!o.gamma || !o.beta || !o.emb || !o.og || !o.ob || o.C < 1) { set_error("adagn_affine: op %d of the table is incomplete", i0 + i); return -1; }
      t.gamma[i] = o.gamma; t.beta[i] = o.beta; t.emb[i] = o.emb; t.og[i] = o.og; t.ob[i] = o.ob; t.C[i] = o.C;
      cmax = std::max(cmax, o.C);
    }
    for (int i = n; i < ADAGN_MAX_OPS; ++i) { t.gamma[i] = t.beta[i] = nullptr; t.emb[i] = nullptr; t.og[i] = t.ob[i] = nullptr; t.C[i] = 0; }
    DPB_DISPATCH_STMT(dtype, T, DPB_LAUNCH((adagn_affine_kernel<T>), dim3((cmax + 255) / 256, n, batch), dim3(256), 0, st, t, ld, per_sample));
    DPB_CHECK(hipGetLastError());
  }
  return 0;
}

int launch_groupnorm(int dtype, int mode, const GNArgs& a, hipStream_t st) {
  if (mode == MODE_PRIMAL) return DPB_DISPATCH_T(dtype, T, (gn_launch<T, MODE_PRIMAL>(a, st)));
  if (mode == MODE_TANGENT) return DPB_DISPATCH_T(dtype, T, (gn_launch<T, MODE_TANGENT>(a, st)));
  return DPB_DISPATCH_T(dtype, T, (gn_launch<T, MODE_ADJOINT>(a, st)));
}

template <typename T, int MODE, int MAXI>
__global__ __launch_bounds__(256) void ln_kernel(LNArgs a, long nrows) {
  constexpr int CH = TT<T>::CH;
  const OutBuf yb = out_buf(a.y, nrows * a.C * (long)sizeof(T));
  const int lane = threadIdx.x & 63;
  const long row = (long)blockIdx.x * 4 + (threadIdx.x >> 6);
  if (row >= nrows) return;
  const int nch = a.C / CH;
  long prow = row;
  if (MODE != MODE_PRIMAL) {
    long j = row / a.rows_per_sample, l = row - j * a.rows_per_sample;
    prow = (j / a.kps) * a.rows_per_sample + l;
  }
  const T* xp = (const T*)a.x + prow * a.C;
  float x[MAXI][CH];
  float v[MAXI][CH];
  float s = 0.f;
#pragma unroll
  for (int i = 0; i < MAXI; ++i) {
    int c = lane + i * 64;
    if (c < nch) {
      Vec<T>::load(xp + c * CH, x[i]);
      if (MODE != MODE_PRIMAL) {
        if (a.src.slab) Raw<T>::unpack(slab_chunk<T>(a.src, row, c * CH), v[i]);
        else Vec<T>::load((const T*)a.d + row * a.C + c * CH, v[i]);
      }
#pragma unroll
      for (int e = 0; e < CH; ++e) s += x[i][e];
    }
  }
  const float inv_c = 1.f / a.C;
  const float mean = wave_sum(s) * inv_c;
  float vs = 0.f;
#pragma unroll
  for (int i = 0; i < MAXI; ++i) {
    int c = lane + i * 64;
    if (c < nch) {
#pragma unroll
      for (int e = 0; e < CH; ++e) {
        x[i][e] -= mean;
        vs += x[i][e] * x[i][e];
      }
    }
  }
  const float rstd = rsqrtf(wave_sum(vs) * inv_c + a.eps);
  if (MODE == MODE_PRIMAL) {
    T* yp = (T*)a.y + row * a.C;
#pragma unroll
    for (int i = 0; i < MAXI; ++i) {
      int c = lane + i * 64;
      if (c < nch) {
        float o[CH];
#pragma unroll
        for (int e = 0; e < CH; ++e) o[e] = x[i][e] * rstd * a.gamma[c * CH + e] + a.beta[c * CH + e];
        vec_store_at<T>(yb, yp + c * CH, o);
      }
    }
    return;
  }
  float s1 = 0.f, s2 = 0.f;
#pragma unroll
  for (int i = 0; i < MAXI; ++i) {
    int c = lane + i * 64;
    if (c < nch) {
#pragma unroll
      for (int e = 0; e < CH; ++e) {
        if (MODE == MODE_ADJOINT) v[i][e] *= a.gamma[c * CH + e];
        x[i][e] *= rstd;
        s1 += v[i][e];
        s2 += x[i][e] * v[i][e];
      }
    }
  }
  const float m1 = wave_sum(s1) * inv_c, m2 = wave_sum(s2) * inv_c;
  T* yp = (T*)a.y + row * a.C;
#pragma unroll
  for (int i = 0; i < MAXI; ++i) {
    int c = lane + i * 64;
    if (c < nch) {
      float o[CH];
#pragma unroll
      for (int e = 0; e < CH; ++e) {
        float w = rstd * (v[i][e] - m1 - x[i][e] * m2);
        o[e] = (MODE == MODE_TANGENT) ? w * a.gamma[c * CH + e] : w;
      }
      if (a.accumulate) {
        float old[CH];
        Vec<T>::load(yp + c * CH, old);
#pragma unroll
        for (int e = 0; e < CH; ++e) o[e] += old[e];
      }
      vec_store_at<T>(yb, yp + c * CH, o);
    }
  }
}

template <int LPR>
__device__ inline float seg_sum(float v) {
#pragma unroll
  for (int o = LPR >> 1; o > 0; o >>= 1) v += __shfl_xor(v, o, 64);
  return v;
}
template <typename T, int MODE, int LPR, int NI>
__global__ __launch_bounds__(256) void ln_rows_kernel(LNArgs a, long nrows) {
  constexpr int CH = TT<T>::CH, RPW = 64 / LPR;
  const OutBuf yb = out_buf(a.y, nrows * a.C * (long)sizeof(T));
  const int lane = threadIdx.x & 63, l = lane % LPR;
  const long row = ((long)blockIdx.x * 4 + (threadIdx.x >> 6)) * RPW + lane / LPR;
  const bool live = row < nrows;
  const long r = live ? row : nrows - 1;
  long prow = r;
  if (MODE != MODE_PRIMAL) {
    long j = r / a.rows_per_sample, ll = r - j * a.rows_per_sample;
    prow = (j / a.kps) * a.rows_per_sample + ll;
  }
  const T* xp = (const T*)a.x + prow * a.C;
  float x[NI][CH];
  float v[NI][CH];
  float s = 0.f;
#pragma unroll
  for (int i = 0; i < NI; ++i) {
    const int c = l + i * LPR;
    Vec<T>::load(xp + c * CH, x[i]);
    if (MODE != MODE_PRIMAL) {
      if (a.src.slab) { if (live) Raw<T>::unpack(slab_chunk<T>(a.src, r, c * CH), v[i]); else for (int e = 0; e < CH; ++e) v[i][e] = 0.f; }
      else Vec<T>::load((const T*)a.d + r * a.C + c * CH, v[i]);
    }
#pragma unroll
    for (int e = 0; e < CH; ++e) s += x[i][e];
  }
  const float inv_c = 1.f / a.C;
  const float mean = seg_sum<LPR>(s) * inv_c;
  float vs = 0.f;
#pragma unroll
  for (int i = 0; i < NI; ++i)
#pragma unroll
    for (int e = 0; e < CH; ++e) {
      x[i][e] -= mean;
      vs += x[i][e] * x[i][e];
    }
  const float rstd = rsqrtf(seg_sum<LPR>(vs) * inv_c + a.eps);
  T* yp = (T*)a.y + r * a.C;
  if (MODE == MODE_PRIMAL) {
    if (!live) return;
#pragma unroll
    for (int i = 0; i < NI; ++i) {
      const int c = l + i * LPR;
      float o[CH];
#pragma unroll
      for (int e = 0; e < CH; ++e) o[e] = x[i][e] * rstd * a.gamma[c * CH + e] + a.beta[c * CH + e];
      vec_store_at<T>(yb, yp + c * CH, o);
    }
    return;
  }
  float s1 = 0.f, s2 = 0.f;
#pragma unroll
  for (int i = 0; i < NI; ++i) {
    const int c = l + i * LPR;
#pragma unroll
    for (int e = 0; e < CH; ++e) {
      if (MODE == MODE_ADJOINT) v[i][e] *= a.gamma[c * CH + e];
      x[i][e] *= rstd;
      s1 += v[i][e];
      s2 += x[i][e] * v[i][e];
    }
  }
  const float m1 = seg_sum<LPR>(s1) * inv_c, m2 = seg_sum<LPR>(s2) * inv_c;
  if (!live) return;
#pragma unroll
  for (int i = 0; i < NI; ++i) {
    const int c = l + i * LPR;
    float o[CH];
#pragma unroll
    for (int e = 0; e < CH; ++e) {
      float w = rstd * (v[i][e] - m1 - x[i][e] * m2);
      o[e] = (MODE == MODE_TANGENT) ? w * a.gamma[c * CH + e] : w;
    }
    if (a.accumulate) {
      float old[CH];
      Vec<T>::load(yp + c * CH, old);
#pragma unroll
      for (int e = 0; e < CH; ++e) o[e] += old[e];
    }
    vec_store_at<T>(yb, yp + c * CH, o);
  }
}

template <typename T, int MODE, int LPR>
static bool ln_rows_launch(const LNArgs& a, long nrows, int ni, hipStream_t st) {
  const dim3 grid((unsigned)((nrows + 4 * (64 / LPR) - 1) / (4 * (64 / LPR))));
  if (ni == 3) DPB_LAUNCH((ln_rows_kernel<T, MODE, LPR, 3>), grid, dim3(256), 0, st, a, nrows);
  else if (ni == 5) DPB_LAUNCH((ln_rows_kernel<T, MODE, LPR, 5>), grid, dim3(256), 0, st, a, nrows);
  else return false;
  return true;
}

template <typename T, int MODE>
static int ln_launch(const LNArgs& a, hipStream_t st) {
  constexpr int CH = TT<T>::CH;
  if (a.C % CH || a.C / CH > 5 * 64) { set_error("layernorm: C=%d unsupported", a.C); return -1; }
  long nrows = (long)((MODE == MODE_PRIMAL) ? a.Bp : a.NT) * a.rows_per_sample;
  {
    static const int rows_env = getenv("DPB_LN_ROWS") ? atoi(getenv("DPB_LN_ROWS")) : 1;
    const int nch = a.C / CH;
    bool done = false;
    if (rows_env && nrows > 0) {
      for (int lpr = 8; lpr <= 32 && !done; lpr *= 2) {
        if (nch % lpr || (nch / lpr != 3 && nch / lpr != 5)) continue;
        if (lpr == 8) done = ln_rows_launch<T, MODE, 8>(a, nrows, nch / lpr, st);
        else if (lpr == 16) done = ln_rows_launch<T, MODE, 16>(a, nrows, nch / lpr, st);
        else done = ln_rows_launch<T, MODE, 32>(a, nrows, nch / lpr, st);
      }
    }
    if (done) { DPB_CHECK(hipGetLastError()); return 0; }
  }
  const dim3 grid((unsigned)((nrows + 3) / 4));
  const int need = (a.C / CH + 63) / 64;
  if (need <= 1) DPB_LAUNCH((ln_kernel<T, MODE, 1>), grid, dim3(256), 0, st, a, nrows);
  else if (need <= 2) DPB_LAUNCH((ln_kernel<T, MODE, 2>), grid, dim3(256), 0, st, a, nrows);
  else if (need <= 3) DPB_LAUNCH((ln_kernel<T, MODE, 3>), grid, dim3(256), 0, st, a, nrows);
  else DPB_LAUNCH((ln_kernel<T, MODE, 5>), grid, dim3(256), 0, st, a, nrows);
  DPB_CHECK(hipGetLastError());
  return 0;
}

int launch_layernorm(int dtype, int mode, const LNArgs& a, hipStream_t st) {
  if (mode == MODE_PRIMAL) return DPB_DISPATCH_T(dtype, T, (ln_launch<T, MODE_PRIMAL>(a, st)));
  if (mode == MODE_TANGENT) return DPB_DISPATCH_T(dtype, T, (ln_launch<T, MODE_TANGENT>(a, st)));
  return DPB_DISPATCH_T(dtype, T, (ln_launch<T, MODE_ADJOINT>(a, st)));
}

}
```

Baseline: 122.5 iters/s.

## Fold feed-forward output and proj_out linears into one tangent GEMM

Detects a linear (FF out) feeding another linear (proj_out) with a residual, and precomputes a concatenated weight [Wpo | Wpo·W_ff] at setup. In tangent passes, the residual tangent and the GEGLU tangent are written side by side in one strided buffer, so the two chained GEMMs become a single GEMM with K = C+F, and the first linear is skipped. Strided leading dimensions are threaded through the layernorm, geglu, nchw→nhwc, split-k reduce and LN epilogue paths. The cost is extra workspace and a setup-time GEMM, plus bf16 rounding differences from the pre-multiplied weights.

```diff
diff --git a/diffusion_pullback_amd/csrc/elementwise.hip b/diffusion_pullback_amd/csrc/elementwise.hip
--- a/diffusion_pullback_amd/csrc/elementwise.hip
+++ b/diffusion_pullback_amd/csrc/elementwise.hip
@@ -47,7 +47,7 @@
       Vec<T>::load(dp + ca + dg_, dg);
 #pragma unroll
       for (int e = 0; e < CH; ++e) o[e] = da[e] * av[e] + dg[e] * gv[e];
-      Vec<T>::store((T*)a.y + row * a.F + c, o);
+      Vec<T>::store((T*)a.y + row * (a.ldy ? a.ldy : a.F) + c, o);
     } else {
       float gy[CH], o2[CH];
       Vec<T>::load((const T*)a.d + row * a.F + c, gy);
@@ -209,7 +209,7 @@
 }
 
 template <typename T>
-__global__ __launch_bounds__(256) void nchw_to_nhwc_kernel(const float* src, T* dst, int C, int HW, int Cpad) {
+__global__ __launch_bounds__(256) void nchw_to_nhwc_kernel(const float* src, T* dst, int C, int HW, int Cpad, int ldd) {
   __shared__ float tile[32][33];
   const int n = blockIdx.z;
   const int p0 = blockIdx.x * 32, c0 = blockIdx.y * 32;
@@ -221,7 +221,7 @@
   __syncthreads();
   for (int k = ty; k < 32; k += 8) {
     int p = p0 + k, c = c0 + tx;
-    if (p < HW && c < Cpad) TT<T>::st(dst + ((long)n * HW + p) * Cpad + c, tile[tx][k]);
+    if (p < HW && c < Cpad) TT<T>::st(dst + ((long)n * HW + p) * ldd + c, tile[tx][k]);
   }
 }
 template <typename T>
@@ -240,9 +240,9 @@
     if (c < C && p < HW) dst[((long)n * C + c) * HW + p] = tile[tx][k];
   }
 }
-int launch_nchw_to_nhwc(int dtype, const float* src, void* dst, int n, int C, int HW, int Cpad, hipStream_t st) {
+int launch_nchw_to_nhwc(int dtype, const float* src, void* dst, int n, int C, int HW, int Cpad, hipStream_t st, int ldd) {
   dim3 grid((HW + 31) / 32, (Cpad + 31) / 32, n);
-  DPB_DISPATCH_STMT(dtype, T, DPB_LAUNCH((nchw_to_nhwc_kernel<T>), grid, dim3(256), 0, st, src, (T*)dst, C, HW, Cpad));
+  DPB_DISPATCH_STMT(dtype, T, DPB_LAUNCH((nchw_to_nhwc_kernel<T>), grid, dim3(256), 0, st, src, (T*)dst, C, HW, Cpad, ldd ? ldd : Cpad));
   DPB_CHECK(hipGetLastError());
   return 0;
 }
diff --git a/diffusion_pullback_amd/csrc/engine.cpp b/diffusion_pullback_amd/csrc/engine.cpp
--- a/diffusion_pullback_amd/csrc/engine.cpp
+++ b/diffusion_pullback_amd/csrc/engine.cpp
@@ -29,6 +29,17 @@
   int rows = 0, C = 0, kind = 0, Cv = 0;
   bool is_const = true;
   size_t p_off = 0, t_off = 0, g_off = 0, g_off0 = 0;
+  int t_ld = 0;
+};
+
+struct FfPlan {
+  int ff_op = -1, po_op = -1;
+  int h2 = -1, g = -1;
+  int C = 0, F = 0;
+  size_t W = 0;
+  size_t T = 0, Tg = 0;
+  bool built = false;
+  bool on = false;
 };
 
 struct AttnPlan {
@@ -55,6 +66,7 @@
   int ln_next = -1;
   int ln_prev = -1;
   int fold_plan = -1, fold_role = 0;
+  int ff_plan = -1, ff_role = 0;
 };
 
 }
@@ -67,6 +79,7 @@
   std::vector<Buf> bufs;
   std::vector<Op> ops;
   std::vector<AttnPlan> plans;
+  std::vector<FfPlan> ffs;
   std::vector<int> producer;
   std::vector<std::vector<int>> mod_users;
   int x_buf = -1, x_channels = 0, temb_buf = -1, temb_dim = 0, temb_flip = 0, temb_hm1 = 0, ctx_buf = -1;
@@ -204,6 +217,23 @@
 bool fold_on(const dpb_engine* e, const Pass& ps, const AttnPlan& p) {
   return p.fold_live && fold_route(e, p) && e->producer[ps.src] < p.q_op && e->producer[ps.tap] >= p.o_op;
 }
+int g_ff_fold = getenv("DPB_FF_FOLD") ? atoi(getenv("DPB_FF_FOLD")) : 1;
+bool ff_route(const dpb_engine* e, const Pass& ps, const FfPlan& p) {
+  if (!g_ff_fold || !p.built || ps.mode != MODE_TANGENT || !ps.bact[p.h2]) return false;
+  return e->producer[ps.src] <= e->producer[p.h2] && e->producer[ps.tap] >= p.po_op;
+}
+void ff_layout(dpb_engine* e, const Pass& ps) {
+  for (FfPlan& p : e->ffs) {
+    p.on = ff_route(e, ps, p);
+    Buf &h = e->bufs[p.h2], &g = e->bufs[p.g];
+    h.t_off = p.T;
+    h.t_ld = p.on ? p.C + p.F : p.C;
+    g.t_off = p.on ? p.T + (size_t)p.C * e->es : p.Tg;
+    g.t_ld = p.on ? p.C + p.F : p.F;
+  }
+}
+bool ff_on(const dpb_engine* e, const Op& op) { return op.ff_plan >= 0 && e->ffs[op.ff_plan].on; }
+
 int gemm(dpb_engine* e, GemmArgs a, bool can_defer = false) {
   if (e->pend.on)
     if (int r = flush_pending(e)) return r;
@@ -227,8 +257,11 @@
   const Buf& bi = e->bufs[d.in0];
   const Buf& bo = e->bufs[d.out];
   if (mode == 1 && !ps.bact[d.in0]) {
+    const Buf& br = e->bufs[d.res];
+    if (br.t_ld != br.C || bo.t_ld != bo.C) return launch_copy_cols(e->dtype, e->T(d.res), br.t_ld, 0, e->T(d.out), bo.t_ld, 0, (long)n * bo.rows, bo.C, 0, e->stream);
     return launch_axpy(e->dtype, e->T(d.res), e->T(d.out), (long)n * bo.rows * bo.C, 0, e->stream);
   }
+  if (mode == 1 && op.ff_role == 1 && ff_on(e, op)) return 0;
   GemmArgs g;
   const bool shared_out = bo.kind == DPB_BUF_SHARED;
   const int ns = shared_out ? 1 : n;
@@ -238,8 +271,8 @@
   g.N = Cout;
   g.K = KS * KS * Cin;
   g.ldb = g.K;
-  g.ldc = bo.C;
-  g.lda = bi.C;
+  g.ldc = mode == 0 ? bo.C : bo.t_ld;
+  g.lda = mode == 0 ? bi.C : bi.t_ld;
   g.gather = d.ip[9];
   if (g.gather == GATHER_NONE) {
     g.M = ns * bi.rows;
@@ -258,7 +291,12 @@
   }
   if (d.res >= 0 && (mode == 0 || ps.bact[d.res])) {
     g.R = mode == 0 ? primal_ptr(e, ps, d.res) : e->T(d.res);
-    g.ldr = e->bufs[d.res].C;
+    g.ldr = mode == 0 ? e->bufs[d.res].C : e->bufs[d.res].t_ld;
+  }
+  if (mode == 1 && op.ff_role == 2 && ff_on(e, op)) {
+    const FfPlan& p = e->ffs[op.ff_plan];
+    g.A = e->T(p.h2); g.lda = p.C + p.F;
+    g.B = e->ws + p.W; g.K = g.ldb = p.C + p.F;
   }
   if (mode == 1 && op.fold_role && fold_on(e, ps, e->plans[op.fold_plan])) {
     const AttnPlan& p = e->plans[op.fold_plan];
@@ -281,7 +319,7 @@
     const dpb_op_desc& gd = e->ops[op.geglu_next].d;
     GemmArgs f = g;
     f.epi = EPI_GEGLU_TAN; f.hprim = e->P(d.out); f.epi_kps = n / e->cur_batch; f.rows_per_sample = bo.rows;
-    f.C = e->T(gd.out); f.ldc = e->bufs[gd.out].C;
+    f.C = e->T(gd.out); f.ldc = e->bufs[gd.out].t_ld;
     gemm_prep(e, f);
     if (gemm_epi_supported(e->dtype, f)) {
       e->skip[op.geglu_next] = 1;
@@ -397,7 +435,7 @@
   const GemmArgs& g = e->pend.a;
   src.slab = g.slab; src.splitk = g.splitk; src.MN = (long)g.M * g.N; src.N = g.N;
   src.R = g.R; src.ldr = g.ldr;
-  src.store = store ? g.C : nullptr;
+  src.store = store ? g.C : nullptr; src.lds = g.ldc;
   e->pend.on = false;
 }
 
@@ -458,6 +496,7 @@
   a.gamma = (const float*)d.w[0];
   a.beta = (const float*)d.w[1];
   a.rows_per_sample = bi.rows; a.C = bi.C; a.eps = d.fp[0];
+  if (ps.mode == MODE_TANGENT) a.ldd = bi.t_ld;
   fill_norm_io(e, d, ps, n, a);
   return launch_layernorm(e->dtype, ps.mode, a, e->stream);
 }
@@ -470,6 +509,7 @@
   a.rows_per_sample = bi.rows; a.F = bi.C / 2; a.il = d.ip[1];
   a.stash = ps.fwd.stash;
   fill_io(e, d, ps, n, a);
+  if (ps.mode == MODE_TANGENT) a.ldy = e->bufs[d.out].t_ld;
   return launch_geglu(e->dtype, ps.mode, a, e->stream);
 }
 
@@ -1055,6 +1095,34 @@
       if (!plain(od) || od.in0 != d.out || uses[d.out] != 1) continue;
       p.q_op = (int)j - 1; p.o_op = (int)j + 1; p.fold_ok = true;
     }
+    for (size_t j = 0; j + 1 < e->ops.size() && e->dtype != DT_F32; ++j) {
+      const dpb_op_desc& fd = e->ops[j].d;
+      auto linear = [&](const Op& o) {
+        const dpb_op_desc& c = o.d;
+        return c.kind == DPB_OP_CONV && c.ip[9] == DPB_GATHER_NONE && c.ip[6] == 1 && c.res >= 0 && c.rowbias < 0 && c.w[1] && !o.is_const &&
+               c.ip[5] == e->bufs[c.out].C && e->bufs[c.in0].kind == DPB_BUF_ACT && e->bufs[c.out].kind == DPB_BUF_ACT &&
+               e->bufs[c.res].kind == DPB_BUF_ACT && e->bufs[c.res].C == e->bufs[c.out].C && o.ln_next < 0 && o.geglu_next < 0 && !o.fold_role && o.ff_plan < 0;
+      };
+      if (!linear(e->ops[j]) || uses[fd.out] != 1) continue;
+      const int r = user[fd.out];
+      const dpb_op_desc& pd = e->ops[r].d;
+      if (!linear(e->ops[r]) || pd.in0 != fd.out || pd.res == fd.out || e->bufs[pd.out].rows != e->bufs[fd.out].rows || e->bufs[pd.out].C != e->bufs[fd.out].C) continue;
+      const int h2 = fd.res, g = fd.in0, hp = e->producer[h2], gp = e->producer[g];
+      if (h2 == g || hp < 0 || gp < 0 || e->bufs[h2].is_const || e->bufs[g].is_const || e->bufs[h2].rows != e->bufs[g].rows) continue;
+      const dpb_op_desc& hd = e->ops[hp].d;
+      if (hd.kind != DPB_OP_CONV || hd.ip[9] != DPB_GATHER_NONE || e->ops[gp].d.kind != DPB_OP_GEGLU || uses[g] != 1) continue;
+      bool ok = true;
+      for (size_t i = 0; i < e->ops.size(); ++i)
+        for (int b : op_inputs(e->ops[i].d))
+          if (b == h2 && (int)i != (int)j && e->ops[i].d.kind != DPB_OP_LAYERNORM) ok = false;
+      for (const FfPlan& q : e->ffs) ok = ok && q.h2 != h2 && q.g != h2 && q.h2 != g && q.g != g;
+      if (!ok) continue;
+      FfPlan p;
+      p.ff_op = (int)j; p.po_op = r; p.h2 = h2; p.g = g; p.C = e->bufs[h2].C; p.F = e->bufs[g].C;
+      e->ops[j].ff_plan = e->ops[r].ff_plan = (int)e->ffs.size();
+      e->ops[j].ff_role = 1; e->ops[r].ff_role = 2;
+      e->ffs.push_back(p);
+    }
     e->skip.assign(e->ops.size(), 0);
   }
   size_t off = 0;
@@ -1064,8 +1132,20 @@
     size_t n = e->maxB;
     b.p_off = take(n * b.rows * (size_t)b.C * es);
   }
-  for (auto& b : e->bufs)
-    if (!b.is_const) b.t_off = take((size_t)e->maxT * b.rows * b.C * es);
+  for (auto& b : e->bufs) b.t_ld = b.C;
+  for (FfPlan& p : e->ffs) {
+    const size_t hb = align_up((size_t)e->maxT * e->bufs[p.h2].rows * p.C * es);
+    p.T = take(hb + (size_t)e->maxT * e->bufs[p.g].rows * p.F * es);
+    p.Tg = p.T + hb;
+    p.W = take((size_t)p.C * (p.C + p.F) * es);
+    e->bufs[p.h2].t_off = p.T; e->bufs[p.g].t_off = p.Tg;
+  }
+  for (size_t i = 0; i < e->bufs.size(); ++i) {
+    Buf& b = e->bufs[i];
+    bool paired = false;
+    for (const FfPlan& p : e->ffs) paired = paired || p.h2 == (int)i || p.g == (int)i;
+    if (!b.is_const && !paired) b.t_off = take((size_t)e->maxT * b.rows * b.C * es);
+  }
   for (auto& b : e->bufs)
     if (!b.is_const) b.g_off = b.g_off0 = take((size_t)e->maxT * b.rows * b.C * es);
   size_t s1 = 0, s2 = 0, t1 = 0, dv = 0, ctmp = 0, maxrc = 0;
@@ -1169,6 +1249,20 @@
   e->ws = (char*)ws;
   e->cur_batch = 0;
   DPB_CHECK(hipMemsetAsync(ws, 0, e->ws_bytes, e->stream));
+  for (FfPlan& p : e->ffs) {
+    p.built = false;
+    const void* Wpo = e->ops[p.po_op].d.w[0];
+    const int ldw = p.C + p.F;
+    e->pend.on = false;
+    GemmArgs g;
+    g.A = Wpo; g.lda = p.C;
+    g.B = e->ops[p.ff_op].d.w[1]; g.ldb = p.C;
+    g.C = e->ws + p.W + (size_t)p.C * e->es; g.ldc = ldw;
+    g.M = p.C; g.N = p.F; g.K = p.C;
+    if (int r = gemm(e, g)) return r;
+    if (int r = launch_copy_cols(e->dtype, Wpo, p.C, 0, e->ws + p.W, ldw, 0, p.C, p.C, 0, e->stream)) return r;
+    p.built = true;
+  }
   return 0;
 }
 
@@ -1347,8 +1441,9 @@
   const Pass ps(e, MODE_TANGENT, tap, src, flags);
   const LaunchSpan span(e);
   e->flops = 0; e->gbytes = 0;
+  ff_layout(e, ps);
   const Buf& bx = e->bufs[src];
-  if (int r = launch_nchw_to_nhwc(e->dtype, V, e->T(src), nt, seed_channels(e, src), bx.rows, bx.C, e->stream)) return r;
+  if (int r = launch_nchw_to_nhwc(e->dtype, V, e->T(src), nt, seed_channels(e, src), bx.rows, bx.C, e->stream, bx.t_ld)) return r;
   if (e->tstats_bytes && !gn_deterministic()) DPB_CHECK(hipMemsetAsync(e->ws + e->tstats_off, 0, e->tstats_bytes, e->stream));
   const int last = e->producer[tap];
   std::fill(e->skip.begin(), e->skip.end(), 0);
@@ -1765,6 +1860,7 @@
   else if (!strcmp(key, "ln_fuse")) { g_ln_fuse = value; return 0; }
   else if (!strcmp(key, "cross_primal")) { g_cross_primal = value; return 0; }
   else if (!strcmp(key, "cross_fold")) { g_cross_fold = value; return 0; }
+  else if (!strcmp(key, "ff_fold")) { g_ff_fold = value; return 0; }
   else if (!strcmp(key, "geglu_fwd")) { g_geglu_fwd = value; return 0; }
   else if (!strcmp(key, "iter_alias")) { g_iter_alias = value; return 0; }
   else return fail("unknown debug key %s", key);
diff --git a/diffusion_pullback_amd/csrc/epilogue.h b/diffusion_pullback_amd/csrc/epilogue.h
--- a/diffusion_pullback_amd/csrc/epilogue.h
+++ b/diffusion_pullback_amd/csrc/epilogue.h
@@ -41,7 +41,8 @@
 __device__ __forceinline__ void epilogue_ln(const GemmArgs& p, bf16* C, const bf16* R, const float* smem_f, int wave, int lane, int mrow0_block, const LnPre<WN>& q) {
   constexpr int NI = 2 * WN / 64;
   static_assert(2 * WN % 64 == 0, "N = 2 WN must be a multiple of 64");
-  const OutBuf ob2 = out_buf(EPI == EPI_LN_TAN ? p.C2 : (void*)C, (long)p.M * p.ldc * 2);
+  const int ld2 = EPI == EPI_LN_TAN ? p.N : p.ldc;
+  const OutBuf ob2 = out_buf(EPI == EPI_LN_TAN ? p.C2 : (void*)C, (long)p.M * ld2 * 2);
   const int wy = wave >> 1, rg = lane >> 3, l = lane & 7;
   const float inv_c = 1.f / (float)p.N;
   float gam[NI][8];
@@ -106,7 +107,7 @@
 #pragma unroll
         for (int e = 0; e < 8; ++e) o[e] += old[e];
       }
-      store8_at<FL>(ob2, (EPI == EPI_LN_TAN ? (bf16*)p.C2 : C) + (long)m * p.ldc + n, o);
+      store8_at<FL>(ob2, (EPI == EPI_LN_TAN ? (bf16*)p.C2 : C) + (long)m * ld2 + n, o);
     }
   }
 }
diff --git a/diffusion_pullback_amd/csrc/gemm.hip b/diffusion_pullback_amd/csrc/gemm.hip
--- a/diffusion_pullback_amd/csrc/gemm.hip
+++ b/diffusion_pullback_amd/csrc/gemm.hip
@@ -521,7 +521,7 @@
 int gemm_epi_supported(int dtype, const GemmArgs& a) {
   if (a.epi == EPI_LN_TAN || a.epi == EPI_LN_ADJ) {
     const GemmTile& ln = kGemmTiles[T_R64_LN];
-    return dtype != DT_F32 && a.Z1 * a.Z2 == 1 && a.gather == GATHER_NONE && a.N == ln.bn && a.ldc == ln.bn && a.M >= ln.bm && a.K % 64 == 0 && a.zeros &&
+    return dtype != DT_F32 && a.Z1 * a.Z2 == 1 && a.gather == GATHER_NONE && a.N == ln.bn && (a.epi == EPI_LN_TAN ? a.ldc >= ln.bn && a.ldc % 8 == 0 : a.ldc == ln.bn) && a.M >= ln.bm && a.K % 64 == 0 && a.zeros &&
            a.ln_x && a.ln_gamma && !a.A2 && !a.bias && !a.rowbias && a.alpha == 1.f && (a.epi == EPI_LN_ADJ || (a.C2 && !a.accumulate)) && (!a.R || a.ldr % 8 == 0);
   }
   if (dtype == DT_F32 || a.Z1 * a.Z2 != 1 || a.gather != GATHER_NONE || a.N % 128 || a.M <= 0) return 0;
@@ -639,7 +639,7 @@
   }
   if (r) return r;
   if (a.splitk > 1) {
-    const bool plain = Z == 1 && a.alpha == 1.f && !a.bias && !a.rowbias && !a.accumulate && a.ldc == a.N && a.vec_ok && !(a.N & 7) && a.epi == EPI_PLAIN;
+    const bool plain = Z == 1 && a.alpha == 1.f && !a.bias && !a.rowbias && !a.accumulate && a.vec_ok && !(a.N & 7) && a.epi == EPI_PLAIN;
     if (t_pending && plain) {
       *t_pending = a;
     } else {
diff --git a/diffusion_pullback_amd/csrc/kernels.h b/diffusion_pullback_amd/csrc/kernels.h
--- a/diffusion_pullback_amd/csrc/kernels.h
+++ b/diffusion_pullback_amd/csrc/kernels.h
@@ -153,6 +153,7 @@
   const float* slab = nullptr; int splitk = 0; long MN = 0; int N = 0;
   const void* R = nullptr; int ldr = 0;
   void* store = nullptr;
+  int lds = 0;
 };
 struct GNArgs {
   const void* x = nullptr;
@@ -186,6 +187,7 @@
   int rows_per_sample = 0, Bp = 1, NT = 0, kps = 1, C = 0;
   float eps = 1e-5f;
   int accumulate = 0;
+  int ldd = 0;
   SlabSrc src;
 };
 int launch_layernorm(int dtype, int mode, const LNArgs& a, hipStream_t st);
@@ -235,6 +237,7 @@
   int rows_per_sample = 0, Bp = 1, NT = 0, kps = 1, F = 0;
   int accumulate = 0;
   int stash = 1;
+  int ldy = 0;
   int il = 0;
 };
 int launch_geglu(int dtype, int mode, const GegluArgs& a, hipStream_t st);
@@ -246,7 +249,7 @@
 int launch_copy_cols(int dtype, const void* src, int lds, int cs0, void* dst, int ldd, int cd0, long rows, int ncols,
                      int accumulate, hipStream_t st);
 int launch_zero_cols(int dtype, void* dst, int ldd, int cd0, long rows, int ncols, hipStream_t st);
-int launch_nchw_to_nhwc(int dtype, const float* src, void* dst, int n, int C, int HW, int Cpad, hipStream_t st);
+int launch_nchw_to_nhwc(int dtype, const float* src, void* dst, int n, int C, int HW, int Cpad, hipStream_t st, int ldd = 0);
 int launch_nhwc_to_nchw(int dtype, const void* src, float* dst, int n, int C, int HW, int Cpad, hipStream_t st);
 constexpr int SHIFT_MAX_ROWS = 64;
 struct ShiftRows { int dir[SHIFT_MAX_ROWS]; float scale[SHIFT_MAX_ROWS]; };
diff --git a/diffusion_pullback_amd/csrc/norm.hip b/diffusion_pullback_amd/csrc/norm.hip
--- a/diffusion_pullback_amd/csrc/norm.hip
+++ b/diffusion_pullback_amd/csrc/norm.hip
@@ -51,7 +51,7 @@
     for (int e = 0; e < CH; ++e) v[e] += r[e];
   }
   const uint4 packed = Raw<T>::pack(v);
-  if (s.store) *reinterpret_cast<uint4*>((T*)s.store + row * s.N + c0) = packed;
+  if (s.store) *reinterpret_cast<uint4*>((T*)s.store + row * (s.lds ? s.lds : s.N) + c0) = packed;
   return packed;
 }
 
@@ -613,7 +613,7 @@
       Vec<T>::load(xp + c * CH, x[i]);
       if (MODE != MODE_PRIMAL) {
         if (a.src.slab) Raw<T>::unpack(slab_chunk<T>(a.src, row, c * CH), v[i]);
-        else Vec<T>::load((const T*)a.d + row * a.C + c * CH, v[i]);
+        else Vec<T>::load((const T*)a.d + row * (a.ldd ? a.ldd : a.C) + c * CH, v[i]);
       }
 #pragma unroll
       for (int e = 0; e < CH; ++e) s += x[i][e];
@@ -714,7 +714,7 @@
     Vec<T>::load(xp + c * CH, x[i]);
     if (MODE != MODE_PRIMAL) {
       if (a.src.slab) { if (live) Raw<T>::unpack(slab_chunk<T>(a.src, r, c * CH), v[i]); else for (int e = 0; e < CH; ++e) v[i][e] = 0.f; }
-      else Vec<T>::load((const T*)a.d + r * a.C + c * CH, v[i]);
+      else Vec<T>::load((const T*)a.d + r * (a.ldd ? a.ldd : a.C) + c * CH, v[i]);
     }
 #pragma unroll
     for (int e = 0; e < CH; ++e) s += x[i][e];
```

New measurement: 123.7 iters/s, median of 6. No clear change (+0.9%).
